# lanterndata/lantern

Measured on AMD Instinct MI355X. Metric: QPS (recall@10 alongside), 1000000x768 f32 l2sq ef=64 k=10, higher is better.
Workload: dtype f32

## Files before the change

include/lantern_gpu.h:

```cpp
#ifndef LANTERN_GPU_H
#define LANTERN_GPU_H

#include <stdbool.h>
#include <stddef.h>
#include <stdint.h>

#ifdef __cplusplus
extern "C" {
#endif

#define LANTERN_GPU_EXPORT __attribute__((visibility("default")))


typedef void       *usearch_index_t;
typedef uint64_t    usearch_key_t;
typedef uint64_t    usearch_label_t;
typedef float       usearch_distance_t;
typedef const char *usearch_error_t;

typedef enum usearch_metric_kind_t {
    usearch_metric_unknown_k = 0,
    usearch_metric_cos_k = 1,
    usearch_metric_l2sq_k = 3,
    usearch_metric_hamming_k = 8
// ... 170 lines not shown
                                                                 size_t query_stride_bytes, size_t nq, size_t k, size_t ef, size_t skip,
                                                                 uint64_t *d_labels, float *d_distances, uint32_t *d_slots,
                                                                 uint32_t *d_counts, uint64_t *d_dist_evals, uint64_t *d_expansions,
                                                                 void *stream, usearch_error_t *);
LANTERN_GPU_EXPORT void lantern_gpu_search_batch_filtered_each(usearch_index_t, const lantern_gpu_filter_t *const *filters, const void *queries,
                                                               size_t nq, usearch_scalar_kind_t, size_t k, size_t ef, usearch_label_t *labels,
                                                               float *distances, uint32_t *counts, usearch_error_t *);
LANTERN_GPU_EXPORT void lantern_gpu_search_batch_filtered_each_device(usearch_index_t, const lantern_gpu_filter_t *const *filters,
                                                                      const void *d_queries, size_t query_stride_bytes, size_t nq, size_t k,
                                                                      size_t ef, size_t skip, uint64_t *d_labels, float *d_distances,
                                                                      uint32_t *d_slots, uint32_t *d_counts, uint64_t *d_dist_evals,
                                                                      uint64_t *d_expansions, void *stream, usearch_error_t *);
LANTERN_GPU_EXPORT void lantern_gpu_search_batch_filtered_each_lane(usearch_index_t, int lane, const lantern_gpu_filter_t *const *filters,
                                                                    const void *queries, size_t nq, usearch_scalar_kind_t, size_t k, size_t ef,
                                                                    usearch_label_t *labels, float *distances, uint32_t *counts,
                                                                    usearch_error_t *);
LANTERN_GPU_EXPORT void lantern_gpu_last_filtered_each(usearch_index_t, uint32_t out[6], usearch_error_t *);
LANTERN_GPU_EXPORT void lantern_gpu_set_search_shape(usearch_index_t, int waves_per_query, int max_workgroups,
                                                     usearch_error_t *);

LANTERN_GPU_EXPORT void lantern_gpu_exact_search(usearch_index_t, const void *queries, size_t nq, size_t k,
                                                 uint32_t *slots, float *distances, usearch_error_t *);

LANTERN_GPU_EXPORT size_t lantern_gpu_dense_profile(int on, float *ms, uint32_t *rows, uint32_t *cols, uint32_t *fused, size_t cap);
LANTERN_GPU_EXPORT void lantern_gpu_exact_knn_stats(uint64_t *queries, uint64_t *certified, uint64_t *fallback);

LANTERN_GPU_EXPORT void lantern_gpu_search_row_trace(usearch_index_t, int on, size_t nq, size_t per_query_cap, uint32_t *trace,
                                                     uint32_t *counts, usearch_error_t *);

LANTERN_GPU_EXPORT int lantern_gpu_last_search_grid(usearch_index_t, usearch_error_t *);
LANTERN_GPU_EXPORT const char *lantern_gpu_plan_search(const int64_t in[31], uint32_t out[12]);
LANTERN_GPU_EXPORT const char *lantern_gpu_plan_search_screen(const int64_t in[32], uint32_t out[13]);
LANTERN_GPU_EXPORT const char *lantern_gpu_plan_search_screen_prefetch(const int64_t in[33], uint32_t out[14]);

LANTERN_GPU_EXPORT void lantern_gpu_distance_gather(usearch_index_t, const void *query, const uint32_t *slots,
                                                    size_t n, float *out, usearch_error_t *);
LANTERN_GPU_EXPORT float lantern_gpu_last_gather_ms(usearch_index_t, usearch_error_t *);
LANTERN_GPU_EXPORT void lantern_gpu_search_screen_stats(usearch_index_t, uint64_t *logical, uint64_t *exact, usearch_error_t *);
LANTERN_GPU_EXPORT void lantern_gpu_set_insert_screen(usearch_index_t, int mode, usearch_error_t *);
LANTERN_GPU_EXPORT void lantern_gpu_insert_screen_stats(usearch_index_t, uint64_t out[4], usearch_error_t *);
LANTERN_GPU_EXPORT const char *lantern_gpu_plan_insert(const int64_t in[13], uint32_t out[7]);
LANTERN_GPU_EXPORT size_t lantern_gpu_export_screen(usearch_index_t, size_t first, size_t count, int8_t *rows, float *meta, float *norms,
                                                    usearch_error_t *);
LANTERN_GPU_EXPORT void lantern_gpu_screen_probe(usearch_index_t, const void *query, const uint32_t *slots, size_t n, float radius,
                                                 int workgroup, uint8_t *rejected, usearch_error_t *);
LANTERN_GPU_EXPORT void lantern_gpu_distance_matrix(const void *a, size_t na, const void *b, size_t nb,
                                                    usearch_scalar_kind_t, size_t dims, usearch_metric_kind_t,
                                                    int exact_order, float *out, usearch_error_t *);

LANTERN_GPU_EXPORT void lantern_gpu_assign_to_clusters(const float *dataset, size_t n, size_t row_dims, size_t subvector_start,
                                                       size_t subvector_dim, const float *centers, size_t k,
                                                       usearch_metric_kind_t metric, uint32_t *out_cluster,
                                                       float *out_distance, usearch_error_t *);

typedef struct lantern_gpu_graph_info
{
    size_t   size;
    size_t   upper_blocks;
    uint32_t connectivity;
    uint32_t entry_slot;
    int32_t  max_level;
    uint32_t vector_words;
} lantern_gpu_graph_info;
LANTERN_GPU_EXPORT lantern_gpu_graph_info lantern_gpu_graph_info_get(usearch_index_t, usearch_error_t *);
LANTERN_GPU_EXPORT void lantern_gpu_export_graph(usearch_index_t, uint8_t *levels, uint32_t *nbr0, uint32_t *upper_off,
                                                 uint32_t *upper_nbr, uint64_t *labels, void *vectors,
                                                 usearch_error_t *);
LANTERN_GPU_EXPORT void lantern_gpu_export_codes(usearch_index_t, uint8_t *codes, usearch_error_t *);
LANTERN_GPU_EXPORT void lantern_gpu_pq_compact(usearch_index_t, usearch_error_t *);
LANTERN_GPU_EXPORT void lantern_gpu_pq_expand(usearch_index_t, usearch_error_t *);
LANTERN_GPU_EXPORT size_t lantern_gpu_row_bytes(usearch_index_t, usearch_error_t *);
LANTERN_GPU_EXPORT void lantern_gpu_memory_usage(usearch_index_t, size_t *row_bytes, size_t *other_bytes, usearch_error_t *);
LANTERN_GPU_EXPORT void lantern_gpu_import_graph(usearch_index_t, size_t size, const void *vectors,
                                                 const uint64_t *labels, const uint8_t *levels, const uint32_t *nbr0,
                                                 const uint32_t *upper_off, const uint32_t *upper_nbr,
                                                 uint32_t entry_slot, int32_t max_level, usearch_error_t *);
// ... 143 lines not shown
```

lantern_amd/capi.py:

```python
from __future__ import annotations

import ctypes as C
import os

import numpy as np

HERE = os.path.dirname(os.path.abspath(__file__))
LIB_PATH = os.path.join(HERE, "lib", "liblantern_gpu.so")

METRIC_COS, METRIC_L2SQ, METRIC_HAMMING = 1, 3, 8
SCALAR_F32, SCALAR_F16, SCALAR_I8, SCALAR_B1 = 1, 3, 4, 5
METRICS = {"cos": METRIC_COS, "l2sq": METRIC_L2SQ, "hamming": METRIC_HAMMING}
EMPTY = 0xFFFFFFFF
USEARCH_HEADER_SIZE = 136


class LanternGpuError(RuntimeError):
    pass


class InitOptions(C.Structure):
    _fields_ = [
        ("metric_kind", C.c_int),
        ("metric", C.c_void_p),
# ... 54 lines not shown
    "lantern_gpu_set_seed", "lantern_gpu_set_add_batch", "lantern_gpu_add_many", "lantern_gpu_flush",
    "lantern_gpu_add_with_level", "lantern_gpu_search_batch", "lantern_gpu_search_batch_device", "lantern_gpu_search_batch_device_strided",
    "lantern_gpu_set_search_shape", "lantern_gpu_exact_search", "lantern_gpu_dense_profile", "lantern_gpu_exact_knn_stats", "lantern_gpu_distance_gather",
    "lantern_gpu_host_alloc", "lantern_gpu_host_free", "lantern_gpu_save_stream", "lantern_gpu_pq_compact", "lantern_gpu_pq_expand", "lantern_gpu_memory_usage", "lantern_gpu_spec_profile", "lantern_gpu_search_unique_rows", "lantern_gpu_search_row_trace", "lantern_gpu_last_search_grid", "lantern_gpu_last_gather_ms", "lantern_gpu_search_screen_stats",
    "lantern_gpu_set_insert_screen", "lantern_gpu_insert_screen_stats", "lantern_gpu_plan_insert",
    "lantern_gpu_distance_matrix", "lantern_gpu_assign_to_clusters", "lantern_gpu_graph_info_get", "lantern_gpu_export_graph", "lantern_gpu_import_graph",
    "lantern_gpu_export_codes",
    "lantern_gpu_counters_get", "lantern_gpu_set_profiling", "lantern_gpu_build_profile_get", "lantern_gpu_search_phase_profile", "lantern_scan_begin", "lantern_scan_rescan", "lantern_scan_gettuple", "lantern_scan_trace", "lantern_scan_end",
    "lantern_l2sq_dist", "lantern_cos_dist", "lantern_hamming_dist", "lantern_index_server_start", "lantern_index_server_start_tls",
    "lantern_index_server_port", "lantern_index_server_status_port", "lantern_index_server_status",
    "lantern_index_server_served", "lantern_index_server_stop",
    "lantern_gpu_graph_checksum", "lantern_gpu_comm_unique_id", "lantern_gpu_comm_init_rccl", "lantern_gpu_comm_init_host",
    "lantern_gpu_comm_init_local", "lantern_gpu_comm_free", "lantern_gpu_comm_rank", "lantern_gpu_comm_world",
    "lantern_gpu_comm_set_timeout", "lantern_gpu_comm_stats", "lantern_gpu_comm_allgatherv_host",
    "lantern_gpu_comm_allgatherv_device", "lantern_gpu_shard_range", "lantern_gpu_add_sharded", "lantern_gpu_add_row_sharded", "lantern_gpu_search_partitioned", "lantern_gpu_search_batch_lane", "lantern_gpu_search_batch_lane_notify", "lantern_gpu_row_bytes",
    "lantern_gpu_level_for", "lantern_gpu_plan_batch", "lantern_gpu_row_shard_plan", "lantern_gpu_plan_search", "lantern_gpu_plan_search_screen", "lantern_gpu_plan_search_screen_prefetch",
    "lantern_scan_server_start", "lantern_scan_server_start_fn", "lantern_scan_server_port", "lantern_scan_server_stats",
    "lantern_scan_server_batch_histogram", "lantern_scan_server_timing", "lantern_scan_server_stop", "lantern_scan_client_connect", "lantern_scan_client_search", "lantern_scan_client_search_next",
    "lantern_scan_client_close", "lantern_scan_begin_client",
    "lantern_mirror_acquire", "lantern_mirror_index", "lantern_mirror_version", "lantern_mirror_rebind", "lantern_mirror_advance", "lantern_mirror_release",
    "lantern_mirror_invalidate", "lantern_mirror_set_capacity", "lantern_mirror_stats",
    "UsearchNodeBytes", "usearch_init_node", "node_tuple_size", "label_from_node", "level_from_node", "reset_node_label", "get_node_neighbors_mut",
    "lantern_quant_bits_scalar_kind",
    "lantern_gpu_filter_from_labels", "lantern_gpu_filter_from_slot_bitmap", "lantern_gpu_filter_count", "lantern_gpu_filter_free",
    "lantern_gpu_set_filter_policy", "lantern_gpu_filter_stats", "lantern_gpu_last_filtered_launch", "lantern_gpu_search_batch_filtered", "lantern_gpu_search_batch_filtered_device",
    "lantern_gpu_cursor_search_filtered", "lantern_scan_set_filter",
    "lantern_gpu_filter_resident_bytes", "lantern_scan_server_start_filtered_fn", "lantern_scan_server_filter_stats", "lantern_scan_client_set_filter",
    "lantern_scan_client_clear_filter",
    "lantern_gpu_search_batch_filtered_each", "lantern_gpu_search_batch_filtered_each_device", "lantern_gpu_search_batch_filtered_each_lane", "lantern_gpu_last_filtered_each",
    "lantern_gpu_set_filter_seeds", "lantern_gpu_last_filtered_seeds",
    "lantern_gpu_search_batch_params", "lantern_gpu_search_batch_params_lane", "lantern_gpu_search_batch_params_lane_notify",
    "lantern_gpu_search_batch_params_device", "lantern_gpu_last_params_launch", "lantern_scan_server_start_params_fn",
    "lantern_gpu_export_screen", "lantern_gpu_screen_probe",
]
QUERY_PARAMS = np.dtype([("k", np.uint32), ("ef", np.uint32), ("skip", np.uint32), ("reserved", np.uint32)])


def query_params(params) -> np.ndarray:
    if isinstance(params, np.ndarray) and params.dtype == QUERY_PARAMS:
        return np.ascontiguousarray(params)
    out = np.zeros(len(params), dtype=QUERY_PARAMS)
    for i, p in enumerate(params):
        p = tuple(int(x) for x in p)
        out[i] = (p[0], p[1] if len(p) > 1 else 0, p[2] if len(p) > 2 else 0, 0)
    return out


FILTER_SKIP_DELETED = 1
FILTER_PATHS = {"auto": 0, "walk": 1, "exact": 2}

BATCH_SEARCH_FN = C.CFUNCTYPE(C.c_int, C.c_void_p, C.c_void_p, C.c_size_t, C.c_size_t, C.c_size_t, C.c_size_t, C.POINTER(C.c_uint64),
                              C.POINTER(C.c_float), C.POINTER(C.c_uint32), C.POINTER(C.c_char_p))

FILTER_MAKE_FN = C.CFUNCTYPE(C.c_void_p, C.c_void_p, C.POINTER(C.c_uint64), C.c_size_t, C.c_uint32, C.POINTER(C.c_uint64), C.POINTER(C.c_uint64),
                             C.POINTER(C.c_char_p))
FILTER_FREE_FN = C.CFUNCTYPE(None, C.c_void_p, C.c_void_p)
BATCH_SEARCH_PARAMS_FN = C.CFUNCTYPE(C.c_int, C.c_void_p, C.c_void_p, C.c_size_t, C.c_size_t, C.c_void_p, C.c_size_t, C.POINTER(C.c_uint64),
                                     C.POINTER(C.c_float), C.POINTER(C.c_uint32), C.POINTER(C.c_char_p))
BATCH_SEARCH_EACH_FN = C.CFUNCTYPE(C.c_int, C.c_void_p, C.POINTER(C.c_void_p), C.c_void_p, C.c_size_t, C.c_size_t, C.c_size_t, C.c_size_t,
                                   C.POINTER(C.c_uint64), C.POINTER(C.c_float), C.POINTER(C.c_uint32), C.POINTER(C.c_char_p))

QUERIES_DONE_FN = C.CFUNCTYPE(None, C.c_void_p, C.POINTER(C.c_uint32), C.c_size_t)
ALLGATHERV_FN = C.CFUNCTYPE(C.c_int, C.c_void_p, C.c_void_p, C.POINTER(C.c_size_t), C.POINTER(C.c_size_t), C.c_int, C.c_int)
COMM_ID_BYTES = 128

_lib = None
# ... 28 lines not shown
        "usearch_save": (None, [vp, C.c_char_p, err]),
        "usearch_save_buffer": (None, [vp, vp, sz, err]),
        "usearch_load": (None, [vp, C.c_char_p, err]),
        "usearch_load_buffer": (None, [vp, vp, sz, err]),
        "usearch_serialized_length": (sz, [vp, err]),
        "usearch_header_get_entry_slot": (u64, [vp]),
        "usearch_header_set_entry_slot": (None, [vp, u64]),
        "usearch_view_mem_lazy": (None, [vp, vp, err]),
        "usearch_update_header": (None, [vp, vp, err]),
        "lantern_gpu_version": (C.c_char_p, []),
        "lantern_gpu_device_count": (i32, []),
        "lantern_gpu_set_seed": (None, [vp, u64, err]),
        "lantern_gpu_set_add_batch": (None, [vp, sz, sz, err]),
        "lantern_gpu_add_many": (None, [vp, vp, vp, sz, i32, err]),
        "lantern_gpu_flush": (None, [vp, err]),
        "lantern_gpu_add_with_level": (None, [vp, u64, vp, i32, i32, err]),
        "lantern_gpu_search_batch": (None, [vp, vp, sz, i32, sz, sz, vp, vp, vp, err]),
        "lantern_gpu_search_batch_device": (None, [vp, vp, sz, sz, sz, sz, vp, vp, vp, vp, vp, vp, vp, err]),
        "lantern_gpu_search_batch_device_strided": (None, [vp, vp, sz, sz, sz, sz, sz, vp, vp, vp, vp, vp, vp, vp, err]),
        "lantern_gpu_set_search_shape": (None, [vp, i32, i32, err]),
        "lantern_gpu_exact_search": (None, [vp, vp, sz, sz, vp, vp, err]),
        "lantern_gpu_dense_profile": (sz, [i32, vp, vp, vp, vp, sz]),
        "lantern_gpu_exact_knn_stats": (None, [C.POINTER(u64), C.POINTER(u64), C.POINTER(u64)]),
        "lantern_gpu_distance_gather": (None, [vp, vp, vp, sz, vp, err]),
        "lantern_gpu_spec_profile": (None, [vp, i32, vp, err]),
        "lantern_gpu_search_unique_rows": (None, [vp, i32, C.POINTER(u64), err]),
        "lantern_gpu_search_row_trace": (None, [vp, i32, sz, sz, vp, vp, err]),
        "lantern_gpu_last_search_grid": (i32, [vp, err]),
        "lantern_gpu_last_gather_ms": (f32, [vp, err]),
        "lantern_gpu_search_screen_stats": (None, [vp, C.POINTER(u64), C.POINTER(u64), err]),
        "lantern_gpu_set_insert_screen": (None, [vp, C.c_int, err]),
        "lantern_gpu_insert_screen_stats": (None, [vp, vp, err]),
        "lantern_gpu_export_screen": (sz, [vp, sz, sz, vp, vp, vp, err]),
        "lantern_gpu_screen_probe": (None, [vp, vp, vp, sz, f32, i32, vp, err]),
        "lantern_gpu_save_stream": (None, [vp, vp, vp, err]),
        "lantern_gpu_pq_compact": (None, [vp, err]),
        "lantern_gpu_pq_expand": (None, [vp, err]),
        "lantern_gpu_memory_usage": (None, [vp, C.POINTER(sz), C.POINTER(sz), err]),
        "lantern_gpu_distance_matrix": (None, [vp, sz, vp, sz, i32, sz, i32, i32, vp, err]),
        "lantern_gpu_assign_to_clusters": (None, [vp, sz, sz, sz, sz, vp, sz, i32, vp, vp, err]),
        "lantern_gpu_graph_info_get": (GraphInfo, [vp, err]),
        "lantern_gpu_export_graph": (None, [vp, vp, vp, vp, vp, vp, vp, err]),
        "lantern_gpu_import_graph": (None, [vp, sz, vp, vp, vp, vp, vp, vp, u32, C.c_int32, err]),
        "lantern_gpu_export_codes": (None, [vp, vp, err]),
        "lantern_gpu_counters_get": (Counters, [vp, err]),
        "lantern_gpu_set_profiling": (None, [vp, i32, err]),
        "lantern_gpu_build_profile_get": (BuildProfile, [vp, err]),
        "lantern_gpu_search_phase_profile": (None, [vp, i32, vp, err]),
        "lantern_scan_begin": (vp, [vp, i32, i32, err]),
        "lantern_scan_rescan": (None, [vp, vp, i32, err]),
        "lantern_scan_gettuple": (C.c_bool, [vp, C.POINTER(u64), err]),
        "lantern_scan_trace": (sz, [vp, vp, sz]),
        "lantern_scan_end": (None, [vp]),
        "lantern_l2sq_dist": (f32, [vp, i32, vp, i32, err]),
        "lantern_cos_dist": (f32, [vp, i32, vp, i32, err]),
        "lantern_hamming_dist": (C.c_int32, [vp, i32, vp, i32, err]),
        "lantern_index_server_start": (vp, [C.c_char_p, i32, i32, C.c_char_p, err]),
        "lantern_index_server_start_tls": (vp, [C.c_char_p, i32, i32, C.c_char_p, C.c_char_p, C.c_char_p, err]),
        "lantern_index_server_port": (i32, [vp]),
        "lantern_index_server_status_port": (i32, [vp]),
        "lantern_index_server_status": (i32, [vp]),
        "lantern_index_server_served": (u64, [vp]),
        "lantern_index_server_stop": (None, [vp]),
        "lantern_gpu_graph_checksum": (u64, [vp, err]),
        "lantern_gpu_comm_unique_id": (None, [vp, err]),
        "lantern_gpu_comm_init_rccl": (vp, [i32, i32, vp, err]),
        "lantern_gpu_comm_init_host": (vp, [i32, i32, ALLGATHERV_FN, vp, err]),
        "lantern_gpu_comm_init_local": (None, [i32, C.POINTER(vp), err]),
        "lantern_gpu_comm_free": (None, [vp]),
        "lantern_gpu_comm_rank": (i32, [vp]),
        "lantern_gpu_comm_world": (i32, [vp]),
        "lantern_gpu_comm_set_timeout": (None, [vp, C.c_double]),
        "lantern_gpu_comm_stats": (None, [vp, C.POINTER(u64), C.POINTER(u64)]),
        "lantern_gpu_comm_allgatherv_host": (None, [vp, vp, C.POINTER(sz), C.POINTER(sz), err]),
        "lantern_gpu_comm_allgatherv_device": (None, [vp, vp, C.POINTER(sz), C.POINTER(sz), vp, err]),
        "lantern_gpu_shard_range": (None, [sz, i32, i32, C.POINTER(sz), C.POINTER(sz)]),
        "lantern_gpu_add_sharded": (None, [vp, vp, vp, vp, sz, i32, err]),
        "lantern_gpu_add_row_sharded": (None, [vp, vp, vp, vp, sz, i32, err]),
        "lantern_gpu_search_partitioned": (None, [vp, vp, vp, sz, i32, sz, sz, vp, vp, vp, err]),
        "lantern_gpu_row_bytes": (sz, [vp, err]),
        "lantern_gpu_search_batch_lane": (None, [vp, i32, vp, sz, i32, sz, sz, vp, vp, vp, err]),
        "lantern_gpu_search_batch_lane_notify": (None, [vp, i32, vp, sz, i32, sz, sz, vp, vp, vp, vp, vp, err]),
        "lantern_gpu_level_for": (i32, [u64, u64, u32]),
        "lantern_gpu_plan_batch": (sz, [sz, i32, vp, sz, sz, sz]),
        "lantern_gpu_plan_search": (C.c_char_p, [vp, vp]),
        "lantern_gpu_plan_search_screen": (C.c_char_p, [vp, vp]),
        "lantern_gpu_plan_search_screen_prefetch": (C.c_char_p, [vp, vp]),
        "lantern_gpu_plan_insert": (C.c_char_p, [vp, vp]),
        "lantern_gpu_row_shard_plan": (sz, [vp, i32, u64, u32, sz, sz, vp, vp, vp, sz]),
        "lantern_scan_server_start": (vp, [vp, C.c_char_p, i32, sz, C.c_uint, err]),
        "lantern_scan_server_start_fn": (vp, [BATCH_SEARCH_FN, vp, sz, C.c_char_p, i32, sz, C.c_uint, err]),
        "lantern_scan_server_port": (i32, [vp]),
        "lantern_scan_server_stats": (None, [vp, C.POINTER(u64), C.POINTER(u64), C.POINTER(u64), C.POINTER(u64)]),
        "lantern_scan_server_batch_histogram": (sz, [vp, C.POINTER(u64), sz]),
        "lantern_scan_server_timing": (None, [vp, C.POINTER(C.c_double)]),
        "lantern_scan_server_stop": (None, [vp]),
        "lantern_scan_client_connect": (vp, [C.c_char_p, i32, err]),
        "lantern_scan_client_search": (sz, [vp, vp, sz, sz, sz, vp, vp, err]),
        "lantern_scan_client_search_next": (sz, [vp, vp, sz, sz, sz, vp, vp, err]),
        "lantern_scan_client_close": (None, [vp]),
        "lantern_scan_begin_client": (vp, [vp, sz, i32, i32, err]),
        "lantern_mirror_acquire": (vp, [u64, u64, C.POINTER(InitOptions), vp, vp, sz, err]),
        "lantern_mirror_index": (vp, [vp]),
        "lantern_mirror_version": (u64, [vp]),
        "lantern_mirror_rebind": (None, [vp, C.POINTER(InitOptions)]),
        "lantern_mirror_advance": (None, [vp, u64]),
        "lantern_mirror_release": (None, [vp]),
        "lantern_mirror_invalidate": (None, [u64]),
        "lantern_mirror_set_capacity": (None, [sz]),
        "lantern_mirror_stats": (None, [C.POINTER(u64), C.POINTER(u64), C.POINTER(u64), C.POINTER(u64)]),
        "UsearchNodeBytes": (u32, [C.POINTER(Metadata), i32, i32]),
        "usearch_init_node": (None, [C.POINTER(Metadata), vp, u64, u32, u64, vp, sz]),
        "node_tuple_size": (u32, [vp, u32, C.POINTER(Metadata)]),
        "label_from_node": (u64, [vp]),
        "level_from_node": (C.c_ulong, [vp]),
        "reset_node_label": (None, [vp]),
        "get_node_neighbors_mut": (vp, [C.POINTER(Metadata), vp, u32, C.POINTER(u32)]),
        "lantern_quant_bits_scalar_kind": (i32, [i32, C.c_bool, err]),
        "lantern_gpu_filter_from_labels": (vp, [vp, vp, sz, u32, err]),
        "lantern_gpu_filter_from_slot_bitmap": (vp, [vp, vp, sz, u32, err]),
# ... 236 lines not shown

    def unique_rows(self, on, read=False):
        out = C.c_uint64(0)
        _call("lantern_gpu_search_unique_rows", self.h, 1 if on else 0, C.byref(out) if read else None)
        return int(out.value) if read else None

    def last_gather_ms(self) -> float:
        return float(_call("lantern_gpu_last_gather_ms", self.h))

    def screen_stats(self):
        logical, exact = C.c_uint64(0), C.c_uint64(0)
        _call("lantern_gpu_search_screen_stats", self.h, C.byref(logical), C.byref(exact))
        return int(logical.value), int(exact.value)

    def set_insert_screen(self, mode):
        _call("lantern_gpu_set_insert_screen", self.h, int(mode))

    def insert_screen_stats(self):
        out = np.zeros(4, dtype=np.uint64)
        _call("lantern_gpu_insert_screen_stats", self.h, _ptr(out))
        return tuple(int(x) for x in out)

    def export_screen(self, first=0, count=None):
        if count is None:
            count = len(self) - first
        row_bytes = int(_call("lantern_gpu_export_screen", self.h, first, count, None, None, None))
        if row_bytes == 0:
            return {"codes": np.zeros((count, 0), np.int8), "meta": None, "norms": None, "row_bytes": 0}
        codes, meta = np.zeros((count, row_bytes), np.int8), np.zeros((count, 2), np.float32)
        norms = np.zeros(count, np.float32) if self.metric == METRIC_COS else None
        _call("lantern_gpu_export_screen", self.h, first, count, _ptr(codes), _ptr(meta), _ptr(norms))
        return {"codes": codes, "meta": meta, "norms": norms, "row_bytes": row_bytes}

    def screen_probe(self, query, slots, radius, workgroup=256):
        q = _rows(query, self.metric)[0]
        s = np.ascontiguousarray(slots, dtype=np.uint32)
        out = np.zeros(s.size, dtype=np.uint8)
        _call("lantern_gpu_screen_probe", self.h, _ptr(q), _ptr(s), s.size, float(radius), int(workgroup), _ptr(out))
        return out.astype(bool)

    def last_search_grid(self) -> int:
        return int(_call("lantern_gpu_last_search_grid", self.h))

    def row_trace_begin(self, nq, per_query_cap):
        self._trace_shape = (int(nq), int(per_query_cap))
        _call("lantern_gpu_search_row_trace", self.h, 1, int(nq), int(per_query_cap), None, None)

    def row_trace_end(self):
        nq, cap = self._trace_shape
        trace = np.zeros((nq, cap), dtype=np.uint32)
        counts = np.zeros(nq, dtype=np.uint32)
        _call("lantern_gpu_search_row_trace", self.h, 0, nq, cap, _ptr(trace), _ptr(counts))
        return trace, counts

    def pq_compact(self):
        _call("lantern_gpu_pq_compact", self.h)

    def pq_expand(self):
        _call("lantern_gpu_pq_expand", self.h)

    def row_bytes(self) -> int:
        return int(_call("lantern_gpu_row_bytes", self.h))

    def memory_usage(self):
        a, b = C.c_size_t(), C.c_size_t()
        _call("lantern_gpu_memory_usage", self.h, C.byref(a), C.byref(b))
# ... 452 lines not shown
    m = Metadata()
    m.neighbors_bytes, m.neighbors_base_bytes = 4 + M * 6, 4 + 2 * M * 6
    m.inverse_log_connectivity = 1.0 / math.log(M)
    m.connectivity, m.dimensions = M, dims
    o = m.init_options
    o.metric_kind, o.quantization, o.dimensions, o.connectivity = metric, quantization, dims, M
    o.pq, o.num_subvectors, o.num_centroids = pq, num_subvectors, num_centroids
    return m


def header_entry_slot(header: bytes) -> int:
    buf = C.create_string_buffer(bytes(header), USEARCH_HEADER_SIZE)
    return int(lib().usearch_header_get_entry_slot(C.cast(buf, C.c_void_p)))


def level_for(seed: int, slot: int, M: int) -> int:
    return int(lib().lantern_gpu_level_for(seed, slot, M))


def plan_batch(size: int, max_level: int, pending_levels, max_batch: int, min_ratio: int) -> int:
    lv = np.ascontiguousarray(pending_levels, dtype=np.int32)
    return int(lib().lantern_gpu_plan_batch(size, max_level, _ptr(lv), lv.size, max_batch, min_ratio))


PLAN_SEARCH_IN = ("chunks", "M", "M0", "mcode", "n", "ef_default", "num_cus", "pq_compact", "pqd_inv", "pq_S16", "search_vis_slots", "search_max_wg",
                  "phase_profile", "spec_profile", "nq", "k", "ef", "skip", "waves", "each", "max_expansion", "env_spec_set", "env_spec",
                  "env_adc_spec_set", "env_adc_spec", "env_pq_adc", "env_spec_waves", "env_lds_list", "env_wide_rows", "env_solo", "env_waves_per_cu")
PLAN_SEARCH_OUT = ("path", "spec", "expansion", "waves", "grid", "vis_slots", "lds", "spec_prefetch", "spec_cache", "wide_rows", "took_spec", "lds_list")


def plan_search(fields) -> tuple[dict, str | None]:
    vals = [fields[n] for n in PLAN_SEARCH_IN] if isinstance(fields, dict) else list(fields)
    assert len(vals) == len(PLAN_SEARCH_IN)
    if isinstance(fields, dict) and "screen_list_prefetch" in fields:
        names = PLAN_SEARCH_OUT + ("screen_lds", "list_prefetch")
        a = np.asarray(vals + [fields.get("screen", 0), fields["screen_list_prefetch"]], dtype=np.int64)
        out = np.zeros(len(names), dtype=np.uint32)
        why = lib().lantern_gpu_plan_search_screen_prefetch(_ptr(a), _ptr(out))
    elif isinstance(fields, dict) and "screen" in fields:
        names = PLAN_SEARCH_OUT + ("screen_lds",)
        a, out = np.asarray(vals + [fields["screen"]], dtype=np.int64), np.zeros(len(names), dtype=np.uint32)
        why = lib().lantern_gpu_plan_search_screen(_ptr(a), _ptr(out))
    else:
        names = PLAN_SEARCH_OUT
        a, out = np.asarray(vals, dtype=np.int64), np.zeros(len(names), dtype=np.uint32)
        why = lib().lantern_gpu_plan_search(_ptr(a), _ptr(out))
    return dict(zip(names, (int(x) for x in out))), (why.decode() if why else None)


PLAN_INSERT_IN = ("mcode", "chunks", "M0", "efc", "rows", "num_cus", "waves", "screen_table", "mode", "lds_list", "only_upper", "lone_ok", "vis_slots_env")
PLAN_INSERT_OUT = ("screened", "vis_slots", "lds", "screen_lds", "lone", "spec_prefetch", "spec_cache")


def plan_insert(fields) -> tuple[dict, str | None]:
    vals = [fields[n] for n in PLAN_INSERT_IN] if isinstance(fields, dict) else list(fields)
    assert len(vals) == len(PLAN_INSERT_IN)
    a, out = np.asarray(vals, dtype=np.int64), np.zeros(len(PLAN_INSERT_OUT), dtype=np.uint32)
    why = lib().lantern_gpu_plan_insert(_ptr(a), _ptr(out))
    return dict(zip(PLAN_INSERT_OUT, (int(x) for x in out))), (why.decode() if why else None)


def row_shard_plan(shard_sizes, seed: int, M: int, max_batch: int, min_ratio: int):
    sizes = np.ascontiguousarray(shard_sizes, dtype=np.uint64)
    world = int(sizes.size)
    n = int(lib().lantern_gpu_row_shard_plan(_ptr(sizes), world, seed, M, max_batch, min_ratio, None, None, None, 0))
    first, count = np.zeros(max(n, 1), dtype=np.uintp), np.zeros(max(n, 1), dtype=np.uintp)
    share = np.zeros((max(n, 1), world), dtype=np.uintp)
# ... 370 lines not shown
```

lantern_amd/csrc/device_common.hpp:

```cpp
#pragma once
#include <hip/hip_runtime.h>
#include <stdint.h>

namespace lgpu {

constexpr uint32_t EMPTY = 0xFFFFFFFFu;
#ifndef LGPU_ROW_BLOCK
#define LGPU_ROW_BLOCK 3
#endif
#ifndef LGPU_ROW_BLOCK_COS
#define LGPU_ROW_BLOCK_COS 2
#endif
#ifndef LGPU_LIST_PREFETCH
#define LGPU_LIST_PREFETCH 1
#endif
#ifndef LGPU_SCREEN_LIST_PREFETCH
#define LGPU_SCREEN_LIST_PREFETCH 1
#endif
#ifndef LGPU_ROW_BLOCK1
#define LGPU_ROW_BLOCK1 4
#endif
#ifndef LGPU_SCREEN
#define LGPU_SCREEN 1
#endif
// ... 466 lines not shown
    for(int r = 0; r < R; ++r) d[ r ] = acc[ r ].template finish_n<G>(a2, b2[ r ]);
}

__host__ __device__ inline int group_lanes_for(uint32_t chunks) { return chunks >= 128 ? 64 : chunks >= 64 ? 32 : chunks >= 32 ? 16 : 8; }

struct View
{
    const uint4    *vec;
    uint32_t        chunks;
    uint32_t        M, M0;
    uint32_t       *nbr0;
    const uint32_t *upper_off;
    uint32_t       *upper_nbr;
    const uint8_t  *levels;
    const float    *norm2;
    uint32_t        n;
    uint32_t        entry;
    int32_t         max_level;
    const uint4    *pq_centers;
    uint32_t        pq_cps;
    uint32_t        pq_C;
    uint32_t        pq_inv;
    uint32_t        pq_row_bytes;
    const uint4    *screen;
    const float2   *screen_meta;
    uint32_t        screen_chunks;
};

__host__ __device__ __forceinline__ float screen_val(float s, uint32_t w, int b) { return s * (float)(int)(int8_t)(uint8_t)(w >> (8 * b)); }
__host__ __device__ inline bool screen_rows_for(uint32_t chunks) { return chunks >= 128; }
__host__ __device__ inline bool screen_cos_norm_ok(float r) { return r >= 0x1p-48f && r <= 0x1p48f; }
__host__ __device__ inline uint32_t screen_chunks_for(uint32_t chunks) { return (chunks + 3) / 4; }
__host__ __device__ inline uint32_t screen_query_lds_bytes(uint32_t chunks) { return 16 + screen_chunks_for(chunks) * 32; }
__host__ __device__ inline bool screen_l2_scale_ok(float s) { return s >= 0x1p-40f && s <= 0x1p40f; }

__device__ __forceinline__ const uint4 *row_of(const View &v, uint32_t slot) { return v.vec + (size_t)slot * v.chunks; }

struct PqdRow
{
    const uint8_t *codes;
    const uint4   *centers;
    uint32_t       cps, C, inv;
    __device__ __forceinline__ uint4 operator[](int ch) const
    {
        const uint32_t sv = ((uint32_t)ch * inv) >> 16, off = (uint32_t)ch - sv * cps;
        const uint32_t code = codes[ sv ];
        return centers[ ((size_t)sv * C + code) * cps + off ];
    }
};
template <int METRIC> __device__ __forceinline__ auto row_of_m(const View &v, uint32_t slot)
{
    if constexpr(METRIC >= M_PQD) return PqdRow{ (const uint8_t *)v.vec + (size_t)slot * v.pq_row_bytes, v.pq_centers, v.pq_cps, v.pq_C, v.pq_inv };
    else return v.vec + (size_t)slot * v.chunks;
}
template <int METRIC> __device__ __forceinline__ float row_norm(const View &v, uint32_t slot)
{
    if constexpr(kCachedNorms<METRIC>) return v.norm2[ slot ];
    else return 0.f;
}

__device__ __forceinline__ uint32_t *neighbors_of(const View &v, uint32_t slot, int level, uint32_t &cap)
{
    if(level == 0) {
        cap = v.M0;
        return v.nbr0 + (size_t)slot * v.M0;
    }
// ... 6 lines not shown
```

lantern_amd/csrc/index.cpp:

```cpp
#include "index.hpp"
#include "abi_guard.hpp"
#include "host_trip.hpp"

#include <algorithm>
#include <cmath>
#include <cstdio>
#include <cstdlib>
#include <cstring>
#include <new>

#include <time.h>

#include "comm.hpp"
#include "host_util.hpp"

static bool exact_knn_device(int mcode, uint32_t chunks, const uint4 *d_base, size_t nb, const uint4 *d_q, size_t nq, size_t k,
                             uint32_t *d_slots, float *d_dists, hipStream_t st);


namespace lgpu {

static const char *kNoDevice = "lantern_gpu: no HIP device available (this library has no CPU fallback)";

const char *set_err(Index *ix, const std::string &msg)
// ... 49 lines not shown
View Index::view() const
{
    View v{};
    v.vec = d_vec;
    v.chunks = chunks;
    v.M = M;
    v.M0 = M0;
    v.nbr0 = d_nbr0;
    v.upper_off = d_upper_off;
    v.upper_nbr = d_upper_nbr;
    v.levels = d_levels;
    v.norm2 = d_norm2;
    v.screen = d_screen;
    v.screen_meta = d_screen_meta;
    v.screen_chunks = d_screen ? screen_chunks_for(chunks) : 0u;
    v.n = (uint32_t)n;
    v.entry = entry;
    v.max_level = max_level;
    return v;
}

static bool reserve_locked(Index *ix, size_t newcap)
{
    if(newcap <= ix->cap) return true;
    if(newcap >= 0x7FFFFFFFull) { set_err(ix, "lantern_gpu: capacity above 2^31-1 slots is not supported"); return false; }
    if(!pq_expand_locked(ix)) return false;
    const size_t oc = ix->cap, row = (size_t)ix->chunks * 16;
    if(!dev_grow(ix, (void **)&ix->d_vec, oc * row, newcap * row, -1)) return false;
    if(mcode_base(ix->mcode) == M_COS && !mcode_is_i8(ix->mcode) && !dev_grow(ix, (void **)&ix->d_norm2, oc * 4, newcap * 4, -1)) return false;
    if(ix->screen) {
        const size_t srow = (size_t)screen_chunks_for(ix->chunks) * 16;
        if(!dev_grow(ix, (void **)&ix->d_screen, oc * srow, newcap * srow, 0)) return false;
        if(!dev_grow(ix, (void **)&ix->d_screen_meta, oc * 8, newcap * 8, 0)) return false;
    }
    if(ix->pq && !dev_grow(ix, (void **)&ix->d_codes, oc * ix->pq_S, newcap * ix->pq_S, 0)) return false;
    if(!dev_grow(ix, (void **)&ix->d_labels, oc * 8, newcap * 8, -1)) return false;
    if(!dev_grow(ix, (void **)&ix->d_levels, oc, newcap, 0)) return false;
    if(!dev_grow(ix, (void **)&ix->d_nbr0, oc * ix->M0 * 4, newcap * ix->M0 * 4, 0xFF)) return false;
    if(!dev_grow(ix, (void **)&ix->d_radius0, oc * 4, newcap * 4, 0xFF)) return false;
    if(!dev_grow(ix, (void **)&ix->d_upper_off, oc * 4, newcap * 4, 0xFF)) return false;
    ix->cap = newcap;
    if(ix->d_bitmaps) { (void)hipFree(ix->d_bitmaps); ix->d_bitmaps = nullptr; }
    ix->bitmap_slots = 0;
    ix->bm_words = 0;
    return true;
}

static bool reserve_upper(Index *ix, size_t need_blocks)
{
    if(need_blocks <= ix->upper_cap) return true;
    size_t nc = std::max<size_t>(std::max<size_t>(ix->upper_cap * 2, need_blocks), 1024);
    if(!dev_grow(ix, (void **)&ix->d_upper_nbr, ix->upper_cap * ix->M * 4, nc * ix->M * 4, 0xFF)) return false;
    if(!dev_grow(ix, (void **)&ix->d_radius_upper, ix->upper_cap * 4, nc * 4, 0xFF)) return false;
    ix->upper_cap = nc;
    return true;
}

bool rows_stored(Index *ix, size_t first, size_t count)
{
    if(count == 0) return true;
    if(ix->d_norm2) HIPCHK(ix, launch_fill_norms(ix->mcode, ix->view(), (uint32_t)first, (uint32_t)count, ix->d_norm2, ix->stream));
    if(ix->d_screen)
        HIPCHK(ix, launch_fill_screen(ix->view(), (uint32_t)first, (uint32_t)count, ix->d_screen, ix->d_screen_meta, ix->mcode == M_COS ? ix->d_norm2 : nullptr, ix->stream));
    return true;
}

bool pq_encode_rows(Index *ix, size_t first, size_t count)
{
    if(!ix->pq || count == 0) return true;
    const uint32_t sub_chunks = (ix->pq_subdim + 3) / 4, sub_floats = sub_chunks * 4, row_floats = ix->chunks * 4;
    float    *d_sub = nullptr;
    uint32_t *d_near = nullptr;
    bool ok = hipMalloc((void **)&d_sub, count * (size_t)sub_floats * 4) == hipSuccess && hipMalloc((void **)&d_near, count * 8) == hipSuccess;
    for(uint32_t sv = 0; ok && sv < ix->pq_S; ++sv) {
        ok = ok && launch_pq_take((const float *)ix->d_vec, row_floats, (uint32_t)first, (uint32_t)count, sv, ix->pq_subdim, sub_floats, d_sub, ix->stream) == hipSuccess;
        ok = ok && ::exact_knn_device(ix->metric, sub_chunks, (const uint4 *)(ix->d_centers + (size_t)sv * ix->pq_C * sub_floats), ix->pq_C, (const uint4 *)d_sub,
                                    count, 1, d_near, (float *)(d_near + count), ix->stream);
        ok = ok && launch_pq_put((float *)ix->d_vec, row_floats, (uint32_t)first, (uint32_t)count, sv, ix->pq_subdim, ix->pq_S, d_near, ix->d_codebook,
                                 (uint32_t)ix->opts.dimensions, ix->d_codes, ix->stream) == hipSuccess;
    }
    ok = ok && hipStreamSynchronize(ix->stream) == hipSuccess;
    if(d_sub) (void)hipFree(d_sub);
    if(d_near) (void)hipFree(d_near);
    if(!ok) set_err(ix, "lantern_gpu: HIP failure while quantising vectors");
    return ok;
}

bool pq_decode_rows(Index *ix, size_t first, size_t count)
{
    if(!ix->pq || count == 0) return true;
    HIPCHK(ix, launch_pq_decode((float *)ix->d_vec, ix->chunks * 4, (uint32_t)first, (uint32_t)count, ix->pq_subdim, ix->pq_S, ix->d_codebook,
                                (uint32_t)ix->opts.dimensions, ix->d_codes, ix->stream));
    return true;
}

static uint32_t pqd_inverse(uint32_t cps, uint32_t chunks)
// ... 328 lines not shown
    const size_t first = ix->n;
    const int    W = comm ? comm->world : 1, R = comm ? comm->rank : 0;
    const bool   split = W > 1 && b >= (size_t)W * kShardMinPerRank;
    const size_t b_lo = split ? b * (size_t)R / (size_t)W : 0, b_hi = split ? b * ((size_t)R + 1) / (size_t)W : b;
    std::vector<uint32_t> &link_off = ix->h_link_off;
    link_off.resize(b);
    size_t total_links = 0;
    for(size_t i = 0; i < b; ++i) {
        link_off[ i ] = (uint32_t)total_links;
        total_links += (size_t)ix->M * (size_t)(lv[ i ] + 1);
    }
    const size_t items = total_links / ix->M;
    uint32_t *d_link_off = (uint32_t *)scratch(ix, kScratchLinkOff, b * 4 + items * 4 + items * 4);
    LinkReq  *d_links = (LinkReq *)scratch(ix, kScratchLinks, total_links * sizeof(LinkReq));
    uint64_t *d_tops = (uint64_t *)scratch(ix, kScratchTops, items * (size_t)ix->efc * 8);
    LinkReq  *d_reqs = (LinkReq *)scratch(ix, kScratchReqs, total_links * sizeof(LinkReq));
    char     *d_grp = (char *)scratch(ix, kScratchGroups, total_links * sizeof(uint2) + 16 + (size_t)W * 4);
    void     *d_work = scratch(ix, kScratchWork, total_links * 8 + 16);
    const size_t temp_bytes = group_temp_bytes(total_links);
    char     *d_sort = (char *)scratch(ix, kScratchSort, total_links * 24 + temp_bytes + 64);
    if(!d_link_off || !d_links || !d_tops || !d_reqs || !d_grp || !d_work || !d_sort) return false;
    uint32_t *d_item_node = d_link_off + b, *d_top_count = d_item_node + items;
    uint2    *d_groups = (uint2 *)d_grp;
    uint32_t *d_ngroups = (uint32_t *)(d_grp + total_links * sizeof(uint2));
    uint32_t *d_owner = d_ngroups + 4;
    GroupScratch gs;
    gs.keys_a = (uint64_t *)d_sort;
    gs.keys_b = gs.keys_a + total_links;
    gs.idx_a = (uint32_t *)(gs.keys_b + total_links);
    gs.idx_b = gs.idx_a + total_links;
    gs.temp = (void *)(((uintptr_t)(gs.idx_b + total_links) + 63) & ~(uintptr_t)63);
    gs.temp_bytes = temp_bytes;

    prof_mark(ix, 0);
    HIPCHK(ix, launch_batch_layout(ix->d_levels + first, (uint32_t)b, ix->M, d_link_off, d_item_node, ix->stream));

    static const bool ins_spec_env = !(std::getenv("LANTERN_GPU_INSERT_SPEC") && std::atoi(std::getenv("LANTERN_GPU_INSERT_SPEC")) == 0);
    InsertPlanIn pin;
    pin.mcode = ix->mcode, pin.num_cus = ix->num_cus, pin.waves = ix->insert_waves;
    pin.chunks = ix->chunks, pin.M0 = ix->M0, pin.efc = ix->efc;
    pin.rows = b_hi - b_lo;
    pin.screen_table = ix->d_screen && ix->d_screen_meta;
    pin.mode = ix->insert_screen;
    pin.lds_list = search_env().lds_list;
    pin.only_upper = rs != nullptr;
    pin.lone_ok = ins_spec_env && !comm && !rs;
    if(const char *vs = std::getenv("LANTERN_GPU_INSERT_VIS_SLOTS")) pin.vis_slots_env = std::max(0, std::atoi(vs));
    const InsertPlan ip = plan_insert(pin);
    if(ip.refusal) { set_err(ix, ip.refusal); return false; }
    const bool ins_spec = ip.lone;
    const int  ins_waves = ins_spec ? 11 : ix->insert_waves;
    const int  grid = ins_spec ? (int)std::max<size_t>(1, std::min<size_t>(b_hi - b_lo, (size_t)ix->num_cus)) : search_grid(ix, b_hi - b_lo, ix->insert_waves, 20);
    if(!ensure_bitmaps(ix, (size_t)grid)) return false;
    if(!order_launch(ix, ix->stream)) return false;
    auto link_at = [&](size_t i) { return i < b ? (size_t)link_off[ i ] : total_links; };

    InsertArgs ia;
    ia.view = ix->view();
    if(!ip.screened) ia.view.screen = nullptr, ia.view.screen_meta = nullptr, ia.view.screen_chunks = 0;
    ia.first_slot = (uint32_t)first;
    ia.b_begin = (uint32_t)b_lo;
    ia.count = (uint32_t)b_hi;
    ia.efc = ix->efc;
    ia.link_off = d_link_off;
    ia.tops = d_tops;
    ia.top_count = d_top_count;
// ... 265 lines not shown
    }
    if(total == 0) return true;
    StagedMeta s;
    if(!stage_meta(ix, nullptr, total, s)) return false;
    const size_t in_bytes = input_bytes(ix, kind_in);
    std::vector<uint32_t> padded;
    const void *src = vectors;
    if(n_shard && !(kind_in == ix->scalar && in_bytes == row)) {
        padded.resize(n_shard * (size_t)ix->chunks * 4);
        for(size_t i = 0; i < n_shard; ++i) pad_row(ix, (const char *)vectors + i * in_bytes, kind_in, &padded[ i * (size_t)ix->chunks * 4 ]);
        src = padded.data();
    }
    char     *vec_base = (char *)ix->d_vec + first * row;
    uint64_t *lab_base = ix->d_labels + first;
    if(n_shard) {
        HIPCHK(ix, hipMemcpyAsync(vec_base + my_off * row, src, n_shard * row, hipMemcpyHostToDevice, ix->stream));
        HIPCHK(ix, hipMemcpyAsync(lab_base + my_off, labels, n_shard * 8, hipMemcpyHostToDevice, ix->stream));
    }
    HIPCHK(ix, hipMemcpyAsync(ix->d_levels + first, s.l8.data(), total, hipMemcpyHostToDevice, ix->stream));
    HIPCHK(ix, hipMemcpyAsync(ix->d_upper_off + first, s.uo.data(), total * 4, hipMemcpyHostToDevice, ix->stream));
    HIPCHK(ix, hipStreamSynchronize(ix->stream));
    size_t at = 0;
    for(int r = 0; r < W; ++r) { off[ (size_t)r ] = at * row; cnt[ (size_t)r ] = (size_t)meta[ (size_t)r * 2 ] * row; at += (size_t)meta[ (size_t)r * 2 ]; }
    if(!comm->allgatherv_device(vec_base, off.data(), cnt.data(), ix->stream)) { set_err(ix, comm->err); return false; }
    for(int r = 0; r < W; ++r) { off[ (size_t)r ] = off[ (size_t)r ] / row * 8; cnt[ (size_t)r ] = cnt[ (size_t)r ] / row * 8; }
    if(!comm->allgatherv_device(lab_base, off.data(), cnt.data(), ix->stream)) { set_err(ix, comm->err); return false; }
    std::vector<uint64_t> all_labels(total);
    HIPCHK(ix, hipMemcpyAsync(all_labels.data(), lab_base, total * 8, hipMemcpyDeviceToHost, ix->stream));
    if(!sync_stream(ix, comm)) return false;
    if(!pq_encode_rows(ix, first, total)) return false;
    if(!rows_stored(ix, first, total)) return false;
    bool ok = true;
    run_batches(ix, all_labels.data(), s, total, comm, &ok);
    return ok;
}

static bool row_shard_candidates(Index *ix, const RowShard &rs, size_t first, size_t b, const uint32_t *d_link_off, uint64_t *d_tops, uint32_t *d_top_count)
{
    Index       *loc = rs.loc;
    Comm        *comm = rs.comm;
    const int    W = comm->world, R = comm->rank;
    const size_t K = rs.K, part = b * K, row = (size_t)ix->chunks * 16;
    char *d_all = (char *)scratch(ix, kScratchShardParts, (size_t)W * part * 12 + 64);
    if(!d_all) return false;
    uint64_t *g_lab = (uint64_t *)d_all;
    float    *g_dist = (float *)(d_all + (size_t)W * part * 8);
    bool ok = true;
    if(loc->n == 0) {
        std::vector<float> inf(part, __builtin_inff());
        ok = hipMemsetAsync(g_lab + (size_t)R * part, 0, part * 8, ix->stream) == hipSuccess &&
             hipMemcpyAsync(g_dist + (size_t)R * part, inf.data(), part * 4, hipMemcpyHostToDevice, ix->stream) == hipSuccess &&
             hipStreamSynchronize(ix->stream) == hipSuccess;
    } else {
        std::lock_guard<std::mutex> gl(loc->mu);
        ok = run_search_device(loc, (const uint4 *)((const char *)ix->d_vec + first * row), b, K, rs.ef, 0,
                               SearchOut{ g_lab + (size_t)R * part, g_dist + (size_t)R * part, nullptr, nullptr, nullptr, nullptr }, ix->stream, loc->search_waves);
        if(!ok) set_err(ix, "lantern_gpu: row-sharded build, candidate search: " + loc->err);
    }
    if(ok && W > 1) {
        std::vector<size_t> off((size_t)W), cnt((size_t)W);
        for(int r = 0; r < W; ++r) { off[ (size_t)r ] = (size_t)r * part * 8; cnt[ (size_t)r ] = part * 8; }
        ok = comm->allgatherv_device(g_lab, off.data(), cnt.data(), ix->stream);
        for(int r = 0; r < W; ++r) { off[ (size_t)r ] = (size_t)r * part * 4; cnt[ (size_t)r ] = part * 4; }
        ok = ok && comm->allgatherv_device(g_dist, off.data(), cnt.data(), ix->stream);
        if(!ok) set_err(ix, "lantern_gpu: row-sharded build, exchange of the candidate lists: " + comm->err);
    }
    ok = ok && launch_merge_candidates(g_lab, g_dist, (uint32_t)W, (uint32_t)b, (uint32_t)K, (uint32_t)first, d_link_off, ix->M, ix->efc, d_tops, d_top_count,
// ... 19 lines not shown
    }
    std::vector<uint32_t> padded(count * row_words);
    for(size_t i = 0; i < count; ++i) pad_row(ix, (const char *)vectors + i * in_bytes, kind_in, &padded[ i * row_words ]);
    HIPCHK(ix, hipMemcpyAsync(dst, padded.data(), count * row, hipMemcpyHostToDevice, ix->stream));
    HIPCHK(ix, hipStreamSynchronize(ix->stream));
    return true;
}

bool add_row_sharded_locked(Index *ix, Comm *comm, const uint64_t *labels, const void *vectors, size_t n_shard, int kind_in)
{
    if(ix->n || !ix->pend_labels.empty()) { set_err(ix, "lantern_gpu: the row-sharded build needs an empty index"); return false; }
    if(ix->pq || ix->b1_from_f32) { set_err(ix, "lantern_gpu: the row-sharded build does not take pq or quant_bits = 1 indexes"); return false; }
    const int    W = comm->world, R = comm->rank;
    const size_t row = (size_t)ix->chunks * 16, M0 = ix->M0, efc = ix->efc, in_bytes = input_bytes(ix, kind_in);
    std::vector<uint64_t> sizes((size_t)W, 0);
    std::vector<size_t>   off((size_t)W), cnt((size_t)W);
    sizes[ (size_t)R ] = n_shard;
    for(int r = 0; r < W; ++r) { off[ (size_t)r ] = (size_t)r * 8; cnt[ (size_t)r ] = 8; }
    if(!comm->allgatherv_host(sizes.data(), off.data(), cnt.data())) { set_err(ix, comm->err); return false; }
    std::vector<size_t> lo((size_t)W + 1, 0);
    for(int r = 0; r < W; ++r) lo[ (size_t)r + 1 ] = lo[ (size_t)r ] + (size_t)sizes[ (size_t)r ];
    const size_t N = lo[ (size_t)W ];
    if(N == 0) return true;
    if(N >= 0x7FFFFFFEull) { set_err(ix, "lantern_gpu: capacity above 2^31-1 slots is not supported"); return false; }
    usearch_error_t err = nullptr;
    usearch_init_options_t lo_opts = ix->opts;
    lo_opts.retriever = lo_opts.retriever_mut = nullptr;
    lo_opts.retriever_ctx = nullptr;
    Index *loc = (Index *)usearch_init(&lo_opts, nullptr, &err);
    if(!loc) { set_err(ix, std::string("lantern_gpu: row-sharded build: ") + (err ? err : "cannot create the shard's index")); return false; }
    struct Cleanup { Index *a = nullptr; ~Cleanup() { usearch_error_t ig = nullptr; if(a) usearch_free(a, &ig); } } cleanup;
    cleanup.a = loc;
    loc->seed = ix->seed;
    loc->efc = ix->efc;
    loc->add_batch_max = ix->add_batch_max;
    loc->add_min_ratio = ix->add_min_ratio;
    if(n_shard) {
        usearch_reserve(loc, n_shard, &err);
        if(err) { set_err(ix, std::string("lantern_gpu: row-sharded build, shard graph: ") + err); return false; }
    }
    StagedMeta s;
    if(!stage_meta(ix, nullptr, N, s)) return false;
    struct Batch { size_t first, b; };
    std::vector<Batch>  plan;
    std::vector<size_t> share;
    {
        std::vector<size_t> pf, pc;
        row_shard_plan(sizes.data(), W, s.lv.data(), N, ix->add_batch_max, ix->add_min_ratio, pf, pc, share);
        for(size_t t = 0; t < pf.size(); ++t) plan.push_back({ pf[ t ], pc[ t ] });
    }
    std::vector<uint64_t> by_rank(N), all_labels(N);
    if(n_shard) std::memcpy(&by_rank[ lo[ (size_t)R ] ], labels, n_shard * 8);
    for(int r = 0; r < W; ++r) { off[ (size_t)r ] = lo[ (size_t)r ] * 8; cnt[ (size_t)r ] = (size_t)sizes[ (size_t)r ] * 8; }
    if(W > 1 && !comm->allgatherv_host(by_rank.data(), off.data(), cnt.data())) { set_err(ix, comm->err); return false; }
    {
        std::vector<size_t> cur(lo.begin(), lo.end() - 1);
        for(size_t t = 0; t < plan.size(); ++t) {
            size_t at = plan[ t ].first;
            for(int r = 0; r < W; ++r)
                for(size_t j = 0; j < share[ t * (size_t)W + (size_t)r ]; ++j) all_labels[ at++ ] = by_rank[ cur[ (size_t)r ]++ ];
        }
    }
    HIPCHK(ix, hipMemcpyAsync(ix->d_labels, all_labels.data(), N * 8, hipMemcpyHostToDevice, ix->stream));
    HIPCHK(ix, hipMemcpyAsync(ix->d_levels, s.l8.data(), N, hipMemcpyHostToDevice, ix->stream));
    HIPCHK(ix, hipMemcpyAsync(ix->d_upper_off, s.uo.data(), N * 4, hipMemcpyHostToDevice, ix->stream));
    HIPCHK(ix, hipStreamSynchronize(ix->stream));
// ... 15 lines not shown
        if(my_n && !stage_rows_at(ix, first + my_off, (const char *)vectors + mine * in_bytes, my_n, kind_in)) return false;
        if(W > 1) {
            size_t at = 0;
            for(int r = 0; r < W; ++r) { off[ (size_t)r ] = at * row; cnt[ (size_t)r ] = sh[ r ] * row; at += sh[ r ]; }
            if(!comm->allgatherv_device((char *)ix->d_vec + first * row, off.data(), cnt.data(), ix->stream)) { set_err(ix, comm->err); return false; }
        }
        if(!rows_stored(ix, first, b)) return false;
        if(ix->n == 0) {
            ix->n = 1;
            ix->entry = 0;
            ix->max_level = s.lv[ 0 ];
            ix->c_add_vectors += 1;
        } else if(!run_batch(ix, b, s.lv.data() + first, nullptr, &rs)) {
            return false;
        }
        if(my_n) {
            gl.resize(my_n);
            for(size_t i = 0; i < my_n; ++i) gl[ i ] = (uint64_t)(first + my_off + i) + 1;
            lantern_gpu_add_many(loc, gl.data(), (const char *)vectors + mine * in_bytes, my_n, (usearch_scalar_kind_t)kind_in, &err);
            if(!err) lantern_gpu_flush(loc, &err);
            if(err) { set_err(ix, std::string("lantern_gpu: row-sharded build, shard graph: ") + err); return false; }
            mine += my_n;
        }
        return sync_stream(ix, comm);
    };
    for(size_t t = 0; t < plan.size() && ok; ++t) ok = batch(t);
    if(ix->profiling) prof_resolve(ix, 0);
    const size_t done = ix->n;
    ix->labels.assign(all_labels.begin(), all_labels.begin() + (ptrdiff_t)done);
    ix->levels.assign(s.l8.begin(), s.l8.begin() + (ptrdiff_t)done);
    ix->upper_off.assign(s.uo.begin(), s.uo.begin() + (ptrdiff_t)done);
    ix->upper_blocks = 0;
    for(size_t i = 0; i < done; ++i) ix->upper_blocks += (size_t)s.lv[ i ];
    return ok;
}

bool flush_locked(Index *ix)
{
    const size_t pending = ix->pend_labels.size();
    if(pending == 0) return true;
    const size_t row_words = (size_t)ix->chunks * 4;
    bool         ok = true;
    const size_t pi = insert_rows(ix, ix->pend_labels.data(), ix->pend_levels.data(), ix->pend_rows.data(), pending, &ok);
    ix->pend_labels.erase(ix->pend_labels.begin(), ix->pend_labels.begin() + (ptrdiff_t)pi);
    ix->pend_levels.erase(ix->pend_levels.begin(), ix->pend_levels.begin() + (ptrdiff_t)pi);
    ix->pend_rows.erase(ix->pend_rows.begin(), ix->pend_rows.begin() + (ptrdiff_t)(pi * row_words));
    if(ix->pend_labels.empty()) { std::vector<uint32_t>().swap(ix->pend_rows); }
    return ok;
}


size_t search_one_locked(Index *ix, Cursor *cur, const void *query, int kind, size_t k, size_t ef, bool streaming, uint64_t *labels,
                         float *distances)
{
    if(!streaming) cur->seen.clear();
    if(ix->n == 0 || k == 0) return 0;
    const size_t want = std::min(cur->seen.size() + k, ix->n);
    const size_t row = (size_t)ix->chunks * 16;
    const size_t need = row + want * 16 + 32;
    if(ix->h_single_bytes < need) {
        if(ix->h_single) (void)hipHostFree(ix->h_single);
        ix->h_single = ix->h_single_dev = nullptr;
        ix->h_single_bytes = 0;
        const size_t cap = need * 2 + 4096;
        if(hipHostMalloc((void **)&ix->h_single, cap, hipHostMallocMapped) != hipSuccess) {
            set_err(ix, "lantern_gpu: cannot allocate the pinned single-query block");
            return 0;
// ... 120 lines not shown
{
    if(ix->n || !ix->pend_labels.empty()) { set_err(ix, "lantern_gpu: import needs an empty index"); return false; }
    if(size == 0) return true;
    if(!pq_expand_locked(ix)) return false;
    size_t blocks = 0;
    for(size_t i = 0; i < size; ++i) blocks += levels[ i ];
    if(!reserve_locked(ix, std::max(size, ix->cap)) || !reserve_upper(ix, blocks)) return false;
    if(ix->pq && vectors_are_codes) {
        HIPCHK(ix, hipMemcpy(ix->d_codes, vectors, size * (size_t)ix->pq_S, hipMemcpyHostToDevice));
        if(!pq_decode_rows(ix, 0, size)) return false;
    } else if(ix->chunks * 4 == ix->words) {
        HIPCHK(ix, hipMemcpy(ix->d_vec, vectors, size * (size_t)ix->words * 4, hipMemcpyHostToDevice));
    } else {
        HIPCHK(ix, hipMemset(ix->d_vec, 0, size * (size_t)ix->chunks * 16));
        HIPCHK(ix, hipMemcpy2D(ix->d_vec, (size_t)ix->chunks * 16, vectors, (size_t)ix->words * 4, (size_t)ix->words * 4, size,
                               hipMemcpyHostToDevice));
    }
    if(ix->pq && !vectors_are_codes && !pq_encode_rows(ix, 0, size)) return false;
    if(!rows_stored(ix, 0, size)) return false;
    ix->labels.resize(size);
    for(size_t i = 0; i < size; ++i) ix->labels[ i ] = labels ? labels[ i ] : (uint64_t)i;
    ix->levels.assign(levels, levels + size);
    ix->upper_off.assign(upper_off, upper_off + size);
    HIPCHK(ix, hipMemcpy(ix->d_labels, ix->labels.data(), size * 8, hipMemcpyHostToDevice));
    HIPCHK(ix, hipMemcpy(ix->d_levels, levels, size, hipMemcpyHostToDevice));
    HIPCHK(ix, hipMemcpy(ix->d_nbr0, nbr0, size * ix->M0 * 4, hipMemcpyHostToDevice));
    HIPCHK(ix, hipMemcpy(ix->d_upper_off, upper_off, size * 4, hipMemcpyHostToDevice));
    if(blocks) HIPCHK(ix, hipMemcpy(ix->d_upper_nbr, upper_nbr, blocks * ix->M * 4, hipMemcpyHostToDevice));
    ix->n = size;
    ix->upper_blocks = blocks;
    ix->radius_stale = true;
    ix->entry = entry_slot;
    ix->max_level = max_level;
    if(ix->pq) {
        const char *pc = std::getenv("LANTERN_GPU_PQ_COMPACT");
        if(pc && std::atoi(pc) != 0 && !pq_compact_locked(ix)) return false;
    }
    return true;
}

}

using namespace lgpu;

Index *lgpu::H(usearch_index_t h, usearch_error_t *e)
{
    if(!h) { FAIL(e, "lantern_gpu: null index handle"); return nullptr; }
    if(((const Index *)h)->magic != kIndexMagic) { FAIL(e, "lantern_gpu: not an index handle (stale, freed or foreign pointer)"); return nullptr; }
    (void)hipSetDevice(((Index *)h)->device);
    return (Index *)h;
}

extern "C" {

const char *lantern_gpu_version(void) { return LGPU_EXPERIMENTAL ? "lantern_gpu 0.1 (gfx950) +experimental" : "lantern_gpu 0.1 (gfx950)"; }

int lantern_gpu_device_count(void)
try {
    int n = 0;
    if(hipGetDeviceCount(&n) != hipSuccess) return 0;
    return n;
}
LANTERN_ABI_CATCH(nullptr)

usearch_index_t usearch_init(usearch_init_options_t *o, float *pq_codebook, usearch_error_t *e)
try {
// ... 64 lines not shown
        ix->pq_subdim = (uint32_t)(o->dimensions / o->num_subvectors);
        const size_t d = o->dimensions, subf = (size_t)((ix->pq_subdim + 3) / 4) * 4;
        ix->h_codebook.assign(pq_codebook, pq_codebook + (size_t)ix->pq_C * d);
        std::vector<float> centers((size_t)ix->pq_S * ix->pq_C * subf, 0.f);
        for(size_t sv = 0; sv < ix->pq_S; ++sv)
            for(size_t c = 0; c < ix->pq_C; ++c)
                std::memcpy(&centers[ (sv * ix->pq_C + c) * subf ], pq_codebook + c * d + sv * ix->pq_subdim, (size_t)ix->pq_subdim * 4);
        const bool ok = hipMalloc((void **)&ix->d_codebook, ix->h_codebook.size() * 4) == hipSuccess &&
                        hipMalloc((void **)&ix->d_centers, centers.size() * 4) == hipSuccess &&
                        hipMemcpy(ix->d_codebook, ix->h_codebook.data(), ix->h_codebook.size() * 4, hipMemcpyHostToDevice) == hipSuccess &&
                        hipMemcpy(ix->d_centers, centers.data(), centers.size() * 4, hipMemcpyHostToDevice) == hipSuccess;
        if(!ok) {
            usearch_error_t ignore = nullptr;
            usearch_free(ix, &ignore);
            FAIL(e, "lantern_gpu: device allocation failed (codebook)");
            return nullptr;
        }
    }
    {
        const char *se = std::getenv("LANTERN_GPU_SCREEN");
        ix->screen = LGPU_SCREEN && (ix->mcode == M_L2SQ || ix->mcode == M_COS) && !ix->pq && screen_rows_for(ix->chunks) && !(se && std::atoi(se) == 0);
        const char *ie = std::getenv("LANTERN_GPU_INSERT_SCREEN");
        ix->insert_screen = ie ? (std::atoi(ie) != 0 ? 1 : 0) : (kInsertScreenByDefault ? 1 : 0);
    }
    return ix;
}
LANTERN_ABI_CATCH(e)

void usearch_free(usearch_index_t h, usearch_error_t *e)
try {
    CLEAR(e);
    Index *ix = H(h, e);
    if(!ix) return;
    void *ptrs[] = { ix->d_vec, ix->d_norm2, ix->d_screen, ix->d_screen_meta, ix->d_labels, ix->d_levels, ix->d_nbr0, ix->d_upper_off, ix->d_upper_nbr, ix->d_bitmaps, ix->d_totals, ix->d_tickets,
                     ix->d_radius0, ix->d_radius_upper,
                     ix->d_codebook, ix->d_centers, ix->d_codes, ix->d_codes16, ix->d_touched, ix->d_trace, ix->d_trace_count };
    for(void *p : ptrs)
        if(p) (void)hipFree(p);
    for(void *p : ix->d_scratch)
        if(p) (void)hipFree(p);
    prof_resolve(ix, 0);
    for(hipEvent_t ev : ix->prof_free) (void)hipEventDestroy(ev);
    if(ix->h_single) (void)hipHostFree(ix->h_single);
    if(ix->h_stage) (void)hipHostFree(ix->h_stage);
    for(int sl = 0; sl < Index::kSearchSlots; ++sl) {
        if(sl > 0 && ix->slot_bitmaps[ sl ]) (void)hipFree(ix->slot_bitmaps[ sl ]);
        if(ix->slot_done[ sl ]) (void)hipEventDestroy(ix->slot_done[ sl ]);
    }
    if(ix->insert_done) (void)hipEventDestroy(ix->insert_done);
    for(hipStream_t ls : ix->lane_stream)
        if(ls) (void)hipStreamDestroy(ls);
    for(char *lh : ix->lane_host)
        if(lh) (void)hipHostFree(lh);
    ix->magic = 0;
    delete ix;
}
LANTERN_ABI_CATCH_VOID(e)

void usearch_reserve(usearch_index_t h, size_t capacity, usearch_error_t *e)
try {
    CLEAR(e);
    Index *ix = H(h, e);
    if(!ix) return;
    std::lock_guard<std::mutex> g(ix->mu);
    if(!reserve_locked(ix, capacity)) FAIL(e, ix->err.c_str());
}
LANTERN_ABI_CATCH_VOID(e)
// ... 8 lines not shown
}
LANTERN_ABI_CATCH(e)

size_t usearch_capacity(usearch_index_t h, usearch_error_t *e)
try {
    CLEAR(e);
    Index *ix = H(h, e);
    if(!ix) return 0;
    std::lock_guard<std::mutex> g(ix->mu);
    return std::max(ix->cap, ix->n + ix->pend_labels.size());
}
LANTERN_ABI_CATCH(e)

size_t usearch_dimensions(usearch_index_t h, usearch_error_t *e)
try {
    CLEAR(e);
    Index *ix = H(h, e);
    return ix ? ix->opts.dimensions : 0;
}
LANTERN_ABI_CATCH(e)

static void add_common(Index *ix, const usearch_label_t *labels, const void *vectors, size_t n, usearch_scalar_kind_t kind,
                       int level, usearch_error_t *e)
try {
    if(!kind_accepted(ix, (int)kind)) { FAIL(e, "lantern_gpu: scalar kind of the vector does not match the index"); return; }
    if(!vectors || !labels) { FAIL(e, "lantern_gpu: null vector or label pointer"); return; }
    std::lock_guard<std::mutex> g(ix->mu);
    const size_t row_words = (size_t)ix->chunks * 4;
    const size_t in_bytes = input_bytes(ix, (int)kind);
    if(n >= ix->add_batch_max && (int)kind == ix->scalar && in_bytes == row_words * 4 && level < 0) {
        if(!flush_locked(ix)) { FAIL(e, ix->err.c_str()); return; }
        bool ok = true;
        insert_rows(ix, labels, nullptr, (const uint32_t *)vectors, n, &ok);
        if(!ok) FAIL(e, ix->err.c_str());
        return;
    }
    if(n >= ix->add_batch_max && (int)kind == usearch_scalar_f32_k && level < 0 &&
       (ix->scalar == usearch_scalar_f16_k || ix->scalar == usearch_scalar_i8_k || ix->b1_from_f32)) {
        if(!flush_locked(ix)) { FAIL(e, ix->err.c_str()); return; }
        bool ok = true;
        insert_rows(ix, labels, nullptr, (const uint32_t *)vectors, n, &ok, true);
        if(!ok) FAIL(e, ix->err.c_str());
        return;
    }
    const size_t base = ix->pend_labels.size();
    try {
        ix->pend_labels.insert(ix->pend_labels.end(), labels, labels + n);
        ix->pend_levels.insert(ix->pend_levels.end(), n, level);
        ix->pend_rows.resize((base + n) * row_words);
    } catch(...) {
        ix->pend_labels.resize(base);
        ix->pend_levels.resize(base);
        ix->pend_rows.resize(base * row_words);
        throw;
    }
    for(size_t i = 0; i < n; ++i) pad_row(ix, (const char *)vectors + i * in_bytes, (int)kind, &ix->pend_rows[ (base + i) * row_words ]);
    if(ix->pend_labels.size() >= ix->add_batch_max && !flush_locked(ix)) FAIL(e, ix->err.c_str());
}
LANTERN_ABI_CATCH_VOID(e)

void usearch_add(usearch_index_t h, usearch_label_t label, const void *vector, usearch_scalar_kind_t kind, usearch_error_t *e)
try {
    CLEAR(e);
    Index *ix = H(h, e);
    if(ix) add_common(ix, &label, vector, 1, kind, -1, e);
}
LANTERN_ABI_CATCH_VOID(e)

void *lantern_gpu_host_alloc(size_t bytes)
try {
    void *p = nullptr;
    if(lantern_gpu_device_count() <= 0 || hipHostMalloc(&p, bytes ? bytes : 1, hipHostMallocDefault) != hipSuccess) return nullptr;
    return p;
}
LANTERN_ABI_CATCH(nullptr)

void lantern_gpu_host_free(void *p)
try {
    if(p) (void)hipHostFree(p);
}
LANTERN_ABI_CATCH_VOID(nullptr)

void lantern_gpu_add_many(usearch_index_t h, const usearch_label_t *labels, const void *vectors, size_t n,
                          usearch_scalar_kind_t kind, usearch_error_t *e)
try {
    CLEAR(e);
    Index *ix = H(h, e);
    if(ix && n) add_common(ix, labels, vectors, n, kind, -1, e);
}
LANTERN_ABI_CATCH_VOID(e)
// ... 120 lines not shown
                                  size_t *first, size_t *count, size_t *share, size_t capacity)
try {
    if(!shard_sizes || world < 1) return 0;
    size_t N = 0;
    for(int r = 0; r < world; ++r) N += (size_t)shard_sizes[ r ];
    std::vector<int> lv(N);
    for(size_t i = 0; i < N; ++i) lv[ i ] = level_for(seed, i, connectivity < 2 ? 2 : connectivity);
    std::vector<size_t> pf, pc, ps;
    row_shard_plan(shard_sizes, world, lv.data(), N, max_batch ? max_batch : 1, min_ratio ? min_ratio : 1, pf, pc, ps);
    for(size_t t = 0; t < pf.size() && t < capacity; ++t) {
        if(first) first[ t ] = pf[ t ];
        if(count) count[ t ] = pc[ t ];
        if(share)
            for(int r = 0; r < world; ++r) share[ t * (size_t)world + (size_t)r ] = ps[ t * (size_t)world + (size_t)r ];
    }
    return pf.size();
}
LANTERN_ABI_CATCH(nullptr)

size_t lantern_gpu_plan_batch(size_t current_size, int max_level, const int *pending_levels, size_t pending, size_t max_batch,
                              size_t min_ratio)
try {
    if(!pending_levels) return 0;
    return plan_batch(current_size, max_level, pending_levels, pending, max_batch ? max_batch : 1, min_ratio ? min_ratio : 1);
}
LANTERN_ABI_CATCH(nullptr)

void lantern_gpu_flush(usearch_index_t h, usearch_error_t *e)
try {
    CLEAR(e);
    Index *ix = H(h, e);
    if(!ix) return;
    std::lock_guard<std::mutex> g(ix->mu);
    if(!flush_locked(ix)) FAIL(e, ix->err.c_str());
}
LANTERN_ABI_CATCH_VOID(e)

void lantern_gpu_set_seed(usearch_index_t h, uint64_t seed, usearch_error_t *e)
try {
    CLEAR(e);
    Index *ix = H(h, e);
    if(ix) ix->seed = seed;
}
LANTERN_ABI_CATCH_VOID(e)

void lantern_gpu_set_add_batch(usearch_index_t h, size_t max_batch, size_t min_ratio, usearch_error_t *e)
try {
    CLEAR(e);
    Index *ix = H(h, e);
    if(!ix) return;
    if(max_batch == 0 || min_ratio == 0) { FAIL(e, "lantern_gpu: batch parameters must be positive"); return; }
    std::lock_guard<std::mutex> g(ix->mu);
    ix->add_batch_max = max_batch;
    ix->add_min_ratio = min_ratio;
}
LANTERN_ABI_CATCH_VOID(e)

void lantern_gpu_set_search_shape(usearch_index_t h, int waves, int max_wg, usearch_error_t *e)
try {
    CLEAR(e);
    Index *ix = H(h, e);
    if(!ix) return;
    if(waves < 0 || waves > 8) { FAIL(e, "lantern_gpu: waves_per_query must be in [1, 8], or 0 = automatic"); return; }
    ix->search_waves = waves;
    ix->insert_waves = waves ? waves : 4;
    ix->search_max_wg = max_wg;
}
// ... 945 lines not shown
    s.mcode = (int)in[ 0 ]; s.chunks = (uint32_t)in[ 1 ]; s.M0 = (uint32_t)in[ 2 ]; s.efc = (uint32_t)in[ 3 ]; s.rows = (size_t)in[ 4 ];
    s.num_cus = (int)in[ 5 ]; s.waves = (int)in[ 6 ]; s.screen_table = in[ 7 ] != 0; s.mode = (int)in[ 8 ]; s.lds_list = in[ 9 ] != 0;
    s.only_upper = in[ 10 ] != 0; s.lone_ok = in[ 11 ] != 0; s.vis_slots_env = (int)in[ 12 ];
    const lgpu::InsertPlan p = lgpu::plan_insert(s);
    const uint32_t flat[ 7 ] = { p.screened ? 1u : 0u, p.vis_slots, (uint32_t)p.lds, p.screen_lds, p.lone ? 1u : 0u, p.spec_prefetch, p.spec_cache };
    std::copy(std::begin(flat), std::end(flat), out);
    return p.refusal;
}

size_t lantern_gpu_export_screen(usearch_index_t h, size_t first, size_t count, int8_t *rows, float *meta, float *norms, usearch_error_t *e)
try {
    CLEAR(e);
    if(count > SIZE_MAX - first) { FAIL(e, "lantern_gpu: slot range out of the index"); return 0; }
    Index *ix = H(h, e);
    if(!ix) return 0;
    std::lock_guard<std::mutex> g(ix->mu);
    if(!flush_locked(ix)) { FAIL(e, ix->err.c_str()); return 0; }
    if(first + count > ix->n) { FAIL(e, "lantern_gpu: slot range out of the index"); return 0; }
    if(!ix->d_screen || !ix->d_screen_meta) return 0;
    const size_t srow = (size_t)screen_chunks_for(ix->chunks) * 16;
    bool         ok = true;
    if(count) {
        if(rows) ok = ok && hipMemcpyAsync(rows, (const char *)ix->d_screen + first * srow, count * srow, hipMemcpyDeviceToHost, ix->stream) == hipSuccess;
        if(meta) ok = ok && hipMemcpyAsync(meta, ix->d_screen_meta + first, count * 8, hipMemcpyDeviceToHost, ix->stream) == hipSuccess;
        if(norms && ix->mcode == M_COS && ix->d_norm2)
            ok = ok && hipMemcpyAsync(norms, ix->d_norm2 + first, count * 4, hipMemcpyDeviceToHost, ix->stream) == hipSuccess;
        ok = ok && hipStreamSynchronize(ix->stream) == hipSuccess;
    }
    if(!ok) { FAIL(e, "lantern_gpu: HIP failure exporting the screen"); return 0; }
    return srow;
}
LANTERN_ABI_CATCH(e)

void lantern_gpu_screen_probe(usearch_index_t h, const void *query, const uint32_t *slots, size_t n, float radius, int workgroup,
                              uint8_t *rejected, usearch_error_t *e)
try {
    CLEAR(e);
    if(n > 64) { FAIL(e, "lantern_gpu: screen_probe takes at most 64 slots"); return; }
    if(workgroup != 256 && workgroup != 512) { FAIL(e, "lantern_gpu: screen_probe workgroup must be 256 or 512"); return; }
    if(!query || (n && (!slots || !rejected))) { FAIL(e, "lantern_gpu: null buffer"); return; }
    Index *ix = H(h, e);
    if(!ix) return;
    std::lock_guard<std::mutex> g(ix->mu);
    if(!flush_locked(ix)) { FAIL(e, ix->err.c_str()); return; }
    if(!ix->d_screen || !ix->d_screen_meta) { FAIL(e, "lantern_gpu: the index has no int8 screen"); return; }
    if(n == 0) return;
    for(size_t i = 0; i < n; ++i)
        if(slots[ i ] >= ix->n) { FAIL(e, "lantern_gpu: slot out of range"); return; }
    const size_t row = (size_t)ix->chunks * 16;
    char        *buf = (char *)scratch(ix, kScratchCallIn, row + n * 4 + 64);
    if(!buf) { FAIL(e, ix->err.c_str()); return; }
    std::vector<uint32_t> padded((size_t)ix->chunks * 4);
    pad_row(ix, query, usearch_scalar_f32_k, padded.data());
    uint32_t *d_slots = (uint32_t *)(buf + row);
    uint8_t  *d_out = (uint8_t *)(buf + row + n * 4);
    bool      ok = hipMemcpyAsync(buf, padded.data(), row, hipMemcpyHostToDevice, ix->stream) == hipSuccess;
    ok = ok && hipMemcpyAsync(d_slots, slots, n * 4, hipMemcpyHostToDevice, ix->stream) == hipSuccess;
    ok = ok && launch_screen_probe(ix->mcode, ix->view(), (const uint4 *)buf, d_slots, (uint32_t)n, radius, workgroup, d_out, ix->stream) == hipSuccess;
    ok = ok && hipMemcpyAsync(rejected, d_out, n, hipMemcpyDeviceToHost, ix->stream) == hipSuccess;
    ok = ok && hipStreamSynchronize(ix->stream) == hipSuccess;
    if(!ok) FAIL(e, "lantern_gpu: HIP failure in screen_probe");
}
LANTERN_ABI_CATCH_VOID(e)

float lantern_gpu_last_gather_ms(usearch_index_t h, usearch_error_t *e)
try {
// ... 110 lines not shown
    std::lock_guard<std::mutex> g(ix->mu);
    if(!pq_compact_locked(ix)) FAIL(e, ix->err.c_str());
}
LANTERN_ABI_CATCH_VOID(e)

void lantern_gpu_pq_expand(usearch_index_t h, usearch_error_t *e)
try {
    CLEAR(e);
    Index *ix = H(h, e);
    if(!ix) return;
    std::lock_guard<std::mutex> g(ix->mu);
    if(!pq_expand_locked(ix)) FAIL(e, ix->err.c_str());
}
LANTERN_ABI_CATCH_VOID(e)

size_t lantern_gpu_row_bytes(usearch_index_t h, usearch_error_t *e)
try {
    CLEAR(e);
    Index *ix = H(h, e);
    return ix ? (size_t)ix->chunks * 16 : 0;
}
LANTERN_ABI_CATCH(e)

void lantern_gpu_memory_usage(usearch_index_t h, size_t *row_bytes, size_t *other_bytes, usearch_error_t *e)
try {
    CLEAR(e);
    Index *ix = H(h, e);
    if(!ix) return;
    std::lock_guard<std::mutex> g(ix->mu);
    const size_t cap = ix->cap;
    if(row_bytes) *row_bytes = ix->pq_compact ? std::max<size_t>(ix->n, 1) * ix->pq_S16 : (ix->d_vec ? cap * (size_t)ix->chunks * 16 : 0);
    if(other_bytes)
        *other_bytes = cap * ((size_t)ix->M0 * 4 + 8 + 1 + 4 + 4) + ix->upper_cap * ((size_t)ix->M * 4 + 4) + (ix->d_norm2 ? cap * 4 : 0) +
                       (ix->pq ? cap * (size_t)ix->pq_S : 0) + (ix->d_screen ? cap * ((size_t)screen_chunks_for(ix->chunks) * 16 + 8) : 0);
}
LANTERN_ABI_CATCH_VOID(e)

void lantern_gpu_export_codes(usearch_index_t h, uint8_t *codes, usearch_error_t *e)
try {
    CLEAR(e);
    Index *ix = H(h, e);
    if(!ix) return;
    std::lock_guard<std::mutex> g(ix->mu);
    if(!flush_locked(ix)) { FAIL(e, ix->err.c_str()); return; }
    if(!ix->pq) { FAIL(e, "lantern_gpu: not a pq index"); return; }
    if(ix->n && hipMemcpy(codes, ix->d_codes, ix->n * (size_t)ix->pq_S, hipMemcpyDeviceToHost) != hipSuccess) FAIL(e, "lantern_gpu: HIP failure exporting the codes");
}
LANTERN_ABI_CATCH_VOID(e)

void lantern_gpu_import_graph(usearch_index_t h, size_t size, const void *vectors, const uint64_t *labels, const uint8_t *levels,
                              const uint32_t *nbr0, const uint32_t *upper_off, const uint32_t *upper_nbr, uint32_t entry_slot,
                              int32_t max_level, usearch_error_t *e)
try {
    CLEAR(e);
    Index *ix = H(h, e);
    if(!ix) return;
    std::lock_guard<std::mutex> g(ix->mu);
    if(!import_graph_locked(ix, size, vectors, labels, levels, nbr0, upper_off, upper_nbr, entry_slot, max_level)) FAIL(e, ix->err.c_str());
}
LANTERN_ABI_CATCH_VOID(e)

}
```

lantern_amd/csrc/index.hpp:

```cpp
#pragma once
#include <hip/hip_runtime.h>

#include <deque>
#include <mutex>
#include <string>
#include <thread>
#include <unordered_map>
#include <unordered_set>
#include <functional>
#include <vector>

#include "../../include/lantern_gpu.h"
#include "kernels.hpp"

namespace lgpu {

struct Cursor
{
    std::unordered_set<uint32_t> seen;
};

constexpr int kIndexLanes = 8;

enum ScratchSlot : int
// ... 26 lines not shown
    int      mcode = 0;
    int      scalar = 0;
    uint32_t words = 0;
    uint32_t chunks = 0;
    uint32_t natural_chunks = 0;
    uint32_t M = 16, M0 = 32, efc = 128, ef = 64;
    uint64_t seed = 42;
    size_t   add_batch_max = 8192, add_min_ratio = 16;
    int      search_waves = 0 , search_max_wg = 0, insert_waves = 4;
    int      search_vis_slots = -1;

    bool     b1_from_f32 = false;
    bool     pq = false;
    uint32_t pq_S = 0, pq_C = 0, pq_subdim = 0;
    std::vector<float> h_codebook;
    float   *d_codebook = nullptr;
    float   *d_centers = nullptr;
    uint8_t *d_codes = nullptr;
    bool     pq_compact = false;
    uint8_t *d_codes16 = nullptr;
    uint32_t pq_S16 = 0;
    uint32_t pqd_inv = 0;

    size_t   n = 0, cap = 0;
    uint32_t entry = EMPTY;
    int      max_level = -1;
    size_t   upper_blocks = 0, upper_cap = 0;

    uint4    *d_vec = nullptr;
    float    *d_norm2 = nullptr;
    bool      screen = false;
    uint4    *d_screen = nullptr;
    float2   *d_screen_meta = nullptr;
    uint64_t *d_labels = nullptr;
    uint8_t  *d_levels = nullptr;
    uint32_t *d_nbr0 = nullptr;
    uint32_t *d_upper_off = nullptr;
    uint32_t *d_upper_nbr = nullptr;
    float    *d_radius0 = nullptr, *d_radius_upper = nullptr;
    bool      radius_stale = false;
    uint32_t *d_bitmaps = nullptr;
    size_t    bitmap_slots = 0, bm_words = 0;
    uint32_t *d_tickets = nullptr;
    uint32_t  ticket_next = 0;
    bool      use_tickets = true;
    unsigned long long *d_totals = nullptr;
    int      insert_screen = 0;
    uint64_t insert_launches_screened = 0, insert_launches_plain = 0;

    static const int kLanes = kIndexLanes;
    static const int kSearchSlots = kLanes;
    void  *d_scratch[ kScratchCount ] = {};
    size_t scratch_bytes[ kScratchCount ] = {};
    hipStream_t lane_stream[ kLanes ] = {};
    char       *lane_host[ kLanes + 1 ] = {};
    size_t      lane_host_bytes[ kLanes + 1 ] = {};

    std::vector<uint64_t> labels;
    std::vector<uint8_t>  levels;
    std::vector<uint32_t> upper_off;

    std::mutex            mu;
    std::vector<uint64_t> pend_labels;
    std::vector<uint32_t> pend_rows;
    std::vector<int>      pend_levels;

// ... 70 lines not shown
struct HostBatch
{
    size_t      nq = 0, k = 0, q_bytes = 0, out_at = 0, out_bytes = 0, extra_at = 0, extra_bytes = 0;
    int         which = Index::kLanes;
    char       *hs = nullptr;
    hipStream_t stream = nullptr;
    char       *d_q = nullptr, *d_out = nullptr;

    size_t    bytes() const { return extra_at + extra_bytes + 64; }
    char     *h_out() const { return hs + out_at; }
    char     *h_extra() const { return hs + extra_at; }
    SearchOut out(char *block) const { return { (uint64_t *)block, (float *)(block + nq * k * 8), nullptr, (uint32_t *)(block + nq * k * 12), nullptr, nullptr }; }
};
constexpr const char *kNoStage = "lantern_gpu: cannot allocate the page-locked staging block";
constexpr const char *kNoLaneStage = "lantern_gpu: cannot allocate the lane's page-locked staging block";
HostBatch batch_layout(const Index *ix, int which, size_t nq, size_t k, size_t extra_bytes = 0);
bool      batch_stage(Index *ix, HostBatch &b, const void *queries, int kind);
bool      batch_device(Index *ix, HostBatch &b, bool buffers = true);
bool      batch_upload(const HostBatch &b);
bool      batch_download(const HostBatch &b);
void      batch_unpack(const HostBatch &b, size_t first, size_t count, uint64_t *labels, float *distances, uint32_t *counts );
bool      batch_finish_locked(Index *ix, const HostBatch &b, bool ok, const char *what, uint64_t *labels, float *distances, uint32_t *counts);
size_t    take_unseen(Cursor *cur, const uint64_t *labels, const float *dists, const uint32_t *slots, uint32_t got, size_t k, uint64_t *out_labels,
                      float *out_dists);

const char *set_err(Index *ix, const std::string &msg);
bool        flush_locked(Index *ix);
bool        ensure_bitmaps(Index *ix, size_t slots);
bool        pq_encode_rows(Index *ix, size_t first, size_t count);
bool        pq_decode_rows(Index *ix, size_t first, size_t count);
bool        pq_compact_locked(Index *ix);
bool        pq_expand_locked(Index *ix);
bool        rows_stored(Index *ix, size_t first, size_t count);
void       *scratch(Index *ix, int which, size_t bytes);
bool        pad_row(const Index *ix, const void *vec, int kind_in, uint32_t *dst);
size_t      input_bytes(const Index *ix, int kind_in);
bool        kind_accepted(const Index *ix, int kind_in);
void        pad_rows(const Index *ix, const void *rows, int kind, size_t count, uint32_t *padded);
uint32_t   *next_ticket(Index *ix, size_t work, int grid, hipStream_t stream);
uint32_t    vis_undo_cap();
int         search_grid(const Index *ix, size_t nq, int waves, int waves_per_cu);
int         search_grid(int num_cus, int max_wg, int forced_waves_per_cu, size_t nq, int waves, int waves_per_cu);
struct SearchEnv
{
    bool spec_set = false, adc_spec_set = false;
    int  spec = 0, spec_waves = 0, wide_rows = -1, waves_per_cu = 0;
    bool adc_spec = false, pq_adc = false, lds_list = false, solo = false;
    int  screen_list_prefetch = -1;
};
SearchEnv search_env();
struct SearchPlanIn
{
    uint32_t  chunks = 0, M = 0, M0 = 0, ef_default = 0, pqd_inv = 0, pq_S16 = 0;
    int       mcode = 0, num_cus = 0, search_vis_slots = -1, search_max_wg = 0;
    bool      pq_compact = false, phase_profile = false, spec_profile = false;
    bool      screen = false;
    size_t    n = 0, nq = 0, k = 0, ef = 0, skip = 0;
    int       waves = 0;
    bool      each = false;
    uint32_t  max_expansion = 0;
    SearchEnv env;
};
enum SearchPath : uint32_t { kSearchAdc, kSearchPqd, kSearchClassic, kSearchSpec1, kSearchSpec2, kSearchTwin, kSearchSolo };
struct SearchPlan
{
    SearchPath  path = kSearchClassic;
    int         spec = 0, waves = 0, grid = 0, wide_rows = 0, lds_list = 0;
    uint32_t    expansion = 0, vis_slots = 0, spec_prefetch = 0, spec_cache = 0;
    size_t      lds = 0;
    uint32_t    screen_lds = 0;
    uint32_t    list_prefetch = 0;
    bool        took_spec = false;
    const char *refusal = nullptr;
};
SearchPlan   plan_search(const SearchPlanIn &in);
SearchPlanIn search_plan_in(const Index *ix, size_t nq, size_t k, size_t ef, size_t skip, int waves);
struct InsertPlanIn
{
    int      mcode = 0, num_cus = 0, waves = 0;
    uint32_t chunks = 0, M0 = 0, efc = 0;
    size_t   rows = 0;
    bool     screen_table = false;
    int      mode = 0;
    bool     lds_list = false;
    bool     only_upper = false;
    bool     lone_ok = false;
    int      vis_slots_env = -1;
};
struct InsertPlan
{
    bool        screened = false;
    bool        lone = false;
    uint32_t    vis_slots = 0, screen_lds = 0, spec_prefetch = 0, spec_cache = 0;
    size_t      lds = 0;
    const char *refusal = nullptr;
};
InsertPlan plan_insert(const InsertPlanIn &in);
struct EachLaunch
{
    const char *h_table = nullptr;
    size_t      table_bytes = 0;
    const char *d_table = nullptr;
    size_t      list_at = 0;
};
// ... 33 lines not shown
```

lantern_amd/csrc/kernels.hip:

```cpp
#include <algorithm>
#include <cstdlib>
#include <string>

#include "kernels.hpp"
#include "walk.hpp"
#include "dispatch.hpp"

namespace lgpu {

template <int METRIC, int G, int CPLC = 4>
__global__ void __launch_bounds__(256) k_connect(ConnectArgs a)
{
    const int tid = threadIdx.x, T = blockDim.x;
    RefineLds r;
    unsigned char *p = carve_refine(lgpu_smem, r, a.efc);
    int      *scal = (int *)p;                  p += S_SCALARS * 4;
    uint32_t *kid = (uint32_t *)p;              p += (size_t)((a.view.M + 3) & ~3u) * 4;
    float    *kd = (float *)p;
    const uint32_t item = a.item_begin + blockIdx.x;
    const uint32_t b = a.item_node[ item ];
    const uint32_t M = a.view.M;
    const uint32_t me = a.first_slot + b;
    const int      level = (int)(item - a.link_off[ b ] / M);
    LinkReq       *out = a.links + a.link_off[ b ] + (uint32_t)level * M;
// ... 794 lines not shown
                const uint32_t qc = 4 * c + (uint32_t)k;
                if(qc >= chunks) continue;
                const uint4 x = row[ qc ];
                const float f[ 4 ] = { __uint_as_float(x.x), __uint_as_float(x.y), __uint_as_float(x.z), __uint_as_float(x.w) };
#pragma unroll
                for(int b = 0; b < 4; ++b) {
                    int q = 0;
                    if(ok) q = (int)fminf(127.f, fmaxf(-127.f, rintf(f[ b ] / sc)));
                    w[ k ] |= ((uint32_t)q & 255u) << (8 * b);
                    const double dd = (double)f[ b ] - (double)screen_val(sc, w[ k ], b);
                    r2 = r2 + dd * dd;
                    if constexpr(COS) y2 = y2 + (double)f[ b ] * (double)f[ b ];
                }
            }
            screen[ (size_t)slot * sch + c ] = make_uint4(w[ 0 ], w[ 1 ], w[ 2 ], w[ 3 ]);
        }
        for(int off = 32; off > 0; off >>= 1) {
            r2 = r2 + __shfl_xor(r2, off);
            if constexpr(COS) y2 = y2 + __shfl_xor(y2, off);
        }
        if(lane == 0) {
            float r = __builtin_inff();
            if(ok) {
                const double rr = COS ? sqrt(r2 / y2 * (1.0 + 0x1p-40)) : sqrt(r2 * (1.0 + 0x1p-40));
                r = (float)rr;
                if((double)r < rr) r = nextafterf(r, __builtin_inff());
                if(!__builtin_isfinite(r)) r = __builtin_inff();
            }
            meta[ slot ] = make_float2(COS && ok ? sc / rb : sc, r);
        }
    }
}

template <int METRIC, int G>
__global__ void __launch_bounds__(256) k_gather(View v, const uint4 *query, const uint32_t *slots, uint32_t n, float *out)
{
    const uint32_t gid = (blockIdx.x * blockDim.x + threadIdx.x) / G, gl = threadIdx.x % G;
    const uint32_t ngroups = gridDim.x * blockDim.x / G;
    for(uint32_t i = gid; i < n; i += ngroups) {
        float d = group_dist<METRIC, G>(query, row_of(v, slots[ i ]), (int)v.chunks, (int)gl);
        if(gl == G - 1) out[ i ] = d;
    }
}

template <int METRIC, int G>
__global__ void __launch_bounds__(256, 6) k_gather_walkshape(View v, const uint4 *query, const uint32_t *slots, uint32_t n, float *out)
{
    uint4 *q = (uint4 *)lgpu_smem;
    __shared__ float qn_s;
    const uint32_t tid = threadIdx.x, gl = tid % G, NG = blockDim.x / G;
    for(uint32_t i = tid; i < v.chunks; i += blockDim.x) q[ i ] = query[ i ];
    __syncthreads();
    if(kCachedNorms<METRIC>) {
        if(tid < G) {
            const float qn = group_norm<METRIC, G>(q, (int)v.chunks, (int)tid);
            if(tid == G - 1) qn_s = qn;
        }
        __syncthreads();
    }
    const float    qn2 = kCachedNorms<METRIC> ? qn_s : 0.f;
    const uint32_t gid = blockIdx.x * NG + tid / G, ngroups = gridDim.x * NG;
    for(uint32_t i = gid; i < n; i += 2 * ngroups) {
        const uint32_t j = i + ngroups;
        const uint32_t id0 = slots[ i ], id1 = j < n ? slots[ j ] : id0;
        float          d0, d1;
        group_dist2_n<METRIC, G>(q, row_of(v, id0), row_of(v, id1), (int)v.chunks, (int)gl, qn2, row_norm<METRIC>(v, id0), row_norm<METRIC>(v, id1), d0, d1);
// ... 113 lines not shown

hipError_t launch_apply_lists(const View &v, const uint32_t *records, uint32_t nrecords, hipStream_t stream)
{
    if(nrecords == 0) return hipSuccess;
    const uint64_t threads = (uint64_t)nrecords * (v.M0 + 2);
    hipLaunchKernelGGL(k_apply_lists, dim3((uint32_t)((threads + 255) / 256)), dim3(256), 0, stream, v, records, nrecords);
    return hipGetLastError();
}

hipError_t launch_fill_norms(int metric, const View &v, uint32_t first, uint32_t count, float *norm2, hipStream_t stream)
{
    if(count == 0 || (metric != M_COS && metric != M_COS_F16)) return hipSuccess;
    const int G_ = group_lanes_for(v.chunks);
    uint32_t  blocks = (uint32_t)(((uint64_t)count * G_ + 255) / 256);
    if(blocks > 16384) blocks = 16384;
#define FN(MM, GG) hipLaunchKernelGGL((k_fill_norms<MM, GG>), dim3(blocks), dim3(256), 0, stream, v, first, count, norm2)
#define FNG(MM) switch(G_) { case 64: FN(MM, 64); break; case 32: FN(MM, 32); break; case 16: FN(MM, 16); break; default: FN(MM, 8); }
    if(metric == M_COS) FNG(M_COS) else FNG(M_COS_F16)
#undef FNG
#undef FN
    return hipGetLastError();
}

hipError_t launch_fill_screen(const View &v, uint32_t first, uint32_t count, uint4 *screen, float2 *meta, const float *norm2, hipStream_t stream)
{
    if(count == 0) return hipSuccess;
    uint32_t blocks = (count + 3) / 4;
    if(blocks > 16384) blocks = 16384;
    if(norm2) hipLaunchKernelGGL(k_fill_screen<true>, dim3(blocks), dim3(256), 0, stream, v, first, count, screen, meta, norm2);
    else hipLaunchKernelGGL(k_fill_screen<false>, dim3(blocks), dim3(256), 0, stream, v, first, count, screen, meta, norm2);
    return hipGetLastError();
}

hipError_t launch_gather(int metric, const View &v, const uint4 *query, const uint32_t *slots, uint32_t n, float *out,
                         hipStream_t stream)
{
    if(n == 0) return hipSuccess;
    const int G_ = group_lanes_for(v.chunks);
    uint32_t  blocks = (uint32_t)(((uint64_t)n * G_ + 255) / 256);
    if(blocks > 8192) blocks = 8192;
    if(const char *ws = std::getenv("LANTERN_GPU_GATHER_WALKSHAPE")) {
        if(std::atoi(ws) != 0) {
            int dev = 0, cus = 256;
            (void)hipGetDevice(&dev);
            (void)hipDeviceGetAttribute(&cus, hipDeviceAttributeMultiprocessorCount, dev);
            const uint32_t grid = (uint32_t)std::min<uint64_t>((uint64_t)cus * 6, ((uint64_t)n * G_ + 255) / 256);
            const size_t   lds = (size_t)v.chunks * 16;
#define CALLW(MM, GG) hipLaunchKernelGGL((k_gather_walkshape<MM, GG>), dim3(grid), dim3(256), lds, stream, v, query, slots, n, out)
            LGPU_DISPATCH(metric, v.chunks, CALLW);
#undef CALLW
            return hipGetLastError();
        }
    }
#define CALL(MM, GG) hipLaunchKernelGGL((k_gather<MM, GG>), dim3(blocks), dim3(256), 0, stream, v, query, slots, n, out)
    LGPU_DISPATCH(metric, v.chunks, CALL);
#undef CALL
    return hipGetLastError();
}

hipError_t launch_pairs(int metric, const uint4 *a, uint32_t na, const uint4 *b, uint32_t nb, uint32_t chunks, float *out,
                        hipStream_t stream)
{
    if(na == 0 || nb == 0) return hipSuccess;
    const int G_ = group_lanes_for(chunks);
    uint64_t  want = ((uint64_t)na * nb * G_ + 255) / 256;
    uint32_t  blocks = want > 8192 ? 8192u : (uint32_t)want;
// ... 8 lines not shown
```

lantern_amd/csrc/kernels.hpp:

```cpp
#pragma once
#include <hip/hip_runtime.h>
#include <stddef.h>
#include <stdint.h>

#include "device_common.hpp"
#include <atomic>

#ifndef LGPU_EXPERIMENTAL
#define LGPU_EXPERIMENTAL 0
#endif

namespace lgpu {

struct FrameArgs
{
    const uint4    *queries;
    uint32_t        nq;
    const uint64_t *labels;
    uint64_t       *out_labels;
    float          *out_dists;
    uint32_t       *out_slots;
    uint32_t       *out_counts;
    uint64_t       *out_D;
    uint64_t       *out_E;
    uint32_t       *bitmaps;
    uint32_t        bm_words;
    uint32_t        undo_cap;
    uint32_t        vis_slots;
    unsigned long long *totals;
    uint32_t       *ticket;
    const uint32_t *qlist;
};

struct SearchArgs
{
    View            view;
    FrameArgs       frame;
    uint32_t        k, ef, skip;
    int             lds_list;
    int             wide_rows;
    int             spec;
    uint32_t        spec_prefetch;
    uint32_t        spec_cache;
    const float    *adc_centers;
    uint32_t        adc_S, adc_C, adc_subdim;
    uint32_t        adc_qchunks;
    unsigned long long *phase_cycles;
    uint32_t       *done;
    uint32_t       *done_flags;
    uint32_t       *touched;
    uint32_t       *trace;
    uint32_t       *trace_count;
    uint32_t        trace_cap;
    unsigned long long *screen_totals;
    const uint4    *qparams;
    uint32_t        k_stride;
    uint32_t        list_prefetch;
};

struct LinkReq
{
    uint32_t close;
    uint32_t level;
    uint32_t new_slot;
    float    d;
};

struct InsertArgs
{
    View            view;
    uint32_t        first_slot;
    uint32_t        b_begin;
    uint32_t        count;
    uint32_t        efc;
    const uint32_t *link_off;
    uint64_t       *tops;
    uint32_t       *top_count;
    uint32_t       *bitmaps;
    uint32_t        bm_words;
    uint32_t        undo_cap;
    uint32_t        vis_slots;
    unsigned long long *totals;
    uint32_t       *ticket;
    int             lds_list;
    uint32_t        spec_prefetch, spec_cache;
    uint32_t        only_upper = 0;
};
constexpr int kInsertScreenTotals = 48;

struct ConnectArgs
// ... 63 lines not shown
bool       search_solo_supported(int metric, uint32_t chunks, uint32_t M, uint32_t M0, uint32_t ef);
size_t     search_solo_lds_bytes(uint32_t ne_log2, uint32_t bm_words);
hipError_t launch_search_solo(int metric, const SearchArgs &a, int grid, hipStream_t stream);
#endif
hipError_t launch_search_adc(int metric, const SearchArgs &a, int waves, int grid, hipStream_t stream);
size_t     search_adc_lds_bytes(uint32_t code_chunks, uint32_t qchunks, uint32_t ef_cap, uint32_t M0, uint32_t vis_slots);
hipError_t launch_insert(int metric, const InsertArgs &a, int waves, int grid, hipStream_t stream);
bool       insert_spec_supported(int metric, uint32_t efc, uint32_t M0);
size_t     insert_spec_lds_bytes(uint32_t chunks, uint32_t efc, uint32_t M0, uint32_t vis_slots, uint32_t prefetch, uint32_t cache_entries);
hipError_t launch_insert_spec(int metric, const InsertArgs &a, int waves, int grid, hipStream_t stream);
hipError_t launch_connect(int metric, const ConnectArgs &a, hipStream_t stream);
hipError_t launch_revlink(int metric, const RevlinkArgs &a, void *work, uint32_t *work_count, int num_cus, hipStream_t stream,
                          bool work_count_is_zero = false);
hipError_t launch_apply_own_links(const View &v, uint32_t first_slot, const uint32_t *link_off, const LinkReq *links,
                                  uint32_t total_links, hipStream_t stream);
hipError_t launch_pack_lists(const RevlinkArgs &a, uint32_t *records, hipStream_t stream);
hipError_t launch_apply_lists(const View &v, const uint32_t *records, uint32_t nrecords, hipStream_t stream);

hipError_t launch_pq_take(const float *rows, uint32_t row_floats, uint32_t first, uint32_t count, uint32_t s, uint32_t subdim, uint32_t sub_floats,
                          float *sub, hipStream_t stream);
hipError_t launch_pq_put(float *rows, uint32_t row_floats, uint32_t first, uint32_t count, uint32_t s, uint32_t subdim, uint32_t S, const uint32_t *nearest,
                         const float *codebook, uint32_t dims, uint8_t *codes, hipStream_t stream);
hipError_t launch_pq_decode(float *rows, uint32_t row_floats, uint32_t first, uint32_t count, uint32_t subdim, uint32_t S, const float *codebook, uint32_t dims,
                            const uint8_t *codes, hipStream_t stream);

hipError_t launch_merge_parts(const uint64_t *labels, const float *dists, uint32_t world, uint32_t nq, uint32_t k, uint64_t *out_labels,
                              float *out_dists, uint32_t *out_counts, hipStream_t stream);
hipError_t launch_merge_candidates(const uint64_t *labels, const float *dists, uint32_t world, uint32_t nq, uint32_t k, uint32_t first_slot,
                                   const uint32_t *link_off, uint32_t M, uint32_t stride, uint64_t *tops, uint32_t *top_count, hipStream_t stream);
hipError_t launch_store_quantised(const float *src, uint32_t dims, uint32_t count, int kind, uint32_t *rows, uint32_t row_words, hipStream_t stream);

hipError_t launch_fill_norms(int metric, const View &v, uint32_t first, uint32_t count, float *norm2, hipStream_t stream);
hipError_t launch_fill_screen(const View &v, uint32_t first, uint32_t count, uint4 *screen, float2 *meta, const float *norm2, hipStream_t stream);
hipError_t launch_screen_probe(int metric, const View &v, const uint4 *query, const uint32_t *slots, uint32_t n, float radius, int threads,
                               uint8_t *out, hipStream_t stream);
hipError_t launch_gather(int metric, const View &v, const uint4 *query, const uint32_t *slots, uint32_t n, float *out,
                         hipStream_t stream);
hipError_t launch_pairs(int metric, const uint4 *a, uint32_t na, const uint4 *b, uint32_t nb, uint32_t chunks, float *out,
                        hipStream_t stream);

hipError_t launch_row_norms(const uint4 *rows, uint32_t n, uint32_t chunks, float *out, hipStream_t stream);
hipError_t launch_dequant_f16(const uint4 *src, size_t nchunks, uint4 *dst, hipStream_t stream);
hipError_t launch_dequant_i8(const uint4 *src, size_t nchunks, uint4 *dst, hipStream_t stream);
hipError_t launch_dense(int metric, const uint4 *Q, uint32_t nq, const uint4 *B, uint32_t nb, uint32_t chunks, const float *qn,
                        const float *bn, float *out, uint32_t ldo, hipStream_t stream);
hipError_t launch_dense_topk(int metric, const uint4 *Q, uint32_t nq, const uint4 *B, uint32_t nb, uint32_t chunks, const float *qn,
                             const float *bn, const uint64_t *best, uint32_t kk, uint64_t *cand, uint32_t *cnt, uint32_t cap, uint32_t c_base,
                             hipStream_t stream);
hipError_t launch_select_candidates(uint32_t nq, uint64_t *best, uint32_t kk, const uint64_t *cand, uint32_t *cnt, uint32_t cap, uint32_t *overflow,
                                    hipStream_t stream);
hipError_t launch_select(const float *dist, uint32_t ldo, uint32_t nq, uint32_t ncols, uint32_t c_base, uint64_t *best, uint32_t kk,
                         hipStream_t stream);
hipError_t launch_rerank(int metric, const uint4 *Q, uint32_t nq, const uint4 *B, uint32_t chunks, const uint64_t *best, uint32_t kk,
                         uint32_t k, uint32_t *out_slots, float *out_dists, hipStream_t stream);
hipError_t launch_certify(int metric, const uint64_t *best, uint32_t kk, const float *dists, uint32_t k, const float *qn, uint32_t nq, const float *bn,
                          uint32_t nb, uint32_t dims, uint32_t *flag, hipStream_t stream);
hipError_t launch_gather_rows(const uint4 *src, uint32_t chunks, const uint32_t *idx, uint32_t n, uint4 *dst, hipStream_t stream);
hipError_t launch_emit_topk(const uint64_t *best, uint32_t k, const uint32_t *idx, uint32_t n, uint32_t *out_slots, float *out_dists, hipStream_t stream);

size_t search_lds_bytes(uint32_t chunks, uint32_t ef_cap, uint32_t M0, uint32_t vis_slots);
size_t insert_lds_bytes(uint32_t chunks, uint32_t efc, uint32_t M0, uint32_t vis_slots);

}
```

lantern_amd/csrc/search_kernel.hpp:

```cpp
#pragma once
#include <algorithm>
#include <cstddef>
#include <cstdlib>

#include "kernels.hpp"
#include "walk.hpp"
#include "walk_spec.hpp"
#ifndef LGPU_EXPERIMENTAL
#define LGPU_EXPERIMENTAL 0
#endif
#if LGPU_EXPERIMENTAL
#include "experimental/walk_twin.hpp"
#endif
#include "dispatch.hpp"
#include "query_frame.hpp"

namespace lgpu {

#define LGPU_SEARCH_ARG(base, field) LGPU_KARG(base, decltype(SearchArgs::field), offsetof(SearchArgs, field))
#define LGPU_VIEW_ARG(base, STRUCT, field) LGPU_KARG(base, decltype(View::field), offsetof(STRUCT, view) + offsetof(View, field))
#define LGPU_LOAD_VIEW(v, base, STRUCT)             \
    {                                               \
        v.vec = LGPU_VIEW_ARG(base, STRUCT, vec);   \
        v.chunks = LGPU_VIEW_ARG(base, STRUCT, chunks); \
// ... 34 lines not shown
    static_assert(!EACH || (!PROF && (SPEC == 0 || SPEC == 2)), "the per-query form exists for the classic shapes and the 3 + 8 wave shape");
    const int tid = threadIdx.x, T = blockDim.x;
    WalkLds   s;
    SpecLds   sc;
    {
        const KernargBytes ka = kernarg_opaque();
        unsigned char     *end = carve_walk(lgpu_smem, s, LGPU_VIEW_ARG(ka, SearchArgs, chunks), LGPU_SEARCH_ARG(ka, ef), LGPU_VIEW_ARG(ka, SearchArgs, M0),
                                            LGPU_FRAME_ARG(ka, SearchArgs, vis_slots));
        if constexpr(SPEC != 0) carve_spec(end, sc, LGPU_VIEW_ARG(ka, SearchArgs, M0), LGPU_SEARCH_ARG(ka, spec_prefetch), LGPU_SEARCH_ARG(ka, spec_cache), SPEC == 3 ? 1u : 0u);
        else (void)end;
    }
    constexpr bool SCREEN = LGPU_SCREEN && (METRIC == M_L2SQ || METRIC == M_COS) && G == 64 && !PROF && SPEC == 0 && KPL > 0;
    for(uint32_t pos = blockIdx.x; pos < LGPU_FRAME_ARG(kernarg_opaque(), SearchArgs, nq);) {
        uint32_t    q = pos;
        QueryParams each{};
        if constexpr(EACH) {
            const KernargBytes ka = kernarg_opaque();
            q = frame_query<SearchArgs, true>(ka, pos);
            each = query_params(ka, q);
        }
        uint32_t D = 0, E = 0;
        int      cnt = 0;
        unsigned long long pc[ 8 ] = { 0, 0, 0, 0, 0, 0, 0, 0 }, t_q = 0;
        {
            const KernargBytes ka = kernarg_opaque();
            View               v;
            LGPU_LOAD_VIEW(v, ka, SearchArgs)
            if constexpr(METRIC >= M_PQD) LGPU_LOAD_VIEW_PQD(v, ka, SearchArgs)
            if constexpr(SCREEN) {
                if(tid == 0) {
                    uint64_t *const sp = (uint64_t *)&s.scal[ S_SCREEN ];
                    sp[ 0 ] = (uint64_t)LGPU_VIEW_ARG(ka, SearchArgs, screen);
                    sp[ 1 ] = (uint64_t)LGPU_VIEW_ARG(ka, SearchArgs, screen_meta);
                    s.scal[ S_NREJ ] = 0;
                }
            }
            uint32_t        bm_words;
            uint32_t *const bitmap = frame_bind<SearchArgs>(ka, s, bm_words);
            const int       ef = EACH ? (int)each.ef : (int)LGPU_SEARCH_ARG(ka, ef);
            frame_stage<METRIC, G>(tid, T, s, LGPU_FRAME_ARG(ka, SearchArgs, queries), q, v.chunks);
            if constexpr(SCREEN) {
                if(LGPU_VIEW_ARG(ka, SearchArgs, screen)) screen_stage_query<METRIC>(tid, s, v.chunks, __int_as_float(s.scal[ S_QN2 ]));
            }
            if constexpr(PROF) {
                t_q = (unsigned long long)clock64();
                s.touched = LGPU_SEARCH_ARG(ka, touched);
                s.trace_cap = LGPU_SEARCH_ARG(ka, trace_cap);
                uint32_t *const tr = LGPU_SEARCH_ARG(ka, trace);
                s.trace = tr ? tr + (size_t)q * s.trace_cap : nullptr;
                s.trace_count = tr ? LGPU_SEARCH_ARG(ka, trace_count) + q : nullptr;
            }
            if(v.n != 0 && (!EACH || each.k != 0)) {
                uint32_t start;
                if constexpr(SPEC != 0) start = greedy_descent_spec<METRIC, G>(v, s, v.entry, v.max_level, 0, D);
                else start = greedy_descent<METRIC, G, PROF>(v, s, v.entry, v.max_level, 0, D);
                if constexpr(PROF) pc[ 6 ] = (unsigned long long)clock64() - t_q;
#if LGPU_EXPERIMENTAL
                if constexpr(SPEC == 3)
                    cnt = search_level_twin<METRIC, G, KPL, ROWS, (G == 64 ? 3 : 2), PROF>(v, s, sc, bitmap, bm_words, start, ef, D, E,
                                                                                           PROF ? LGPU_SEARCH_ARG(ka, phase_cycles) : nullptr);
                else
#endif
                if constexpr(SPEC != 0)
                    cnt = search_level_spec<METRIC, G, KPL, ROWS, (G == 64 && SPEC == 2 ? 3 : 2), SPEC == 2, PROF>(v, s, sc, bitmap, bm_words, start, ef, D, E,
                                                                                                                     PROF ? LGPU_SEARCH_ARG(ka, phase_cycles) : nullptr);
                else if constexpr(KPL > 0) cnt = search_level_reg<METRIC, G, KPL, PROF, ROWS, SCREEN>(v, s, bitmap, bm_words, start, 0, ef, D, E, pc, SCREEN ? LGPU_SEARCH_ARG(ka, list_prefetch) : 0u);
// ... 21 lines not shown
```

lantern_amd/csrc/search_launch.hpp:

```cpp
#pragma once
#include "search_kernel.hpp"

namespace lgpu {

#define LGPU_LAUNCH_SEARCH(...)                                                                                        \
    {                                                                                                                  \
        static LdsAttrCache attr_;        \
        ensure_dynamic_lds((const void *)k_search<__VA_ARGS__>, lds, attr_);    \
        hipLaunchKernelGGL((k_search<__VA_ARGS__>), dim3(grid), dim3(64 * waves), lds, stream, a);                     \
    }
#define LGPU_LAUNCH_SEARCH_KPL(MM, GG, PP, RR)                           \
    {                                                                    \
        if(kpl == 1) LGPU_LAUNCH_SEARCH(MM, GG, PP, RR, 1, 0, EACH)      \
        else if(kpl == 2) LGPU_LAUNCH_SEARCH(MM, GG, PP, RR, 2, 0, EACH) \
        else LGPU_LAUNCH_SEARCH(MM, GG, PP, RR, 0, 0, EACH)              \
    }

template <bool EACH> static hipError_t launch_search_classic(int metric, const SearchArgs &a, int waves, int grid, hipStream_t stream)
{
    if(EACH && a.phase_cycles) return hipErrorInvalidValue;
    const size_t lds = search_lds_bytes(a.view.chunks, a.ef, a.view.M0, a.frame.vis_slots) + (a.view.screen ? screen_query_lds_bytes(a.view.chunks) : 0);
    const int    kpl = a.lds_list ? 0 : a.ef <= 64 ? 1 : a.ef <= 128 ? 2 : 0;
    const int    G_ = group_lanes_for(a.view.chunks);
    if(a.wide_rows && !a.phase_cycles && G_ == 64) {
        bool launched = true;
        switch(metric) {
            case M_L2SQ: LGPU_LAUNCH_SEARCH_KPL(M_L2SQ, 64, false, 4); break;
            case M_COS: LGPU_LAUNCH_SEARCH_KPL(M_COS, 64, false, 4); break;
            case M_HAMMING: LGPU_LAUNCH_SEARCH_KPL(M_HAMMING, 64, false, 4); break;
            case M_L2SQ_F16: LGPU_LAUNCH_SEARCH_KPL(M_L2SQ_F16, 64, false, 4); break;
            case M_COS_F16: LGPU_LAUNCH_SEARCH_KPL(M_COS_F16, 64, false, 4); break;
            case M_L2SQ_PQD: LGPU_LAUNCH_SEARCH_KPL(M_L2SQ_PQD, 64, false, 4); break;
            case M_COS_PQD: LGPU_LAUNCH_SEARCH_KPL(M_COS_PQD, 64, false, 4); break;
            default: launched = false;
        }
        if(launched) return hipGetLastError();
    }
    if constexpr(!EACH) {
        if(a.phase_cycles) {
            if(metric == M_L2SQ && G_ == 64) LGPU_LAUNCH_SEARCH_KPL(M_L2SQ, 64, true, 2)
            else if(metric == M_L2SQ && G_ == 16) LGPU_LAUNCH_SEARCH_KPL(M_L2SQ, 16, true, 2)
            else if(metric == M_COS && G_ == 64) LGPU_LAUNCH_SEARCH_KPL(M_COS, 64, true, 2)
            else return hipErrorInvalidValue;
            return hipGetLastError();
        }
    }
#define CALL(MM, GG) LGPU_LAUNCH_SEARCH_KPL(MM, GG, false, 2)
    if(mcode_is_pqd(metric)) PQD_G(metric, a.view.chunks, CALL);
    else LGPU_DISPATCH(metric, a.view.chunks, CALL);
#undef CALL
    return hipGetLastError();
}

#define LGPU_SPEC_ROWS(GG) ((GG) == 64 ? 4 : (GG) == 32 ? 2 : 1)
// ... 54 lines not shown
```

lantern_amd/csrc/search_plan.cpp:

```cpp
#include "index.hpp"

#include <algorithm>
#include <cstdlib>
#include <cstring>

namespace lgpu {

SearchEnv search_env()
{
    SearchEnv e;
    if(const char *se = std::getenv("LANTERN_GPU_SPEC")) { e.spec_set = true; e.spec = std::atoi(se); }
    if(const char *se = std::getenv("LANTERN_GPU_ADC_SPEC")) { e.adc_spec_set = true; e.adc_spec = std::atoi(se) != 0; }
    if(const char *pa = std::getenv("LANTERN_GPU_PQ_ADC")) e.pq_adc = std::atoi(pa) != 0;
    if(const char *sw = std::getenv("LANTERN_GPU_SPEC_WAVES")) e.spec_waves = std::atoi(sw);
    if(const char *ll = std::getenv("LANTERN_GPU_LDS_LIST")) e.lds_list = std::atoi(ll) != 0;
    if(const char *lp = std::getenv("LANTERN_GPU_SCREEN_LIST_PREFETCH")) e.screen_list_prefetch = std::atoi(lp) != 0;
    static const int  wide_env = std::getenv("LANTERN_GPU_WIDE_ROWS") ? std::atoi(std::getenv("LANTERN_GPU_WIDE_ROWS")) : -1;
    static const bool solo_auto = std::getenv("LANTERN_GPU_SOLO") && std::atoi(std::getenv("LANTERN_GPU_SOLO")) != 0;
    static const int  forced = std::getenv("LANTERN_GPU_WAVES_PER_CU") ? std::atoi(std::getenv("LANTERN_GPU_WAVES_PER_CU")) : 0;
    e.wide_rows = wide_env, e.solo = solo_auto, e.waves_per_cu = forced;
    return e;
}

SearchPlanIn search_plan_in(const Index *ix, size_t nq, size_t k, size_t ef, size_t skip, int waves)
{
    SearchPlanIn in;
    in.chunks = ix->chunks; in.M = ix->M; in.M0 = ix->M0; in.ef_default = ix->ef;
    in.mcode = ix->mcode; in.n = ix->n; in.num_cus = ix->num_cus;
    in.pq_compact = ix->pq_compact; in.pqd_inv = ix->pqd_inv; in.pq_S16 = ix->pq_S16;
    in.search_vis_slots = ix->search_vis_slots; in.search_max_wg = ix->search_max_wg;
    in.phase_profile = ix->phase_profile; in.spec_profile = ix->spec_profile;
    in.screen = ix->d_screen && ix->d_screen_meta;
    in.nq = nq; in.k = k; in.ef = ef; in.skip = skip; in.waves = waves;
    in.env = search_env();
    return in;
}

SearchPlan plan_search(const SearchPlanIn &in)
{
    const SearchEnv &env = in.env;
    const size_t     nq = in.nq;
    int              waves = in.waves;
    SearchPlan       p;
    size_t expansion = in.ef ? in.ef : in.ef_default;
    if(expansion < in.k + in.skip) expansion = in.k + in.skip;
    if(in.each) expansion = in.max_expansion;
    p.expansion = (uint32_t)expansion;
    p.lds_list = env.lds_list;
    const bool pqd = in.pq_compact && !env.pq_adc && in.pqd_inv != 0;
    if(in.pq_compact && !pqd) {
        const uint32_t code_chunks = in.pq_S16 / 16;
        uint32_t       vis_slots = 2048;
        if(in.search_vis_slots >= 0) vis_slots = (uint32_t)in.search_vis_slots / 4 * 4;
        while(vis_slots && search_adc_lds_bytes(code_chunks, in.chunks, (uint32_t)expansion, in.M0, vis_slots) > 150 * 1024) vis_slots = vis_slots > 256 ? vis_slots - 256 : 0;
        if(vis_slots && vis_slots < 4 * in.M0) vis_slots = 0;
        size_t lds = search_adc_lds_bytes(code_chunks, in.chunks, (uint32_t)expansion, in.M0, vis_slots);
        if(lds > 160 * 1024) { p.refusal = "lantern_gpu: ef/k exceed the 160 KiB LDS budget of the ADC search kernel"; return p; }
        int per_cu = (int)std::max<size_t>(1, std::min<size_t>(2, (160 * 1024) / lds));
        bool adc_spec = false;
        const uint32_t adc_prefetch = in.M0 % 4 == 0 && in.M0 <= 32 ? 1u : 0u, adc_cache = adc_prefetch ? 128u : 0u;
        if(waves <= 0 && in.M0 >= 2 && in.M0 <= 64 && expansion <= 128 && !env.lds_list) {
            const size_t with_spec = lds + search_spec_lds_bytes(in.M0, adc_prefetch, adc_cache);
            adc_spec = with_spec <= 160 * 1024 && (env.adc_spec_set ? env.adc_spec : (per_cu == 1 || nq <= (size_t)in.num_cus * 2));
            if(adc_spec) {
                lds = with_spec;
// ... 27 lines not shown
                uint32_t     ne_log2 = 9;
                while(ne_log2 > 5 && search_solo_lds_bytes(ne_log2, (uint32_t)words) > 160 * 1024) --ne_log2;
                const bool prof_ok = !in.spec_profile || (in.mcode == M_L2SQ && in.chunks == 32);
                if(pqd || !prof_ok || !search_solo_supported(in.mcode, in.chunks, in.M, in.M0, (uint32_t)expansion) ||
                   search_solo_lds_bytes(ne_log2, (uint32_t)words) > 160 * 1024)
                    spec = 2;
                else {
                    const size_t lds = search_solo_lds_bytes(ne_log2, (uint32_t)words);
                    const size_t per_cu = std::max<size_t>(1, std::min<size_t>(4, (160 * 1024) / lds));
                    size_t       gmax = (size_t)in.num_cus * per_cu;
                    if(in.search_max_wg > 0) gmax = (size_t)in.search_max_wg;
                    p.path = kSearchSolo, p.spec = 4, p.took_spec = true;
                    p.waves = 1, p.grid = (int)std::max<size_t>(1, std::min(gmax, nq));
                    p.vis_slots = (uint32_t)words, p.lds = lds;
                    p.spec_cache = ne_log2, p.lds_list = 0;
                    return p;
                }
            }
            if(spec == 3 && !(expansion <= 64 && (in.mcode == M_L2SQ || in.mcode == M_COS) && (group_lanes_for(in.chunks) == 64 || (in.mcode == M_L2SQ && group_lanes_for(in.chunks) == 16))))
                spec = 2;
#endif
        }
        waves = spec >= 2 ? 11 : spec == 1 ? 4 : waves < 0 ? -waves : 4;
        if(spec && env.spec_waves >= (spec >= 2 ? 4 : 2) && env.spec_waves <= (spec >= 2 ? 11 : 8)) waves = env.spec_waves;
    }
    const int      G_ = group_lanes_for(in.chunks), LW_ = G_ >= 32 ? 1 : G_ == 16 ? 2 : 4;
    const uint32_t spec_prefetch = spec && in.M0 % (uint32_t)LW_ == 0 && in.M0 <= (uint32_t)(G_ * LW_) ? 1u : 0u;
    const uint32_t spec_cache = !spec_prefetch ? 0u : spec >= 2 ? 128u : 64u;
    const size_t   spec_lds = spec ? search_spec_lds_bytes(in.M0, spec_prefetch, spec_cache, spec == 3) : 0;
    const size_t lds_budget = spec >= 2 ? 96 * 1024 : spec == 1 ? 39 * 1024 : 26 * 1024;
    const bool   screened = in.screen && spec == 0 && !pqd && screen_rows_for(in.chunks) && (in.mcode == M_L2SQ || in.mcode == M_COS) &&
                          !(in.phase_profile && !in.each) && !env.lds_list && expansion <= 128;
    const size_t screen_lds = screened ? screen_query_lds_bytes(in.chunks) : 0;
    uint32_t vis_slots = 1024;
    while(vis_slots < 8192 && vis_slots / 4 * 3 < expansion * in.M0 * 2) vis_slots <<= 1;
    if(in.search_vis_slots >= 0) vis_slots = (uint32_t)in.search_vis_slots / 4 * 4;
    while(vis_slots && search_lds_bytes(in.chunks, (uint32_t)expansion, in.M0, vis_slots) + spec_lds + screen_lds > lds_budget)
        vis_slots = vis_slots > 256 ? vis_slots - 256 : 0;
    if(vis_slots && vis_slots < 4 * in.M0) vis_slots = 0;
    p.lds = search_lds_bytes(in.chunks, (uint32_t)expansion, in.M0, vis_slots) + spec_lds + screen_lds;
    p.screen_lds = (uint32_t)screen_lds;
    p.list_prefetch = screened && LGPU_SCREEN_LIST_PREFETCH != 0 && in.M0 <= 64 &&
                      (env.screen_list_prefetch >= 0 ? env.screen_list_prefetch != 0 : LGPU_SCREEN_LIST_PREFETCH >= 2);
    if(p.lds > 160 * 1024) { p.refusal = "lantern_gpu: ef/k exceed the 160 KiB LDS budget of the search kernel"; return p; }
    p.path = pqd ? kSearchPqd : spec == 0 ? kSearchClassic : spec == 1 ? kSearchSpec1 : spec == 2 ? kSearchSpec2 : kSearchTwin;
    p.spec = spec, p.took_spec = spec != 0;
    p.waves = waves, p.grid = search_grid(in.num_cus, in.search_max_wg, env.waves_per_cu, nq, waves, spec >= 2 ? waves : spec == 1 ? 16 : 24);
    p.vis_slots = vis_slots, p.spec_prefetch = spec_prefetch, p.spec_cache = spec_cache;
    p.wide_rows = spec ? 0 : env.wide_rows >= 0 ? env.wide_rows : (nq * (size_t)waves <= (size_t)in.num_cus * 16 && nq >= 64);
    return p;
}

static bool search_launch(Index *ix, const SearchPlan &p, const uint4 *d_queries, size_t nq, size_t k, size_t skip, const SearchOut &out,
                          hipStream_t stream, uint32_t *done, uint32_t *done_flags, const EachLaunch *each)
{
    const bool adc = p.path == kSearchAdc, pqd = p.path == kSearchPqd, solo = p.path == kSearchSolo;
    ix->last_search_grid = p.grid;
    const int slot = acquire_search_slot(ix, stream, (size_t)p.grid);
    if(slot < 0) return false;
    SearchArgs a{};
    a.view = ix->view();
    a.frame.queries = d_queries;
    a.frame.nq = (uint32_t)nq, a.k = (uint32_t)k, a.ef = p.expansion, a.skip = (uint32_t)skip;
    a.frame.labels = ix->d_labels;
    a.frame.out_labels = out.labels, a.frame.out_dists = out.dists, a.frame.out_slots = out.slots;
    a.frame.out_counts = out.counts, a.frame.out_D = out.D, a.frame.out_E = out.E;
    if(!solo) a.frame.bitmaps = ix->slot_bitmaps[ slot ], a.frame.bm_words = (uint32_t)ix->slot_words[ slot ], a.frame.undo_cap = vis_undo_cap();
    a.frame.vis_slots = p.vis_slots;
    a.frame.totals = ix->d_totals;
    a.screen_totals = ix->d_screen ? ix->d_totals + 48 : nullptr;
    a.frame.ticket = next_ticket(ix, nq, p.grid, stream);
    a.done = done, a.done_flags = done_flags;
    a.lds_list = p.lds_list, a.wide_rows = p.wide_rows;
    a.spec = p.spec, a.spec_prefetch = p.spec_prefetch, a.spec_cache = p.spec_cache;
    a.list_prefetch = p.list_prefetch;
    hipError_t e = hipSuccess;
    if(!p.screen_lds) a.view.screen = nullptr, a.view.screen_meta = nullptr, a.view.screen_chunks = 0;
    if(adc || pqd) a.view.vec = (const uint4 *)ix->d_codes16;
    if(adc) {
        a.view.chunks = ix->pq_S16 / 16;
        a.adc_centers = ix->d_centers;
        a.adc_S = ix->pq_S, a.adc_C = ix->pq_C, a.adc_subdim = ix->pq_subdim, a.adc_qchunks = ix->chunks;
    } else {
        if(pqd) {
            a.view.pq_centers = (const uint4 *)ix->d_centers;
            a.view.pq_cps = ix->pq_subdim / 4;
            a.view.pq_C = ix->pq_C;
            a.view.pq_inv = ix->pqd_inv;
            a.view.pq_row_bytes = ix->pq_S16;
        }
        const bool prof_walk = ix->phase_profile && !pqd && !each;
        a.phase_cycles = each ? nullptr : p.spec ? (ix->spec_profile ? ix->d_totals + 16 : nullptr) : prof_walk ? ix->d_totals + 8 : nullptr;
        a.touched = (!p.spec && prof_walk && ix->unique_rows_on && ix->d_touched && ix->touched_words * 32 >= ix->cap) ? ix->d_touched : nullptr;
        if(!p.spec && prof_walk && ix->trace_on && ix->d_trace && nq <= ix->trace_nq) {
            e = hipMemsetAsync(ix->d_trace_count, 0, nq * 4, stream);
            a.trace = ix->d_trace, a.trace_count = ix->d_trace_count, a.trace_cap = (uint32_t)ix->trace_cap;
        }
    }
    if(each) {
        const char *d_tbl = each->d_table;
        if(!d_tbl) {
            char *const d = (char *)scratch(ix, launch_table_scratch(slot), each->table_bytes);
            if(!d) return false;
            if(hipMemcpyAsync(d, each->h_table, each->table_bytes, hipMemcpyHostToDevice, stream) != hipSuccess)
                return set_err(ix, "lantern_gpu: HIP failure (per-query parameter table)"), false;
            d_tbl = d;
        }
        a.qparams = (const uint4 *)d_tbl;
// ... 62 lines not shown
        SearchPlanIn in = search_plan_in(ix, cls[ c ].size(), k_stride, 0, 0, waves);
        in.each = true, in.max_expansion = top[ c ];
        plans[ c ] = plan_search(in);
        if(!plans[ c ].refusal) continue;
        for(uint32_t i : cls[ c ]) {
            in.max_expansion = tbl[ 4 * i + 1 ];
            if(plan_search(in).refusal) return set_err(ix, std::string(plans[ c ].refusal) + " (params[" + std::to_string(i) + "])"), false;
        }
        return set_err(ix, plans[ c ].refusal), false;
    }
    uint32_t *lists = tbl + 4 * nq;
    size_t    at = 0;
    uint32_t  launches = 0, any_spec = 0;
    EachLaunch each[ 3 ];
    for(int c = 0; c < 3; ++c) {
        std::stable_sort(cls[ c ].begin(), cls[ c ].end(), [&](uint32_t x, uint32_t y) { return tbl[ 4 * x + 1 ] > tbl[ 4 * y + 1 ]; });
        each[ c ] = EachLaunch{ h_block, nq * 20, d_block, (nq * 4 + at) * 4 };
        if(!cls[ c ].empty()) std::memcpy(lists + at, cls[ c ].data(), cls[ c ].size() * 4);
        at += cls[ c ].size();
    }
    for(int c = 0; c < 3; ++c) {
        if(cls[ c ].empty()) continue;
        if(!search_launch(ix, plans[ c ], d_queries, cls[ c ].size(), k_stride, 0, out, stream, nullptr, done_flags, &each[ c ])) return false;
        launches += 1;
        any_spec |= plans[ c ].took_spec ? 1u : 0u;
    }
    const uint32_t shape[ 6 ] = { launches, (uint32_t)cls[ 0 ].size(), (uint32_t)cls[ 1 ].size(), (uint32_t)cls[ 2 ].size(), std::max(top[ 0 ], std::max(top[ 1 ], top[ 2 ])), any_spec };
    std::copy(std::begin(shape), std::end(shape), ix->last_params);
    return true;
}

}

static const char *plan_search_flat(const int64_t *in, bool screen, uint32_t *out, uint32_t *screen_lds, int screen_list_prefetch = -1, uint32_t *list_prefetch = nullptr)
{
    if(!in || !out) return "lantern_gpu: null array";
    lgpu::SearchPlanIn s;
    s.screen = screen;
    s.chunks = (uint32_t)in[ 0 ]; s.M = (uint32_t)in[ 1 ]; s.M0 = (uint32_t)in[ 2 ]; s.mcode = (int)in[ 3 ]; s.n = (size_t)in[ 4 ];
    s.ef_default = (uint32_t)in[ 5 ]; s.num_cus = (int)in[ 6 ]; s.pq_compact = in[ 7 ] != 0; s.pqd_inv = (uint32_t)in[ 8 ]; s.pq_S16 = (uint32_t)in[ 9 ];
    s.search_vis_slots = (int)in[ 10 ]; s.search_max_wg = (int)in[ 11 ]; s.phase_profile = in[ 12 ] != 0; s.spec_profile = in[ 13 ] != 0;
    s.nq = (size_t)in[ 14 ]; s.k = (size_t)in[ 15 ]; s.ef = (size_t)in[ 16 ]; s.skip = (size_t)in[ 17 ]; s.waves = (int)in[ 18 ];
    s.each = in[ 19 ] != 0; s.max_expansion = (uint32_t)in[ 20 ];
    s.env.spec_set = in[ 21 ] != 0; s.env.spec = (int)in[ 22 ]; s.env.adc_spec_set = in[ 23 ] != 0; s.env.adc_spec = in[ 24 ] != 0;
    s.env.pq_adc = in[ 25 ] != 0; s.env.spec_waves = (int)in[ 26 ]; s.env.lds_list = in[ 27 ] != 0; s.env.wide_rows = (int)in[ 28 ];
    s.env.solo = in[ 29 ] != 0; s.env.waves_per_cu = (int)in[ 30 ];
    s.env.screen_list_prefetch = screen_list_prefetch;
    const lgpu::SearchPlan p = lgpu::plan_search(s);
    const uint32_t flat[ 12 ] = { (uint32_t)p.path, (uint32_t)p.spec, p.expansion, (uint32_t)p.waves, (uint32_t)p.grid, p.vis_slots, (uint32_t)p.lds,
                                  p.spec_prefetch, p.spec_cache, (uint32_t)p.wide_rows, p.took_spec ? 1u : 0u, (uint32_t)p.lds_list };
    std::copy(std::begin(flat), std::end(flat), out);
    if(screen_lds) *screen_lds = p.screen_lds;
    if(list_prefetch) *list_prefetch = p.list_prefetch;
    return p.refusal;
}
extern "C" const char *lantern_gpu_plan_search(const int64_t in[ 31 ], uint32_t out[ 12 ]) { return plan_search_flat(in, false, out, nullptr); }
extern "C" const char *lantern_gpu_plan_search_screen(const int64_t in[ 32 ], uint32_t out[ 13 ])
{
    if(!in || !out) return "lantern_gpu: null array";
    return plan_search_flat(in, in[ 31 ] != 0, out, out + 12);
}
extern "C" const char *lantern_gpu_plan_search_screen_prefetch(const int64_t in[ 33 ], uint32_t out[ 14 ])
{
    if(!in || !out) return "lantern_gpu: null array";
    return plan_search_flat(in, in[ 31 ] != 0, out, out + 12, in[ 32 ] < 0 ? -1 : in[ 32 ] != 0, out + 13);
}
```

lantern_amd/csrc/usearch_file.cpp:

```cpp
#include <algorithm>
#include <cstdio>
#include <cstdlib>
#include <cstring>
#include <functional>
#include <unordered_map>
#include <vector>

#include "index.hpp"
#include "abi_guard.hpp"

namespace lgpu {

namespace {
constexpr size_t OFF_MAGIC = 0;
constexpr size_t OFF_VERSION = 7;
constexpr size_t OFF_KIND_METRIC = 13;
constexpr size_t OFF_KIND_SCALAR = 14;
constexpr size_t OFF_KIND_KEY = 15;
constexpr size_t OFF_KIND_SLOT = 16;
constexpr size_t OFF_COUNT_PRESENT = 17;
constexpr size_t OFF_COUNT_DELETED = 25;
constexpr size_t OFF_DIMENSIONS = 33;
constexpr size_t OFF_MULTI = 41;
constexpr size_t OFF_G_SIZE = 80;
// ... 359 lines not shown
    std::lock_guard<std::mutex> g(ix->mu);
    try {
        if(!mirror_from_retriever(ix, header136) && e) *e = ix->err.c_str();
    } catch(const std::exception &) {
        if(e) *e = set_err(ix, "lantern_gpu: out of host memory while mirroring the page graph");
    }
}
LANTERN_ABI_CATCH_VOID(e)

void usearch_update_header(usearch_index_t h, char *header136, usearch_error_t *e)
try {
    if(e) *e = nullptr;
    Index *ix = (Index *)h;
    if(ix) (void)hipSetDevice(ix->device);
    if(!ix || !header136) { if(e) *e = "lantern_gpu: null index handle or header"; return; }
    std::lock_guard<std::mutex> g(ix->mu);
    if(!flush_locked(ix)) { if(e) *e = ix->err.c_str(); return; }
    put<uint64_t>(header136, OFF_COUNT_PRESENT, logical_size(ix));
    put<uint64_t>(header136, OFF_G_SIZE, logical_size(ix));
    put<uint64_t>(header136, OFF_G_MAX_LEVEL, ix->n ? (uint64_t)ix->max_level : 0);
    if(ix->n) put<uint64_t>(header136, OFF_G_ENTRY_SLOT, ix->page_mode ? ix->page_slots[ ix->entry ] : (uint64_t)ix->entry);
}
LANTERN_ABI_CATCH_VOID(e)

void usearch_add_external(usearch_index_t h, usearch_label_t label, const void *vector, void *node_tape, usearch_scalar_kind_t kind,
                          int16_t level, uint64_t slot, usearch_error_t *e)
try {
    if(e) *e = nullptr;
    Index *ix = (Index *)h;
    if(ix) (void)hipSetDevice(ix->device);
    if(!ix || !vector || !node_tape) { if(e) *e = "lantern_gpu: null index handle, vector or node tape"; return; }
    if(level < 0 || level > 255) { if(e) *e = "lantern_gpu: level out of range"; return; }
    usearch_error_t err = nullptr;
    lantern_gpu_flush(h, &err);
    if(err) { if(e) *e = err; return; }
    uint32_t id;
    {
        std::lock_guard<std::mutex> g(ix->mu);
        if(ix->page_mode && !ix->current_holder().retriever_mut) { if(e) *e = set_err(ix, "lantern_gpu: usearch_add_external needs init_options.retriever_mut"); return; }
        id = (uint32_t)ix->n;
        if(ix->page_mode) {
            const uint64_t s48 = slot & 0xFFFFFFFFFFFFull;
            if(ix->page_ids.count(s48)) { if(e) *e = set_err(ix, "lantern_gpu: usearch_add_external: the slot is already in the index"); return; }
            if(ix->page_slots.size() != ix->n) { if(e) *e = set_err(ix, "lantern_gpu: the mirror and its page slots are out of step"); return; }
            ix->page_slots.push_back(s48);
            ix->page_ids.emplace(s48, id);
        }
    }
    lantern_gpu_add_with_level(h, label, vector, kind, (int)level, &err);
    if(!err) lantern_gpu_flush(h, &err);
    std::lock_guard<std::mutex> g(ix->mu);
    if(err || ix->n != (size_t)id + 1) {
        if(ix->page_mode && ix->page_slots.size() > ix->n) {
            ix->page_ids.erase(ix->page_slots.back());
            ix->page_slots.pop_back();
        }
        if(e) *e = err ? err : set_err(ix, "lantern_gpu: usearch_add_external: the insertion did not complete");
        return;
    }
    if(!write_back_insert(ix, id, (char *)node_tape) && e) *e = ix->err.c_str();
}
LANTERN_ABI_CATCH_VOID(e)


uint64_t usearch_header_get_entry_slot(char *h) { return get<uint64_t>(h, OFF_G_ENTRY_SLOT); }
void     usearch_header_set_entry_slot(char *h, uint64_t slot) { put<uint64_t>(h, OFF_G_ENTRY_SLOT, slot); }

size_t usearch_serialized_length(usearch_index_t h, usearch_error_t *e)
try {
    if(e) *e = nullptr;
    Index *ix = (Index *)h;
    if(ix) (void)hipSetDevice(ix->device);
    if(!ix) { if(e) *e = "lantern_gpu: null index handle"; return 0; }
    std::lock_guard<std::mutex> g(ix->mu);
    if(!flush_locked(ix)) { if(e) *e = ix->err.c_str(); return 0; }
    return serialized_length(ix);
}
LANTERN_ABI_CATCH(e)

void usearch_save_buffer(usearch_index_t h, char *buffer, size_t length, usearch_error_t *e)
try {
    if(e) *e = nullptr;
    Index *ix = (Index *)h;
// ... 86 lines not shown
```

lantern_amd/csrc/walk.hpp:

```cpp
#pragma once
#include <type_traits>

#include "device_common.hpp"

namespace lgpu {

enum { S_POS = 0, S_NNEW, S_CNT, S_ANY, S_BAD, S_CUR, S_CURD, S_CHANGED, S_VISCNT, S_SPILL, S_QN2, S_NNEW0, S_NNEW1, S_ANY0, S_ANY1,
       S_FRONT = 16, S_WORST = 20,
       S_MASK = 24,
       S_SCALARS = 28,
       S_NSURV = S_ANY0, S_NREJ = S_ANY1, S_SCREEN = S_MASK,
       S_NTEST = 15 };

struct WalkLds
{
    uint4    *q;
    uint64_t *keys;
    uint64_t *keys2;
    uint64_t *newkeys;
    uint64_t *sorted;
    uint32_t *newids;
    int      *scal;
    uint32_t *vis;
    uint32_t  vis_slots;
    uint32_t *touched;
    uint32_t *trace, *trace_count;
    uint32_t  trace_cap;
    uint32_t *undo;
    uint32_t  undo_cap;
};
constexpr uint32_t TRACE_LIST0 = 0x80000000u, TRACE_LISTU = 0xC0000000u;

template <bool PROF> __device__ __forceinline__ void trace_append(const WalkLds &s, uint32_t entry)
{
    if constexpr(PROF) {
        if(s.trace) {
            const uint32_t p = atomicAdd(s.trace_count, 1u);
            if(p < s.trace_cap) s.trace[ p ] = entry;
        }
    } else {
        (void)s;
        (void)entry;
    }
}
// ... 285 lines not shown
                        const uint64_t k = make_key(d[ r ], ids[ r ]);
                        s.newkeys[ at(j) ] = k;
                        any |= k < worst;
                    }
                }
                if(ANY && any) *any_slot = 1;
            }
        }
    } else
    for(int i = g; i < nnew; i += 2 * NG) {
        const int      j = i + NG;
        const uint32_t id0 = s.newids[ at(i) ];
        const uint32_t id1 = j < nnew ? s.newids[ at(j) ] : id0;
        float          d0, d1;
        group_dist2_n<METRIC, G>(walk_query<METRIC>(s), row_of_m<METRIC>(v, id0), row_of_m<METRIC>(v, id1), (int)v.chunks, gl, qn2, row_norm<METRIC>(v, id0),
                                 row_norm<METRIC>(v, id1), d0, d1);
        if(gl == G - 1) {
            reread();
            uint64_t k0 = make_key(d0, id0);
            s.newkeys[ at(i) ] = k0;
            bool any = k0 < worst;
            if(j < nnew) {
                uint64_t k1 = make_key(d1, id1);
                s.newkeys[ at(j) ] = k1;
                any |= k1 < worst;
            }
            if(ANY && any) *any_slot = 1;
        }
    }
}


__device__ __forceinline__ uint32_t *screen_query_block(const WalkLds &s) { return s.vis + s.vis_slots; }

template <int METRIC> __device__ __forceinline__ void screen_stage_query(const int tid, const WalkLds &s, uint32_t chunks, float qn2)
{
    uint32_t *const blk = screen_query_block(s);
    if(__builtin_amdgcn_readfirstlane(tid) < 64) {
        const uint32_t lane = (uint32_t)tid, sch = screen_chunks_for(chunks);
        uint32_t       mb = 0;
        for(uint32_t i = lane; i < chunks; i += 64) {
            const uint4 x = s.q[ i ];
            mb = max(max(mb, x.x & 0x7FFFFFFFu), max(max(x.y & 0x7FFFFFFFu, x.z & 0x7FFFFFFFu), x.w & 0x7FFFFFFFu));
        }
        for(int off = 32; off > 0; off >>= 1) mb = max(mb, (uint32_t)__shfl_xor((int)mb, off));
        const float sx = __uint_as_float(mb) / 32639.f;
        const bool  ok = mb < 0x7F800000u && mb != 0u && (METRIC == M_COS ? (sx >= 0x1p-126f && sx <= 0x1p100f) : screen_l2_scale_ok(sx));
        float    S = 0.f;
        uint32_t hh = 0, hl = 0, ll = 0;
        for(uint32_t i = lane; i < 4 * sch; i += 64) {
            const uint4 x = i < chunks ? s.q[ i ] : make_uint4(0u, 0u, 0u, 0u);
            const float xs[ 4 ] = { __uint_as_float(x.x), __uint_as_float(x.y), __uint_as_float(x.z), __uint_as_float(x.w) };
            uint32_t    hw = 0, lw = 0;
#pragma unroll
            for(int b = 0; b < 4; ++b) {
                const float q = ok ? xs[ b ] / sx : 0.f;
                const float Xf = fminf(fmaxf(__builtin_rintf(q), -32639.f), 32639.f);
                const float rho = __builtin_fabsf(q - Xf) + 0x1p-9f;
                S = __builtin_fmaf(rho, rho, S);
                const int X = (int)Xf, h = (X + 128) >> 8, l = X - 256 * h;
                hw |= ((uint32_t)h & 0xFFu) << (8 * b);
                lw |= ((uint32_t)l & 0xFFu) << (8 * b);
            }
            hh = (uint32_t)dot4_i8(hw, hw, (int)hh);
            hl = (uint32_t)dot4_i8(hw, lw, (int)hl);
            ll = (uint32_t)dot4_i8(lw, lw, (int)ll);
            blk[ 4 + 8 * (i / 4) + i % 4 ] = hw;
            blk[ 8 + 8 * (i / 4) + i % 4 ] = lw;
        }
        S = group_sum<64>(S);
        hh = group_sum<64>(hh), hl = group_sum<64>(hl), ll = group_sum<64>(ll);
        if(lane == 63) {
            float delta = __builtin_inff(), nx2 = 0.f;
            if(ok) {
                delta = (sx * __builtin_sqrtf(S)) * (1.f + 0x1p-10f);
                if constexpr(METRIC == M_COS) delta = (delta / qn2) * (1.f + 0x1p-10f);
                nx2 = (sx * sx) * (float)(65536.0 * (double)(int)hh + 512.0 * (double)(int)hl + (double)(int)ll);
            }
            blk[ 0 ] = __float_as_uint(ok ? sx : 0.f);
            blk[ 1 ] = __float_as_uint(delta);
            blk[ 2 ] = __float_as_uint(nx2);
            blk[ 3 ] = 0u;
        }
    }
    __syncthreads();
}

#ifndef LGPU_SCREEN_NB
#define LGPU_SCREEN_NB 3
#endif
template <int METRIC, int G, int ROWS, bool TALLY = false>
__device__ __forceinline__ int hop_distances_screened(const View &v, WalkLds &s, int nnew, uint64_t worst, float qn2)
{
    static_assert(METRIC == M_L2SQ || METRIC == M_COS, "the screen serves the f32 l2sq and cosine walks");
    constexpr int GS = 8, NB = TALLY ? 3 : LGPU_SCREEN_NB;
    static_assert(G % GS == 0, "a screen group lies within one wave");
    const int       tid = threadIdx.x, T = blockDim.x, gs = tid / GS, NGS = T / GS;
    int             gsl = tid % GS;
    if constexpr(!TALLY) asm volatile("" : "+v"(gsl));
    uint32_t *const surv = (uint32_t *)s.sorted;
    typedef uint32_t u32x4 __attribute__((ext_vector_type(4)));
    typedef float    f32x2 __attribute__((ext_vector_type(2)));
    typedef const __attribute__((address_space(1))) u32x4 *ScreenRow;
    typedef const __attribute__((address_space(1))) f32x2 *ScreenMeta;
    auto uniform = [](uint64_t x) {
        return (uint64_t)(uint32_t)__builtin_amdgcn_readfirstlane((int)(uint32_t)x) |
               (uint64_t)(uint32_t)__builtin_amdgcn_readfirstlane((int)(uint32_t)(x >> 32)) << 32;
    };
    const ScreenRow  screen = (ScreenRow)uniform(((const uint64_t *)&s.scal[ S_SCREEN ])[ 0 ]);
    const ScreenMeta screen_meta = (ScreenMeta)uniform(((const uint64_t *)&s.scal[ S_SCREEN ])[ 1 ]);
    const uint32_t   chunks = v.chunks, sch = screen_chunks_for(chunks);
    const uint32_t *const blk = screen_query_block(s);
    const uint4 *const    planes = (const uint4 *)(blk + 4);
    for(int j = gs; j < nnew; j += NGS) {
        const uint32_t id = s.newids[ j ];
        const ScreenRow row = screen + (size_t)id * sch;
        const f32x2     meta = screen_meta[ id ];
        int            ih = 0, il = 0, c2 = 0;
        for(uint32_t base = (uint32_t)gsl; base < sch; base += NB * GS) {
            u32x4 y[ NB ];
#pragma unroll
            for(int c = 0; c < NB; ++c)
                if(base + c * GS < sch) y[ c ] = row[ base + c * GS ];
#pragma unroll
            for(int c = 0; c < NB; ++c)
                if(base + c * GS < sch) {
                    const uint4    hq = planes[ 2 * (base + c * GS) ], lq = planes[ 2 * (base + c * GS) + 1 ];
                    const uint32_t w[ 4 ] = { y[ c ].x, y[ c ].y, y[ c ].z, y[ c ].w };
                    const uint32_t hs[ 4 ] = { hq.x, hq.y, hq.z, hq.w }, ls[ 4 ] = { lq.x, lq.y, lq.z, lq.w };
#pragma unroll
                    for(int k = 0; k < 4; ++k) {
                        ih = dot4_i8(hs[ k ], w[ k ], ih);
                        il = dot4_i8(ls[ k ], w[ k ], il);
                        if constexpr(METRIC == M_L2SQ) c2 = dot4_i8(w[ k ], w[ k ], c2);
                    }
                }
        }
        ih = (int)group_sum<GS>((uint32_t)ih);
        il = (int)group_sum<GS>((uint32_t)il);
        if constexpr(METRIC == M_L2SQ) c2 = (int)group_sum<GS>((uint32_t)c2);
        if(gsl == GS - 1) {
            bool        reject = false;
            const float sx = __uint_as_float(blk[ 0 ]), delta = __uint_as_float(blk[ 1 ]);
            const float fI = (float)(256.0 * (double)ih + (double)il);
            const float rd = key_dist(worst), e = fmaxf(0x1p-12f, (float)(2 * chunks + 64) * 0x1p-24f);
            if constexpr(METRIC == M_COS) {
                if(screen_cos_norm_ok(qn2)) {
                    const float sim8 = ((fI * sx) * meta.x) / qn2;
                    const float ub = ((sim8 + meta.y * (1.f + delta)) + delta) + e;
                    reject = (1.f - ub) - e > rd;
                }
            } else {
                const float ome = 1.f - e;
                if(screen_l2_scale_ok(meta.x)) {
                    const float nx2 = __uint_as_float(blk[ 2 ]);
                    const float R = (2.f * (sx * meta.x)) * fI, Q = (meta.x * meta.x) * (float)c2;
                    const float m = ((nx2 - R) + Q) - 0x1p-20f * (nx2 + Q);
                    if(__builtin_isfinite(m)) {
                        const float a = (__builtin_sqrtf(fmaxf(m, 0.f)) * ome - meta.y) - delta;
                        const float lb = a > 0.f ? a * a : 0.f;
                        reject = lb > 0x1p-100f && lb * ome > rd;
                    }
                }
            }
            if(reject) s.newkeys[ j ] = ~0ull;
            else surv[ atomicAdd(&s.scal[ S_NSURV ], 1) ] = (uint32_t)j;
        }
    }
    __syncthreads();
    const int ns = s.scal[ S_NSURV ];
    if(tid == 0) {
        s.scal[ S_NREJ ] += nnew - ns;
        if constexpr(TALLY) s.scal[ S_NTEST ] += nnew;
    }
    return ns;
}

template <int METRIC, int G, bool PROF = false, int ROWS = 2>
__device__ int search_level(const View &v, WalkLds &s, uint32_t *bitmap, uint32_t bm_words, uint32_t start, int level, int ef,
                            uint32_t &D, uint32_t &E, unsigned long long *prof = nullptr)
{
    const int tid = threadIdx.x, T = blockDim.x, g = tid / G, gl = tid % G;
    const int lane = tid & 63;
    const bool wave0 = __builtin_amdgcn_readfirstlane(tid) < 64;
    unsigned long long tl = 0;
    if constexpr(PROF) tl = (unsigned long long)clock64();
#define LGPU_MARK(i)                                                  \
    if constexpr(PROF) {                                              \
        if(tid == 0) {                                                \
            const unsigned long long t_ = (unsigned long long)clock64(); \
            prof[ i ] += t_ - tl;                                     \
            tl = t_;                                                  \
        }                                                             \
    }
    for(uint32_t i = tid; i < s.vis_slots; i += T) s.vis[ i ] = EMPTY;
    const float qn2 = __int_as_float(s.scal[ S_QN2 ]);
    if(g == 0) {
        float d = group_dist_n<METRIC, G>(walk_query<METRIC>(s), row_of_m<METRIC>(v, start), (int)v.chunks, gl, qn2, row_norm<METRIC>(v, start));
// ... 254 lines not shown
            }
            LGPU_MARK(3)
            if constexpr(PROF) {
                if(split && lane == 0) prof[ 4 ] += (unsigned long long)clock64() - tw;
            }
        }
        if(visit_wave) {
            if(split) {
                const uint64_t f = front_pub[ par ], w = worst_pub[ par ];
                uint64_t       t = f != ~0ull ? f : w;
                bool           got = f != ~0ull;
                for(int base = 0; base < pend; base += 64) {
                    const uint64_t     N = base + lane < pend ? s.newkeys[ base + lane ] : ~0ull;
                    unsigned long long m = __ballot(N < t);
                    while(m) {
                        t = readlane64(N, (int)__builtin_ctzll(m));
                        got = true;
                        m = __ballot(N < t);
                    }
                }
                node = got ? (uint32_t)t >> 1 : EMPTY;
                LGPU_MARK(3)
            }
            if(node == EMPTY) {
                if(lane == 0) *nnew_slot = -1;
            } else {
                E += 1;
                if(!split) LGPU_MARK(4)
                if(s.vis_slots && !spilled && viscnt + v.M0 > s.vis_slots / 4 * 3) spilled = true;
                uint32_t        cap;
                const uint32_t *list = neighbors_of(v, node, level, cap);
                if(lane == 0) trace_append<PROF>(s, node | (level > 0 ? TRACE_LISTU : TRACE_LIST0));
                const bool have_list = pf_on && node == pf_node;
                int nb_new = 0;
                for(uint32_t off = 0; off < cap; off += 64) {
                    const uint32_t i = off + (uint32_t)lane;
                    uint32_t       nb;
                    if(have_list) nb = pf_nb;
                    else nb = i < cap ? list[ i ] : EMPTY;
                    if constexpr(PROF) {
                        asm volatile("s_waitcnt vmcnt(0)" ::: "memory");
                        LGPU_MARK(5)
                    }
                    const bool isnew = hop_is_new(s, bitmap, nb, spilled);
                    const unsigned long long m = __ballot(isnew);
                    if(isnew) {
                        s.newids[ nb_new + __popcll(m & ((1ull << lane) - 1ull)) ] = nb;
                        mark_touched<PROF>(s, nb);
                    }
                    if(spilled || !s.vis_slots) undo_record(s, undo, isnew, nb, m, lane);
                    nb_new += __popcll(m);
                }
                if(s.vis_slots && !spilled) viscnt += (uint32_t)nb_new;
                if(lane == 0) {
                    *nnew_slot = nb_new;
                    if(SCREEN) s.scal[ S_NSURV ] = 0;
                }
            }
        }
        LGPU_MARK(0)
        __syncthreads();
        const int nnew = *nnew_slot;
        LGPU_MARK(1)
        if(nnew < 0) break;
        pend = nnew;
        if(pf_on && visit_wave) {
            const uint64_t nf = front_pub[ par ^ 1 ];
            pf_node = nf != ~0ull ? (uint32_t)__builtin_amdgcn_readfirstlane((int)((uint32_t)nf >> 1)) : EMPTY;
            if(pf_node != EMPTY) pf_nb = (uint32_t)lane < v.M0 ? v.nbr0[ (size_t)pf_node * v.M0 + (uint32_t)lane ] : EMPTY;
        }
        if(nnew == 0) continue;
        if constexpr(SCREEN) {
            const uint64_t radius = screen_on ? worst_pub[ par ^ 1 ] : ~0ull;
            int            ne = nnew;
            if(radius != ~0ull) ne = hop_distances_screened<METRIC, G, ROWS, TALLY>(v, s, nnew, radius, qn2);
            hop_distances<METRIC, G, ROWS, false, true>(v, s, ne, qn2, ~0ull, nullptr, radius != ~0ull ? (const uint32_t *)s.sorted : nullptr);
        } else {
            hop_distances<METRIC, G, ROWS, false>(v, s, nnew, qn2, ~0ull, nullptr);
        }
        D += (uint32_t)nnew;
        __syncthreads();
        LGPU_MARK(2)
    }
    if(visit_wave) undo_apply<SCREEN && !TALLY>(s, bitmap, bm_words, undo, lane);
    if(list_wave) {
#pragma unroll
        for(int r = 0; r < KPL; ++r)
            if(r * 64 + lane < cnt) s.keys[ r * 64 + lane ] = K[ r ];
        if(lane == 0) s.scal[ S_CNT ] = cnt;
    }
    __syncthreads();
    return s.scal[ S_CNT ];
}
#undef LGPU_MARK

struct RefineLds
{
    float    *cd;
    uint32_t *cid;
    float    *sd;
    uint32_t *sid;
};
__device__ __forceinline__ unsigned char *carve_refine(unsigned char *p, RefineLds &r, uint32_t n_max)
{
    auto up16 = [](size_t x) { return (x + 15) & ~(size_t)15; };
    r.cd = (float *)p;      p += up16((size_t)n_max * 4);
    r.cid = (uint32_t *)p;  p += up16((size_t)n_max * 4);
    r.sd = (float *)p;      p += up16((size_t)n_max * 4);
// ... 55 lines not shown
```

Baseline: 2.546 million.

## Store per-edge neighbour screen metadata beside adjacency lists for screened walks

Adds a per-edge table that copies each level-0 neighbour's screen metadata (scale/norm pair) into a buffer laid out parallel to the adjacency list. It is rebuilt after inserts and loads. During screened search, when a hop heuristic says it pays off, the walk reads the pairs contiguously while reading the neighbour list and stages them in LDS, so the screen no longer does a scattered gather of screen_meta per candidate. In exchange it uses M0*8 extra bytes per node of device memory, adds a full-index refill kernel after mutations, and needs extra LDS and a second global load per neighbour.

```diff
diff --git a/include/lantern_gpu.h b/include/lantern_gpu.h
--- a/include/lantern_gpu.h
+++ b/include/lantern_gpu.h
@@ -226,6 +226,8 @@
 LANTERN_GPU_EXPORT const char *lantern_gpu_plan_search(const int64_t in[31], uint32_t out[12]);
 LANTERN_GPU_EXPORT const char *lantern_gpu_plan_search_screen(const int64_t in[32], uint32_t out[13]);
 LANTERN_GPU_EXPORT const char *lantern_gpu_plan_search_screen_prefetch(const int64_t in[33], uint32_t out[14]);
+LANTERN_GPU_EXPORT const char *lantern_gpu_plan_search_nbr_meta(const int64_t in[35], uint32_t out[15]);
+LANTERN_GPU_EXPORT uint32_t lantern_gpu_last_search_nbr_meta(usearch_index_t, usearch_error_t *);
 
 LANTERN_GPU_EXPORT void lantern_gpu_distance_gather(usearch_index_t, const void *query, const uint32_t *slots,
                                                     size_t n, float *out, usearch_error_t *);
@@ -236,6 +238,7 @@
 LANTERN_GPU_EXPORT const char *lantern_gpu_plan_insert(const int64_t in[13], uint32_t out[7]);
 LANTERN_GPU_EXPORT size_t lantern_gpu_export_screen(usearch_index_t, size_t first, size_t count, int8_t *rows, float *meta, float *norms,
                                                     usearch_error_t *);
+LANTERN_GPU_EXPORT size_t lantern_gpu_export_nbr_meta(usearch_index_t, size_t first, size_t count, float *pairs, usearch_error_t *);
 LANTERN_GPU_EXPORT void lantern_gpu_screen_probe(usearch_index_t, const void *query, const uint32_t *slots, size_t n, float radius,
                                                  int workgroup, uint8_t *rejected, usearch_error_t *);
 LANTERN_GPU_EXPORT void lantern_gpu_distance_matrix(const void *a, size_t na, const void *b, size_t nb,
diff --git a/lantern_amd/capi.py b/lantern_amd/capi.py
--- a/lantern_amd/capi.py
+++ b/lantern_amd/capi.py
@@ -110,6 +110,7 @@
     "lantern_gpu_search_batch_params", "lantern_gpu_search_batch_params_lane", "lantern_gpu_search_batch_params_lane_notify",
     "lantern_gpu_search_batch_params_device", "lantern_gpu_last_params_launch", "lantern_scan_server_start_params_fn",
     "lantern_gpu_export_screen", "lantern_gpu_screen_probe",
+    "lantern_gpu_plan_search_nbr_meta", "lantern_gpu_last_search_nbr_meta", "lantern_gpu_export_nbr_meta",
 ]
 QUERY_PARAMS = np.dtype([("k", np.uint32), ("ef", np.uint32), ("skip", np.uint32), ("reserved", np.uint32)])
 
@@ -204,6 +205,8 @@
         "lantern_gpu_set_insert_screen": (None, [vp, C.c_int, err]),
         "lantern_gpu_insert_screen_stats": (None, [vp, vp, err]),
         "lantern_gpu_export_screen": (sz, [vp, sz, sz, vp, vp, vp, err]),
+        "lantern_gpu_export_nbr_meta": (sz, [vp, sz, sz, vp, err]),
+        "lantern_gpu_last_search_nbr_meta": (C.c_uint32, [vp, err]),
         "lantern_gpu_screen_probe": (None, [vp, vp, vp, sz, f32, i32, vp, err]),
         "lantern_gpu_save_stream": (None, [vp, vp, vp, err]),
         "lantern_gpu_pq_compact": (None, [vp, err]),
@@ -258,6 +261,7 @@
         "lantern_gpu_plan_search": (C.c_char_p, [vp, vp]),
         "lantern_gpu_plan_search_screen": (C.c_char_p, [vp, vp]),
         "lantern_gpu_plan_search_screen_prefetch": (C.c_char_p, [vp, vp]),
+        "lantern_gpu_plan_search_nbr_meta": (C.c_char_p, [vp, vp]),
         "lantern_gpu_plan_insert": (C.c_char_p, [vp, vp]),
         "lantern_gpu_row_shard_plan": (sz, [vp, i32, u64, u32, sz, sz, vp, vp, vp, sz]),
         "lantern_scan_server_start": (vp, [vp, C.c_char_p, i32, sz, C.c_uint, err]),
@@ -560,6 +564,20 @@
         _call("lantern_gpu_export_screen", self.h, first, count, _ptr(codes), _ptr(meta), _ptr(norms))
         return {"codes": codes, "meta": meta, "norms": norms, "row_bytes": row_bytes}
 
+    def export_nbr_meta(self, first=0, count=None):
+        if count is None:
+            count = len(self) - first
+        m0 = int(_call("lantern_gpu_export_nbr_meta", self.h, first, count, None))
+        if m0 == 0:
+            return None
+        pairs = np.zeros((count, m0, 2), np.float32)
+        if int(_call("lantern_gpu_export_nbr_meta", self.h, first, count, _ptr(pairs))) != m0:
+            return None
+        return pairs
+
+    def last_search_nbr_meta(self) -> bool:
+        return bool(_call("lantern_gpu_last_search_nbr_meta", self.h))
+
     def screen_probe(self, query, slots, radius, workgroup=256):
         q = _rows(query, self.metric)[0]
         s = np.ascontiguousarray(slots, dtype=np.uint32)
@@ -1078,7 +1096,12 @@
 def plan_search(fields) -> tuple[dict, str | None]:
     vals = [fields[n] for n in PLAN_SEARCH_IN] if isinstance(fields, dict) else list(fields)
     assert len(vals) == len(PLAN_SEARCH_IN)
-    if isinstance(fields, dict) and "screen_list_prefetch" in fields:
+    if isinstance(fields, dict) and "nbr_meta_valid" in fields:
+        names = PLAN_SEARCH_OUT + ("screen_lds", "list_prefetch", "nbr_meta")
+        a = np.asarray(vals + [fields.get("screen", 0), fields.get("screen_list_prefetch", -1), fields["nbr_meta_valid"], fields.get("env_nbr_meta", -1)], dtype=np.int64)
+        out = np.zeros(len(names), dtype=np.uint32)
+        why = lib().lantern_gpu_plan_search_nbr_meta(_ptr(a), _ptr(out))
+    elif isinstance(fields, dict) and "screen_list_prefetch" in fields:
         names = PLAN_SEARCH_OUT + ("screen_lds", "list_prefetch")
         a = np.asarray(vals + [fields.get("screen", 0), fields["screen_list_prefetch"]], dtype=np.int64)
         out = np.zeros(len(names), dtype=np.uint32)
diff --git a/lantern_amd/csrc/device_common.hpp b/lantern_amd/csrc/device_common.hpp
--- a/lantern_amd/csrc/device_common.hpp
+++ b/lantern_amd/csrc/device_common.hpp
@@ -522,6 +522,7 @@
 __host__ __device__ inline bool screen_cos_norm_ok(float r) { return r >= 0x1p-48f && r <= 0x1p48f; }
 __host__ __device__ inline uint32_t screen_chunks_for(uint32_t chunks) { return (chunks + 3) / 4; }
 __host__ __device__ inline uint32_t screen_query_lds_bytes(uint32_t chunks) { return 16 + screen_chunks_for(chunks) * 32; }
+__host__ __device__ inline uint32_t nbr_meta_lds_bytes(uint32_t M0) { return M0 * 8; }
 __host__ __device__ inline bool screen_l2_scale_ok(float s) { return s >= 0x1p-40f && s <= 0x1p40f; }
 
 __device__ __forceinline__ const uint4 *row_of(const View &v, uint32_t slot) { return v.vec + (size_t)slot * v.chunks; }
diff --git a/lantern_amd/csrc/index.cpp b/lantern_amd/csrc/index.cpp
--- a/lantern_amd/csrc/index.cpp
+++ b/lantern_amd/csrc/index.cpp
@@ -105,6 +105,7 @@
         const size_t srow = (size_t)screen_chunks_for(ix->chunks) * 16;
         if(!dev_grow(ix, (void **)&ix->d_screen, oc * srow, newcap * srow, 0)) return false;
         if(!dev_grow(ix, (void **)&ix->d_screen_meta, oc * 8, newcap * 8, 0)) return false;
+        if(ix->nbr_meta && !dev_grow(ix, (void **)&ix->d_nbr_meta, oc * ix->M0 * 8, newcap * ix->M0 * 8, 0)) return false;
     }
     if(ix->pq && !dev_grow(ix, (void **)&ix->d_codes, oc * ix->pq_S, newcap * ix->pq_S, 0)) return false;
     if(!dev_grow(ix, (void **)&ix->d_labels, oc * 8, newcap * 8, -1)) return false;
@@ -132,9 +133,21 @@
 bool rows_stored(Index *ix, size_t first, size_t count)
 {
     if(count == 0) return true;
+    ix->nbr_meta_valid = false;
     if(ix->d_norm2) HIPCHK(ix, launch_fill_norms(ix->mcode, ix->view(), (uint32_t)first, (uint32_t)count, ix->d_norm2, ix->stream));
     if(ix->d_screen)
         HIPCHK(ix, launch_fill_screen(ix->view(), (uint32_t)first, (uint32_t)count, ix->d_screen, ix->d_screen_meta, ix->mcode == M_COS ? ix->d_norm2 : nullptr, ix->stream));
+    return true;
+}
+
+bool refill_nbr_meta(Index *ix)
+{
+    if(!ix->d_nbr_meta || !ix->d_screen_meta || ix->nbr_meta_valid) return true;
+    if(ix->n) {
+        HIPCHK(ix, launch_fill_nbr_meta(ix->view(), 0, (uint32_t)ix->n, ix->d_nbr_meta, ix->stream));
+        if(!record_launch(ix, ix->stream)) return false;
+    }
+    ix->nbr_meta_valid = true;
     return true;
 }
 
@@ -529,6 +542,7 @@
     gs.temp = (void *)(((uintptr_t)(gs.idx_b + total_links) + 63) & ~(uintptr_t)63);
     gs.temp_bytes = temp_bytes;
 
+    ix->nbr_meta_valid = false;
     prof_mark(ix, 0);
     HIPCHK(ix, launch_batch_layout(ix->d_levels + first, (uint32_t)b, ix->M, d_link_off, d_item_node, ix->stream));
 
@@ -860,7 +874,7 @@
     if(!rows_stored(ix, first, total)) return false;
     bool ok = true;
     run_batches(ix, all_labels.data(), s, total, comm, &ok);
-    return ok;
+    return ok && refill_nbr_meta(ix);
 }
 
 static bool row_shard_candidates(Index *ix, const RowShard &rs, size_t first, size_t b, const uint32_t *d_link_off, uint64_t *d_tops, uint32_t *d_top_count)
@@ -946,6 +960,7 @@
     struct Cleanup { Index *a = nullptr; ~Cleanup() { usearch_error_t ig = nullptr; if(a) usearch_free(a, &ig); } } cleanup;
     cleanup.a = loc;
     loc->seed = ix->seed;
+    loc->nbr_meta = false;
     loc->efc = ix->efc;
     loc->add_batch_max = ix->add_batch_max;
     loc->add_min_ratio = ix->add_min_ratio;
@@ -1027,7 +1042,7 @@
     ix->upper_off.assign(s.uo.begin(), s.uo.begin() + (ptrdiff_t)done);
     ix->upper_blocks = 0;
     for(size_t i = 0; i < done; ++i) ix->upper_blocks += (size_t)s.lv[ i ];
-    return ok;
+    return ok && refill_nbr_meta(ix);
 }
 
 bool flush_locked(Index *ix)
@@ -1214,6 +1229,8 @@
     ix->radius_stale = true;
     ix->entry = entry_slot;
     ix->max_level = max_level;
+    ix->nbr_meta_valid = false;
+    if(!refill_nbr_meta(ix)) return false;
     if(ix->pq) {
         const char *pc = std::getenv("LANTERN_GPU_PQ_COMPACT");
         if(pc && std::atoi(pc) != 0 && !pq_compact_locked(ix)) return false;
@@ -1344,7 +1361,7 @@
     CLEAR(e);
     Index *ix = H(h, e);
     if(!ix) return;
-    void *ptrs[] = { ix->d_vec, ix->d_norm2, ix->d_screen, ix->d_screen_meta, ix->d_labels, ix->d_levels, ix->d_nbr0, ix->d_upper_off, ix->d_upper_nbr, ix->d_bitmaps, ix->d_totals, ix->d_tickets,
+    void *ptrs[] = { ix->d_vec, ix->d_norm2, ix->d_screen, ix->d_screen_meta, ix->d_nbr_meta, ix->d_labels, ix->d_levels, ix->d_nbr0, ix->d_upper_off, ix->d_upper_nbr, ix->d_bitmaps, ix->d_totals, ix->d_tickets,
                      ix->d_radius0, ix->d_radius_upper,
                      ix->d_codebook, ix->d_centers, ix->d_codes, ix->d_codes16, ix->d_touched, ix->d_trace, ix->d_trace_count };
     for(void *p : ptrs)
@@ -1419,7 +1436,7 @@
         if(!flush_locked(ix)) { FAIL(e, ix->err.c_str()); return; }
         bool ok = true;
         insert_rows(ix, labels, nullptr, (const uint32_t *)vectors, n, &ok);
-        if(!ok) FAIL(e, ix->err.c_str());
+        if(!ok || !refill_nbr_meta(ix)) FAIL(e, ix->err.c_str());
         return;
     }
     if(n >= ix->add_batch_max && (int)kind == usearch_scalar_f32_k && level < 0 &&
@@ -1427,7 +1444,7 @@
         if(!flush_locked(ix)) { FAIL(e, ix->err.c_str()); return; }
         bool ok = true;
         insert_rows(ix, labels, nullptr, (const uint32_t *)vectors, n, &ok, true);
-        if(!ok) FAIL(e, ix->err.c_str());
+        if(!ok || !refill_nbr_meta(ix)) FAIL(e, ix->err.c_str());
         return;
     }
     const size_t base = ix->pend_labels.size();
@@ -1442,7 +1459,7 @@
         throw;
     }
     for(size_t i = 0; i < n; ++i) pad_row(ix, (const char *)vectors + i * in_bytes, (int)kind, &ix->pend_rows[ (base + i) * row_words ]);
-    if(ix->pend_labels.size() >= ix->add_batch_max && !flush_locked(ix)) FAIL(e, ix->err.c_str());
+    if(ix->pend_labels.size() >= ix->add_batch_max && (!flush_locked(ix) || (n > 1 && !refill_nbr_meta(ix)))) FAIL(e, ix->err.c_str());
 }
 LANTERN_ABI_CATCH_VOID(e)
 
@@ -1629,7 +1646,7 @@
     Index *ix = H(h, e);
     if(!ix) return;
     std::lock_guard<std::mutex> g(ix->mu);
-    if(!flush_locked(ix)) FAIL(e, ix->err.c_str());
+    if(!flush_locked(ix) || !refill_nbr_meta(ix)) FAIL(e, ix->err.c_str());
 }
 LANTERN_ABI_CATCH_VOID(e)
 
@@ -2641,6 +2658,36 @@
 }
 LANTERN_ABI_CATCH(e)
 
+size_t lantern_gpu_export_nbr_meta(usearch_index_t h, size_t first, size_t count, float *pairs, usearch_error_t *e)
+try {
+    CLEAR(e);
+    if(count > SIZE_MAX - first) { FAIL(e, "lantern_gpu: slot range out of the index"); return 0; }
+    Index *ix = H(h, e);
+    if(!ix) return 0;
+    std::lock_guard<std::mutex> g(ix->mu);
+    if(!flush_locked(ix)) { FAIL(e, ix->err.c_str()); return 0; }
+    if(first + count > ix->n) { FAIL(e, "lantern_gpu: slot range out of the index"); return 0; }
+    if(!ix->d_nbr_meta || !ix->nbr_meta_valid) return 0;
+    if(count && pairs) {
+        const size_t row = (size_t)ix->M0 * 8;
+        const bool   ok = hipMemcpyAsync(pairs, (const char *)ix->d_nbr_meta + first * row, count * row, hipMemcpyDeviceToHost, ix->stream) == hipSuccess &&
+                        hipStreamSynchronize(ix->stream) == hipSuccess;
+        if(!ok) { FAIL(e, "lantern_gpu: HIP failure exporting the neighbours' pairs"); return 0; }
+    }
+    return ix->M0;
+}
+LANTERN_ABI_CATCH(e)
+
+uint32_t lantern_gpu_last_search_nbr_meta(usearch_index_t h, usearch_error_t *e)
+try {
+    CLEAR(e);
+    Index *ix = H(h, e);
+    if(!ix) return 0;
+    std::lock_guard<std::mutex> g(ix->mu);
+    return ix->last_search_nbr_meta;
+}
+LANTERN_ABI_CATCH(e)
+
 void lantern_gpu_screen_probe(usearch_index_t h, const void *query, const uint32_t *slots, size_t n, float radius, int workgroup,
                               uint8_t *rejected, usearch_error_t *e)
 try {
@@ -2817,7 +2864,8 @@
     if(row_bytes) *row_bytes = ix->pq_compact ? std::max<size_t>(ix->n, 1) * ix->pq_S16 : (ix->d_vec ? cap * (size_t)ix->chunks * 16 : 0);
     if(other_bytes)
         *other_bytes = cap * ((size_t)ix->M0 * 4 + 8 + 1 + 4 + 4) + ix->upper_cap * ((size_t)ix->M * 4 + 4) + (ix->d_norm2 ? cap * 4 : 0) +
-                       (ix->pq ? cap * (size_t)ix->pq_S : 0) + (ix->d_screen ? cap * ((size_t)screen_chunks_for(ix->chunks) * 16 + 8) : 0);
+                       (ix->pq ? cap * (size_t)ix->pq_S : 0) + (ix->d_screen ? cap * ((size_t)screen_chunks_for(ix->chunks) * 16 + 8) : 0) +
+                       (ix->d_nbr_meta ? cap * (size_t)ix->M0 * 8 : 0);
 }
 LANTERN_ABI_CATCH_VOID(e)
 
diff --git a/lantern_amd/csrc/index.hpp b/lantern_amd/csrc/index.hpp
--- a/lantern_amd/csrc/index.hpp
+++ b/lantern_amd/csrc/index.hpp
@@ -82,6 +82,10 @@
     bool      screen = false;
     uint4    *d_screen = nullptr;
     float2   *d_screen_meta = nullptr;
+    float2   *d_nbr_meta = nullptr;
+    bool      nbr_meta = true;
+    bool      nbr_meta_valid = false;
+    uint32_t  last_search_nbr_meta = 0;
     uint64_t *d_labels = nullptr;
     uint8_t  *d_levels = nullptr;
     uint32_t *d_nbr0 = nullptr;
@@ -218,6 +222,7 @@
 bool        pq_compact_locked(Index *ix);
 bool        pq_expand_locked(Index *ix);
 bool        rows_stored(Index *ix, size_t first, size_t count);
+bool        refill_nbr_meta(Index *ix);
 void       *scratch(Index *ix, int which, size_t bytes);
 bool        pad_row(const Index *ix, const void *vec, int kind_in, uint32_t *dst);
 size_t      input_bytes(const Index *ix, int kind_in);
@@ -233,6 +238,7 @@
     int  spec = 0, spec_waves = 0, wide_rows = -1, waves_per_cu = 0;
     bool adc_spec = false, pq_adc = false, lds_list = false, solo = false;
     int  screen_list_prefetch = -1;
+    int  nbr_meta = -1;
 };
 SearchEnv search_env();
 struct SearchPlanIn
@@ -241,6 +247,7 @@
     int       mcode = 0, num_cus = 0, search_vis_slots = -1, search_max_wg = 0;
     bool      pq_compact = false, phase_profile = false, spec_profile = false;
     bool      screen = false;
+    bool      nbr_meta_valid = false;
     size_t    n = 0, nq = 0, k = 0, ef = 0, skip = 0;
     int       waves = 0;
     bool      each = false;
@@ -256,6 +263,7 @@
     size_t      lds = 0;
     uint32_t    screen_lds = 0;
     uint32_t    list_prefetch = 0;
+    uint32_t    nbr_meta = 0;
     bool        took_spec = false;
     const char *refusal = nullptr;
 };
diff --git a/lantern_amd/csrc/kernels.hip b/lantern_amd/csrc/kernels.hip
--- a/lantern_amd/csrc/kernels.hip
+++ b/lantern_amd/csrc/kernels.hip
@@ -850,6 +850,19 @@
     }
 }
 
+__global__ void __launch_bounds__(256) k_fill_nbr_meta(View v, uint32_t first, uint32_t count, float2 *nbr_meta)
+{
+    const uint32_t lane = threadIdx.x & 63;
+    const uint32_t wid = (blockIdx.x * blockDim.x + threadIdx.x) >> 6, nw = (gridDim.x * blockDim.x) >> 6;
+    for(uint32_t i = wid; i < count; i += nw) {
+        const size_t at = (size_t)(first + i) * v.M0;
+        for(uint32_t j = lane; j < v.M0; j += 64) {
+            const uint32_t nb = v.nbr0[ at + j ];
+            nbr_meta[ at + j ] = nb < v.n ? v.screen_meta[ nb ] : make_float2(0.f, __builtin_inff());
+        }
+    }
+}
+
 template <int METRIC, int G>
 __global__ void __launch_bounds__(256) k_gather(View v, const uint4 *query, const uint32_t *slots, uint32_t n, float *out)
 {
@@ -1029,6 +1042,16 @@
     return hipGetLastError();
 }
 
+hipError_t launch_fill_nbr_meta(const View &v, uint32_t first, uint32_t count, float2 *nbr_meta, hipStream_t stream)
+{
+    if(count == 0) return hipSuccess;
+    if(!v.screen_meta || !v.nbr0 || !nbr_meta || (uint64_t)first + count > v.n) return hipErrorInvalidValue;
+    uint32_t blocks = (count + 3) / 4;
+    if(blocks > 16384) blocks = 16384;
+    hipLaunchKernelGGL(k_fill_nbr_meta, dim3(blocks), dim3(256), 0, stream, v, first, count, nbr_meta);
+    return hipGetLastError();
+}
+
 hipError_t launch_gather(int metric, const View &v, const uint4 *query, const uint32_t *slots, uint32_t n, float *out,
                          hipStream_t stream)
 {
diff --git a/lantern_amd/csrc/kernels.hpp b/lantern_amd/csrc/kernels.hpp
--- a/lantern_amd/csrc/kernels.hpp
+++ b/lantern_amd/csrc/kernels.hpp
@@ -56,6 +56,7 @@
     const uint4    *qparams;
     uint32_t        k_stride;
     uint32_t        list_prefetch;
+    const float2   *nbr_meta;
 };
 
 struct LinkReq
@@ -185,6 +186,7 @@
 
 hipError_t launch_fill_norms(int metric, const View &v, uint32_t first, uint32_t count, float *norm2, hipStream_t stream);
 hipError_t launch_fill_screen(const View &v, uint32_t first, uint32_t count, uint4 *screen, float2 *meta, const float *norm2, hipStream_t stream);
+hipError_t launch_fill_nbr_meta(const View &v, uint32_t first, uint32_t count, float2 *nbr_meta, hipStream_t stream);
 hipError_t launch_screen_probe(int metric, const View &v, const uint4 *query, const uint32_t *slots, uint32_t n, float radius, int threads,
                                uint8_t *out, hipStream_t stream);
 hipError_t launch_gather(int metric, const View &v, const uint4 *query, const uint32_t *slots, uint32_t n, float *out,
diff --git a/lantern_amd/csrc/search_kernel.hpp b/lantern_amd/csrc/search_kernel.hpp
--- a/lantern_amd/csrc/search_kernel.hpp
+++ b/lantern_amd/csrc/search_kernel.hpp
@@ -90,6 +90,7 @@
                     uint64_t *const sp = (uint64_t *)&s.scal[ S_SCREEN ];
                     sp[ 0 ] = (uint64_t)LGPU_VIEW_ARG(ka, SearchArgs, screen);
                     sp[ 1 ] = (uint64_t)LGPU_VIEW_ARG(ka, SearchArgs, screen_meta);
+                    *(uint64_t *)&s.scal[ S_NBRMETA ] = (uint64_t)LGPU_SEARCH_ARG(ka, nbr_meta);
                     s.scal[ S_NREJ ] = 0;
                 }
             }
diff --git a/lantern_amd/csrc/search_launch.hpp b/lantern_amd/csrc/search_launch.hpp
--- a/lantern_amd/csrc/search_launch.hpp
+++ b/lantern_amd/csrc/search_launch.hpp
@@ -19,7 +19,9 @@
 template <bool EACH> static hipError_t launch_search_classic(int metric, const SearchArgs &a, int waves, int grid, hipStream_t stream)
 {
     if(EACH && a.phase_cycles) return hipErrorInvalidValue;
-    const size_t lds = search_lds_bytes(a.view.chunks, a.ef, a.view.M0, a.frame.vis_slots) + (a.view.screen ? screen_query_lds_bytes(a.view.chunks) : 0);
+    if(a.nbr_meta && !a.view.screen) return hipErrorInvalidValue;
+    const size_t lds = search_lds_bytes(a.view.chunks, a.ef, a.view.M0, a.frame.vis_slots) + (a.view.screen ? screen_query_lds_bytes(a.view.chunks) : 0) +
+                       (a.nbr_meta ? nbr_meta_lds_bytes(a.view.M0) : 0);
     const int    kpl = a.lds_list ? 0 : a.ef <= 64 ? 1 : a.ef <= 128 ? 2 : 0;
     const int    G_ = group_lanes_for(a.view.chunks);
     if(a.wide_rows && !a.phase_cycles && G_ == 64) {
diff --git a/lantern_amd/csrc/search_plan.cpp b/lantern_amd/csrc/search_plan.cpp
--- a/lantern_amd/csrc/search_plan.cpp
+++ b/lantern_amd/csrc/search_plan.cpp
@@ -15,6 +15,7 @@
     if(const char *sw = std::getenv("LANTERN_GPU_SPEC_WAVES")) e.spec_waves = std::atoi(sw);
     if(const char *ll = std::getenv("LANTERN_GPU_LDS_LIST")) e.lds_list = std::atoi(ll) != 0;
     if(const char *lp = std::getenv("LANTERN_GPU_SCREEN_LIST_PREFETCH")) e.screen_list_prefetch = std::atoi(lp) != 0;
+    if(const char *nm = std::getenv("LANTERN_GPU_NBR_META")) e.nbr_meta = std::atoi(nm) != 0;
     static const int  wide_env = std::getenv("LANTERN_GPU_WIDE_ROWS") ? std::atoi(std::getenv("LANTERN_GPU_WIDE_ROWS")) : -1;
     static const bool solo_auto = std::getenv("LANTERN_GPU_SOLO") && std::atoi(std::getenv("LANTERN_GPU_SOLO")) != 0;
     static const int  forced = std::getenv("LANTERN_GPU_WAVES_PER_CU") ? std::atoi(std::getenv("LANTERN_GPU_WAVES_PER_CU")) : 0;
@@ -31,6 +32,7 @@
     in.search_vis_slots = ix->search_vis_slots; in.search_max_wg = ix->search_max_wg;
     in.phase_profile = ix->phase_profile; in.spec_profile = ix->spec_profile;
     in.screen = ix->d_screen && ix->d_screen_meta;
+    in.nbr_meta_valid = in.screen && ix->d_nbr_meta && ix->nbr_meta_valid;
     in.nq = nq; in.k = k; in.ef = ef; in.skip = skip; in.waves = waves;
     in.env = search_env();
     return in;
@@ -124,16 +126,27 @@
     const bool   screened = in.screen && spec == 0 && !pqd && screen_rows_for(in.chunks) && (in.mcode == M_L2SQ || in.mcode == M_COS) &&
                           !(in.phase_profile && !in.each) && !env.lds_list && expansion <= 128;
     const size_t screen_lds = screened ? screen_query_lds_bytes(in.chunks) : 0;
-    uint32_t vis_slots = 1024;
-    while(vis_slots < 8192 && vis_slots / 4 * 3 < expansion * in.M0 * 2) vis_slots <<= 1;
-    if(in.search_vis_slots >= 0) vis_slots = (uint32_t)in.search_vis_slots / 4 * 4;
-    while(vis_slots && search_lds_bytes(in.chunks, (uint32_t)expansion, in.M0, vis_slots) + spec_lds + screen_lds > lds_budget)
-        vis_slots = vis_slots > 256 ? vis_slots - 256 : 0;
-    if(vis_slots && vis_slots < 4 * in.M0) vis_slots = 0;
-    p.lds = search_lds_bytes(in.chunks, (uint32_t)expansion, in.M0, vis_slots) + spec_lds + screen_lds;
-    p.screen_lds = (uint32_t)screen_lds;
     p.list_prefetch = screened && LGPU_SCREEN_LIST_PREFETCH != 0 && in.M0 <= 64 &&
                       (env.screen_list_prefetch >= 0 ? env.screen_list_prefetch != 0 : LGPU_SCREEN_LIST_PREFETCH >= 2);
+    auto slots_for = [&](size_t extra) {
+        uint32_t vs = 1024;
+        while(vs < 8192 && vs / 4 * 3 < expansion * in.M0 * 2) vs <<= 1;
+        if(in.search_vis_slots >= 0) vs = (uint32_t)in.search_vis_slots / 4 * 4;
+        while(vs && search_lds_bytes(in.chunks, (uint32_t)expansion, in.M0, vs) + spec_lds + screen_lds + extra > lds_budget)
+            vs = vs > 256 ? vs - 256 : 0;
+        if(vs && vs < 4 * in.M0) vs = 0;
+        return vs;
+    };
+    size_t   nbr_lds = screened && in.nbr_meta_valid && !p.list_prefetch && env.nbr_meta != 0 ? nbr_meta_lds_bytes(in.M0) : 0;
+    uint32_t vis_slots = slots_for(nbr_lds);
+    const size_t bare_lds = search_lds_bytes(in.chunks, (uint32_t)expansion, in.M0, 0) + spec_lds + screen_lds;
+    if(nbr_lds && !vis_slots && (slots_for(0) || 160 * 1024 / bare_lds != 160 * 1024 / (bare_lds + nbr_lds))) {
+        nbr_lds = 0;
+        vis_slots = slots_for(0);
+    }
+    p.nbr_meta = nbr_lds != 0;
+    p.lds = search_lds_bytes(in.chunks, (uint32_t)expansion, in.M0, vis_slots) + spec_lds + screen_lds + nbr_lds;
+    p.screen_lds = (uint32_t)screen_lds;
     if(p.lds > 160 * 1024) { p.refusal = "lantern_gpu: ef/k exceed the 160 KiB LDS budget of the search kernel"; return p; }
     p.path = pqd ? kSearchPqd : spec == 0 ? kSearchClassic : spec == 1 ? kSearchSpec1 : spec == 2 ? kSearchSpec2 : kSearchTwin;
     p.spec = spec, p.took_spec = spec != 0;
@@ -166,6 +179,8 @@
     a.lds_list = p.lds_list, a.wide_rows = p.wide_rows;
     a.spec = p.spec, a.spec_prefetch = p.spec_prefetch, a.spec_cache = p.spec_cache;
     a.list_prefetch = p.list_prefetch;
+    a.nbr_meta = p.nbr_meta ? ix->d_nbr_meta : nullptr;
+    ix->last_search_nbr_meta = a.nbr_meta ? 1u : 0u;
     hipError_t e = hipSuccess;
     if(!p.screen_lds) a.view.screen = nullptr, a.view.screen_meta = nullptr, a.view.screen_chunks = 0;
     if(adc || pqd) a.view.vec = (const uint4 *)ix->d_codes16;
@@ -294,7 +309,8 @@
 
 }
 
-static const char *plan_search_flat(const int64_t *in, bool screen, uint32_t *out, uint32_t *screen_lds, int screen_list_prefetch = -1, uint32_t *list_prefetch = nullptr)
+static const char *plan_search_flat(const int64_t *in, bool screen, uint32_t *out, uint32_t *screen_lds, int screen_list_prefetch = -1, uint32_t *list_prefetch = nullptr,
+                                    bool nbr_meta_valid = false, int nbr_meta_env = -1, uint32_t *nbr_meta = nullptr)
 {
     if(!in || !out) return "lantern_gpu: null array";
     lgpu::SearchPlanIn s;
@@ -308,12 +324,14 @@
     s.env.pq_adc = in[ 25 ] != 0; s.env.spec_waves = (int)in[ 26 ]; s.env.lds_list = in[ 27 ] != 0; s.env.wide_rows = (int)in[ 28 ];
     s.env.solo = in[ 29 ] != 0; s.env.waves_per_cu = (int)in[ 30 ];
     s.env.screen_list_prefetch = screen_list_prefetch;
+    s.nbr_meta_valid = screen && nbr_meta_valid, s.env.nbr_meta = nbr_meta_env;
     const lgpu::SearchPlan p = lgpu::plan_search(s);
     const uint32_t flat[ 12 ] = { (uint32_t)p.path, (uint32_t)p.spec, p.expansion, (uint32_t)p.waves, (uint32_t)p.grid, p.vis_slots, (uint32_t)p.lds,
                                   p.spec_prefetch, p.spec_cache, (uint32_t)p.wide_rows, p.took_spec ? 1u : 0u, (uint32_t)p.lds_list };
     std::copy(std::begin(flat), std::end(flat), out);
     if(screen_lds) *screen_lds = p.screen_lds;
     if(list_prefetch) *list_prefetch = p.list_prefetch;
+    if(nbr_meta) *nbr_meta = p.nbr_meta;
     return p.refusal;
 }
 extern "C" const char *lantern_gpu_plan_search(const int64_t in[ 31 ], uint32_t out[ 12 ]) { return plan_search_flat(in, false, out, nullptr); }
@@ -327,3 +345,8 @@
     if(!in || !out) return "lantern_gpu: null array";
     return plan_search_flat(in, in[ 31 ] != 0, out, out + 12, in[ 32 ] < 0 ? -1 : in[ 32 ] != 0, out + 13);
 }
+extern "C" const char *lantern_gpu_plan_search_nbr_meta(const int64_t in[ 35 ], uint32_t out[ 15 ])
+{
+    if(!in || !out) return "lantern_gpu: null array";
+    return plan_search_flat(in, in[ 31 ] != 0, out, out + 12, in[ 32 ] < 0 ? -1 : in[ 32 ] != 0, out + 13, in[ 33 ] != 0, in[ 34 ] < 0 ? -1 : in[ 34 ] != 0, out + 14);
+}
diff --git a/lantern_amd/csrc/usearch_file.cpp b/lantern_amd/csrc/usearch_file.cpp
--- a/lantern_amd/csrc/usearch_file.cpp
+++ b/lantern_amd/csrc/usearch_file.cpp
@@ -415,7 +415,11 @@
     if(!ix || !vector || !node_tape) { if(e) *e = "lantern_gpu: null index handle, vector or node tape"; return; }
     if(level < 0 || level > 255) { if(e) *e = "lantern_gpu: level out of range"; return; }
     usearch_error_t err = nullptr;
-    lantern_gpu_flush(h, &err);
+    auto flush = [&]() {
+        std::lock_guard<std::mutex> g(ix->mu);
+        if(!flush_locked(ix)) err = ix->err.c_str();
+    };
+    flush();
     if(err) { if(e) *e = err; return; }
     uint32_t id;
     {
@@ -431,7 +435,7 @@
         }
     }
     lantern_gpu_add_with_level(h, label, vector, kind, (int)level, &err);
-    if(!err) lantern_gpu_flush(h, &err);
+    if(!err) flush();
     std::lock_guard<std::mutex> g(ix->mu);
     if(err || ix->n != (size_t)id + 1) {
         if(ix->page_mode && ix->page_slots.size() > ix->n) {
diff --git a/lantern_amd/csrc/walk.hpp b/lantern_amd/csrc/walk.hpp
--- a/lantern_amd/csrc/walk.hpp
+++ b/lantern_amd/csrc/walk.hpp
@@ -10,6 +10,7 @@
        S_MASK = 24,
        S_SCALARS = 28,
        S_NSURV = S_ANY0, S_NREJ = S_ANY1, S_SCREEN = S_MASK,
+       S_NBRMETA = S_VISCNT,
        S_NTEST = 15 };
 
 struct WalkLds
@@ -361,6 +362,18 @@
 
 
 __device__ __forceinline__ uint32_t *screen_query_block(const WalkLds &s) { return s.vis + s.vis_slots; }
+typedef float f32x2_t __attribute__((ext_vector_type(2)));
+__device__ __forceinline__ f32x2_t *screen_newmeta(const WalkLds &s, uint32_t chunks)
+{
+    return (f32x2_t *)(screen_query_block(s) + screen_query_lds_bytes(chunks) / 4);
+}
+__device__ __forceinline__ uint64_t screen_nbr_table(const WalkLds &s)
+{
+    const uint64_t x = ((const uint64_t *)&s.scal[ S_NBRMETA ])[ 0 ];
+    return (uint64_t)(uint32_t)__builtin_amdgcn_readfirstlane((int)(uint32_t)x) |
+           (uint64_t)(uint32_t)__builtin_amdgcn_readfirstlane((int)(uint32_t)(x >> 32)) << 32;
+}
+__device__ __forceinline__ bool nbr_pays(uint32_t D, int hop, uint32_t M0) { return D * 8u >= (uint32_t)hop * M0 * 5u; }
 
 template <int METRIC> __device__ __forceinline__ void screen_stage_query(const int tid, const WalkLds &s, uint32_t chunks, float qn2)
 {
@@ -419,7 +432,7 @@
 #define LGPU_SCREEN_NB 3
 #endif
 template <int METRIC, int G, int ROWS, bool TALLY = false>
-__device__ __forceinline__ int hop_distances_screened(const View &v, WalkLds &s, int nnew, uint64_t worst, float qn2)
+__device__ __forceinline__ int hop_distances_screened(const View &v, WalkLds &s, int nnew, uint64_t worst, float qn2, bool nbr = false)
 {
     static_assert(METRIC == M_L2SQ || METRIC == M_COS, "the screen serves the f32 l2sq and cosine walks");
     constexpr int GS = 8, NB = TALLY ? 3 : LGPU_SCREEN_NB;
@@ -444,7 +457,13 @@
     for(int j = gs; j < nnew; j += NGS) {
         const uint32_t id = s.newids[ j ];
         const ScreenRow row = screen + (size_t)id * sch;
-        const f32x2     meta = screen_meta[ id ];
+        f32x2           meta;
+        if constexpr(!TALLY) {
+            if(nbr) meta = screen_newmeta(s, chunks)[ j ];
+            else meta = screen_meta[ id ];
+        } else {
+            meta = screen_meta[ id ];
+        }
         int            ih = 0, il = 0, c2 = 0;
         for(uint32_t base = (uint32_t)gsl; base < sch; base += NB * GS) {
             u32x4 y[ NB ];
@@ -492,7 +511,15 @@
                     }
                 }
             }
-            if(reject) s.newkeys[ j ] = ~0ull;
+            if(reject) {
+                if constexpr(!TALLY) {
+                    uint32_t ones = ~0u;
+                    asm volatile("" : "+v"(ones));
+                    s.newkeys[ j ] = (uint64_t)ones << 32 | ones;
+                } else {
+                    s.newkeys[ j ] = ~0ull;
+                }
+            }
             else surv[ atomicAdd(&s.scal[ S_NSURV ], 1) ] = (uint32_t)j;
         }
     }
@@ -813,12 +840,22 @@
                 const uint32_t *list = neighbors_of(v, node, level, cap);
                 if(lane == 0) trace_append<PROF>(s, node | (level > 0 ? TRACE_LISTU : TRACE_LIST0));
                 const bool have_list = pf_on && node == pf_node;
+                typedef const __attribute__((address_space(1))) f32x2_t *NbrMeta;
+                NbrMeta nbr_row = nullptr;
+                if constexpr(SCREEN && !TALLY) {
+                    if(screen_on && nbr_pays(D, hop, v.M0)) nbr_row = (NbrMeta)screen_nbr_table(s);
+                    if(nbr_row) nbr_row += (size_t)node * cap;
+                }
                 int nb_new = 0;
                 for(uint32_t off = 0; off < cap; off += 64) {
                     const uint32_t i = off + (uint32_t)lane;
                     uint32_t       nb;
                     if(have_list) nb = pf_nb;
                     else nb = i < cap ? list[ i ] : EMPTY;
+                    f32x2_t pair = { 0.f, 0.f };
+                    if constexpr(SCREEN && !TALLY) {
+                        if(nbr_row && i < cap) pair = nbr_row[ i ];
+                    }
                     if constexpr(PROF) {
                         asm volatile("s_waitcnt vmcnt(0)" ::: "memory");
                         LGPU_MARK(5)
@@ -826,7 +863,11 @@
                     const bool isnew = hop_is_new(s, bitmap, nb, spilled);
                     const unsigned long long m = __ballot(isnew);
                     if(isnew) {
-                        s.newids[ nb_new + __popcll(m & ((1ull << lane) - 1ull)) ] = nb;
+                        const int at = nb_new + __popcll(m & ((1ull << lane) - 1ull));
+                        s.newids[ at ] = nb;
+                        if constexpr(SCREEN && !TALLY) {
+                            if(nbr_row) screen_newmeta(s, v.chunks)[ at ] = pair;
+                        }
                         mark_touched<PROF>(s, nb);
                     }
                     if(spilled || !s.vis_slots) undo_record(s, undo, isnew, nb, m, lane);
@@ -854,7 +895,7 @@
         if constexpr(SCREEN) {
             const uint64_t radius = screen_on ? worst_pub[ par ^ 1 ] : ~0ull;
             int            ne = nnew;
-            if(radius != ~0ull) ne = hop_distances_screened<METRIC, G, ROWS, TALLY>(v, s, nnew, radius, qn2);
+            if(radius != ~0ull) ne = hop_distances_screened<METRIC, G, ROWS, TALLY>(v, s, nnew, radius, qn2, !TALLY && nbr_pays(D, hop, v.M0) && screen_nbr_table(s) != 0);
             hop_distances<METRIC, G, ROWS, false, true>(v, s, ne, qn2, ~0ull, nullptr, radius != ~0ull ? (const uint32_t *)s.sorted : nullptr);
         } else {
             hop_distances<METRIC, G, ROWS, false>(v, s, nnew, qn2, ~0ull, nullptr);
```

Measured after the change: 2.666 million, median of 6. 1.05x the previous value.
